# cebarker1000/heatflow

Hardware: AMD Instinct MI355X
Metric: DOF-updates/s (timesteps/s x nDOF) on geballe_with_diamond (higher is better)
Workload: dtype f64

## Files before the change

heatflow_amd/csrc/heatflow_hip.hip:

```cpp

#include "hf_amg_io.hpp"

namespace {

struct MeshTables {
  std::vector<int32_t> rowptr, colidx;
  ColDict spmv;
  RowGather rg;
  std::vector<char> tag_used;
  int max_blk_nnz = 0;
};

constexpr char BLOB_MAGIC[8] = {'H', 'F', 'P', 'A', 'T', '0', '2', 0};
struct BlobHeader {
  char magic[8];
  int64_t total_bytes, nnz;
  int32_t n, ne, rba, ts, max_blk_nnz, tab_len, rg_ok, rg_max_dict, spmv_max_dict, reserved;
  int64_t count[12];
};

void steady_swap(hf_ctx* ctx) {
  hf_ctx::Steady& S = ctx->steady;
  std::swap(ctx->nbc, S.nbc); std::swap(ctx->d_bc_dofs, S.bc_dofs); std::swap(ctx->d_g, S.g);
  std::swap(ctx->nlift_rows, S.nlift_rows); std::swap(ctx->nlift, S.nlift);
// ... 32 lines not shown
  dev_free(&ctx->d_load);
  ctx->have_load = false;
}

void source_free(hf_ctx* ctx) {
  dev_free(&ctx->src.F1); dev_free(&ctx->src.sum); dev_free(&ctx->src.absorb);
  ctx->src = hf_ctx::Source();
}

int source_steps_ok(hf_ctx* ctx, int64_t n_steps, const char* call) {
  hf_ctx::Source& S = ctx->src;
  if (!S.on) return HF_OK;
  if (!S.amp.empty() && S.next + static_cast<size_t>(n_steps) > S.amp.size())
    return fail(ctx, HF_ERR_STATE, "%s: the source has %zu amplitudes left for %lld steps (hf_set_source_amplitudes)", call,
                S.amp.size() - S.next, static_cast<long long>(n_steps));
  if (ctx->have_load && !S.sum) HF_TRY(dev_alloc(ctx, &S.sum, ctx->n));
  return HF_OK;
}

void tangent_free(hf_ctx* ctx) {
  free_batch_state(ctx->tanb);
  dev_free(&ctx->tan.col); dev_free(&ctx->tan.dir); dev_free(&ctx->tan.F);
  ctx->tan = hf_ctx::Tangent();
}

void kt_free(hf_ctx* ctx) {
  hf_ctx::KappaT& K = ctx->kt;
  dev_free(&K.hdr); dev_free(&K.vals); dev_free(&K.pic); dev_free(&K.b0); dev_free(&K.change);
  dev_free(&K.chdr); dev_free(&K.cvals); dev_free(&K.w);
  K = hf_ctx::KappaT();
}

void an_free(hf_ctx* ctx) {
  dev_free(&ctx->an.d_m);
  ctx->an = hf_ctx::Aniso();
}

const char* kt_kind(const hf_ctx* ctx) { return ctx->kt.k_on || !ctx->kt.c_on ? "kappa(T)" : "rho_c(T)"; }

int install_mesh(hf_ctx* ctx, int32_t n, int32_t ne, const double* zr, const int32_t* tri, const int32_t* tag, MeshTables& T) {
  free_batch(ctx);
  free_batch_state(ctx->fluxb);
  free_batch_cols(ctx);
  proj_free(ctx);
  steady_free(ctx);
  load_free(ctx);
  source_free(ctx);
  tangent_free(ctx);
  kt_free(ctx);
  an_free(ctx);
  value_lists_free(ctx);
  ctx->n = n; ctx->ne = ne; ctx->nnz = static_cast<int64_t>(T.colidx.size());
  ctx->nchunks = (n + RB - 1) / RB;
  ctx->nblk_a = (n + RBA - 1) / RBA;
  ctx->P = std::min(ctx->nchunks, MAXP);
  if (ctx->P >= 64) ctx->P &= ~7;
  ctx->nchunks_s = (n + SRPC - 1) / SRPC;
  ctx->Ps = std::min(ctx->nchunks_s, MAXP);
  if (ctx->Ps >= 64) ctx->Ps &= ~7;
  ctx->max_chunk_nnz_s = 0;
  for (int c = 0; c < ctx->nchunks_s; ++c)
    ctx->max_chunk_nnz_s = std::max(ctx->max_chunk_nnz_s, T.rowptr[std::min<int64_t>(n, (c + 1LL) * SRPC)] - T.rowptr[static_cast<size_t>(c) * SRPC]);
  ctx->max_cdict = T.spmv.max_dict;
  ctx->c16 = true;
  if (const char* e = std::getenv("HEATFLOW_SPMV_C16")) ctx->c16 = (e[0] != '0');
  if (static_cast<size_t>(ctx->max_chunk_nnz_s + ctx->max_cdict) * 8 > 64 * 1024) ctx->c16 = false;
  ctx->cdict_own = static_cast<int>(T.spmv.ptr.size()) == ctx->nchunks_s + 1;
  for (int c = 0; c < ctx->nchunks_s && ctx->cdict_own; ++c) {
    const int32_t r0 = c * SRPC, r1 = std::min<int32_t>(n, r0 + SRPC);
    const int32_t* lo = T.spmv.dict.data() + T.spmv.ptr[c];
    const int32_t* hi = T.spmv.dict.data() + T.spmv.ptr[c + 1];
    const int32_t* at = std::lower_bound(lo, hi, r0);
    ctx->cdict_own = hi - at >= r1 - r0 && at[0] == r0 && at[r1 - r0 - 1] == r1 - 1;
  }
  ctx->max_blk_nnz = T.max_blk_nnz;
  if (static_cast<size_t>((ctx->max_blk_nnz + 1) & ~1) * 16 + (RBA + 1) * 4 > 160 * 1024)
    return fail(ctx, HF_ERR_ARG, "row block holds %d nonzeros: LDS slab too large", ctx->max_blk_nnz);
  ctx->tab_len = static_cast<int>(T.tag_used.size());
  ctx->h_tag_used = T.tag_used;
  ctx->assembled = false; ctx->have_mat = false;
  ctx->h_tri.assign(tri, tri + 3 * static_cast<size_t>(ne));
  ctx->h_tag.assign(tag, tag + ne);
  ctx->owner_ready = false;
  ctx->ncolors = 0; ctx->elist_len = 0;
  dev_free(&ctx->d_blk_eptr); dev_free(&ctx->d_blk_cptr); dev_free(&ctx->d_blk_ent);

  std::vector<int4> elem(ne);
  for (int32_t e = 0; e < ne; ++e) elem[e] = make_int4(tri[3 * e], tri[3 * e + 1], tri[3 * e + 2], tag[e]);
  HF_TRY(dev_alloc(ctx, &ctx->d_zr, n));
  HF_TRY(dev_alloc(ctx, &ctx->d_elem, ne));
  HF_TRY(dev_alloc(ctx, &ctx->d_kappa, ctx->tab_len));
  HF_TRY(dev_alloc(ctx, &ctx->d_rhoc, ctx->tab_len));
  HF_TRY(dev_alloc(ctx, &ctx->d_rowptr, n + 1));
  HF_TRY(dev_alloc(ctx, &ctx->d_colidx, ctx->nnz));
  HF_TRY(dev_alloc(ctx, &ctx->d_cdict_ptr, T.spmv.ptr.size()));
  HF_TRY(dev_alloc(ctx, &ctx->d_cdict, T.spmv.dict.size()));
  HF_TRY(dev_alloc(ctx, &ctx->d_cid, T.spmv.id.size()));
  ctx->n_cdict = static_cast<int64_t>(T.spmv.dict.size());
  HF_HIP(copy_sync(ctx, ctx->d_zr, zr, sizeof(double) * 2 * n, hipMemcpyHostToDevice));
  ctx->rg_ok = T.rg.ok && rowgather_smem_bytes(T.max_blk_nnz, T.rg.cols.max_dict) <= 160 * 1024;
  std::fill_n(ctx->rg_grid, static_cast<int>(RG_VARIANTS), 0);
  if (ctx->rg_ok) {
    const RowGather& G = T.rg;
    ctx->rg_max_dict = G.cols.max_dict;
    ctx->h_rg_tags = G.tags;
    ctx->n_rg_ell = static_cast<int64_t>(G.ell.size());
    ctx->n_rg_dict = static_cast<int64_t>(G.cols.dict.size());
    HF_TRY(dev_alloc(ctx, &ctx->d_rg_hdr, G.hdr.size()));
    HF_TRY(dev_alloc(ctx, &ctx->d_rg_ell, G.ell.size()));
    HF_TRY(dev_alloc(ctx, &ctx->d_rg_cid, G.cols.id.size() + 16));
    HF_TRY(dev_alloc(ctx, &ctx->d_rg_dict, G.cols.dict.size()));
    HF_TRY(dev_alloc(ctx, &ctx->d_rg_zrb, G.cols.dict.size()));
    HF_TRY(dev_alloc(ctx, &ctx->d_kappa_rg, 64));
    HF_TRY(dev_alloc(ctx, &ctx->d_rhoc_rg, 64));
    HF_HIP(copy_sync(ctx, ctx->d_rg_hdr, G.hdr.data(), sizeof(int4) * G.hdr.size(), hipMemcpyHostToDevice));
    HF_HIP(copy_sync(ctx, ctx->d_rg_ell, G.ell.data(), sizeof(uint16_t) * G.ell.size(), hipMemcpyHostToDevice));
    HF_HIP(hipMemsetAsync(ctx->d_rg_cid + G.cols.id.size(), 0, sizeof(uint16_t) * 16, ctx->stream));
    HF_HIP(copy_sync(ctx, ctx->d_rg_cid, G.cols.id.data(), sizeof(uint16_t) * G.cols.id.size(), hipMemcpyHostToDevice));
    HF_HIP(copy_sync(ctx, ctx->d_rg_dict, G.cols.dict.data(), sizeof(int32_t) * G.cols.dict.size(), hipMemcpyHostToDevice));
    const int64_t total = ctx->n_rg_dict;
    hipLaunchKernelGGL(k_gather_coords, dim3(static_cast<unsigned>((total + 255) / 256)), dim3(256), 0, ctx->stream, total, ctx->d_rg_dict,
                       ctx->d_zr, ctx->d_rg_zrb);
    HF_HIP(hipGetLastError());
  }
  HF_TRY(dev_alloc(ctx, &ctx->d_M, ctx->nnz));
  HF_TRY(dev_alloc(ctx, &ctx->d_A, ctx->nnz));
  HF_TRY(dev_alloc(ctx, &ctx->d_dinv, n));
  HF_TRY(dev_alloc(ctx, &ctx->d_u, n));
  HF_TRY(dev_alloc(ctx, &ctx->d_uprev, n));
  HF_TRY(dev_alloc(ctx, &ctx->d_ustart, n));
  ctx->have_prev = false;
  ctx->bdf_hist = false;
  free_responses(ctx);
  HF_TRY(dev_alloc(ctx, &ctx->d_b, n));
  HF_TRY(dev_alloc(ctx, &ctx->d_r, 2 * static_cast<size_t>(n) + 4));
  HF_HIP(hipMemsetAsync(ctx->d_r, 0, sizeof(double) * (2 * static_cast<size_t>(n) + 4), ctx->stream));
  HF_TRY(dev_alloc(ctx, &ctx->d_p, n));
  HF_TRY(dev_alloc(ctx, &ctx->d_Ap, n));
  HF_TRY(dev_alloc(ctx, &ctx->d_tmp, n));
  HF_TRY(dev_alloc(ctx, &ctx->d_z, n));
  HF_TRY(dev_alloc(ctx, &ctx->d_z2, n));
  free_amg(ctx);
  HF_HIP(copy_sync(ctx, ctx->d_elem, elem.data(), sizeof(int4) * ne, hipMemcpyHostToDevice));
  HF_HIP(copy_sync(ctx, ctx->d_rowptr, T.rowptr.data(), sizeof(int32_t) * (n + 1), hipMemcpyHostToDevice));
  HF_HIP(copy_sync(ctx, ctx->d_colidx, T.colidx.data(), sizeof(int32_t) * ctx->nnz, hipMemcpyHostToDevice));
  HF_HIP(copy_sync(ctx, ctx->d_cdict_ptr, T.spmv.ptr.data(), sizeof(int32_t) * T.spmv.ptr.size(), hipMemcpyHostToDevice));
  HF_HIP(copy_sync(ctx, ctx->d_cdict, T.spmv.dict.data(), sizeof(int32_t) * T.spmv.dict.size(), hipMemcpyHostToDevice));
  HF_HIP(copy_sync(ctx, ctx->d_cid, T.spmv.id.data(), sizeof(uint16_t) * T.spmv.id.size(), hipMemcpyHostToDevice));
  HF_HIP(hipMemsetAsync(ctx->d_u, 0, sizeof(double) * n, ctx->stream));
  HF_HIP(hipStreamSynchronize(ctx->stream));
  ctx->h_rowptr.swap(T.rowptr);
  ctx->h_colidx.swap(T.colidx);
  ctx->nbc = 0; ctx->nlift = 0; ctx->nlift_rows = 0;
  ctx->have_mesh = true;
  ctx->pred_iters = 0;
  ctx->flux_ready = false;
  if (!ctx->rg_ok) HF_TRY(ensure_owner_lists(ctx));
  return HF_OK;
}

struct Section { const void* src; size_t bytes; bool on_device; };

void list_sections(const hf_ctx* c, Section out[12], int64_t count[12]) {
  const int nblk = c->nblk_a, nch = c->nchunks_s;
  const bool rg = c->rg_ok;
  const Section s[12] = {
      {c->h_rowptr.data(), sizeof(int32_t) * (static_cast<size_t>(c->n) + 1), false},
      {c->h_colidx.data(), sizeof(int32_t) * static_cast<size_t>(c->nnz), false},
      {c->d_cdict_ptr, sizeof(int32_t) * (static_cast<size_t>(nch) + 1), true},
      {c->d_cdict, sizeof(int32_t) * static_cast<size_t>(c->n_cdict), true},
      {c->d_cid, sizeof(uint16_t) * static_cast<size_t>(c->nnz), true},
      {c->h_tag_used.data(), c->h_tag_used.size(), false},
      {c->d_rg_hdr, rg ? sizeof(int4) * 2 * static_cast<size_t>(nblk) : 0, true},
      {c->d_rg_ell, rg ? sizeof(uint16_t) * static_cast<size_t>(c->n_rg_ell) : 0, true},
      {c->h_rg_tags.data(), rg ? sizeof(int32_t) * c->h_rg_tags.size() : 0, false},
      {c->d_rg_dict, rg ? sizeof(int32_t) * static_cast<size_t>(c->n_rg_dict) : 0, true},
      {c->d_rg_cid, rg ? sizeof(uint16_t) * static_cast<size_t>(c->nnz) : 0, true},
      {nullptr, 0, false}};
  const size_t unit[12] = {4, 4, 4, 4, 2, 1, 16, 2, 4, 4, 2, 1};
  for (int k = 0; k < 12; ++k) { out[k] = s[k]; count[k] = static_cast<int64_t>(s[k].bytes / unit[k]); }
}

int64_t mesh_tables_bytes(const hf_ctx* c) {
  Section s[12];
  int64_t cnt[12];
  list_sections(c, s, cnt);
  size_t total = pad16(sizeof(BlobHeader));
  for (int k = 0; k < 12; ++k) total += pad16(s[k].bytes);
  return static_cast<int64_t>(total);
}

int write_mesh_tables(hf_ctx* ctx, unsigned char* dst) {
  Section s[12];
  BlobHeader h{};
  list_sections(ctx, s, h.count);
  std::memcpy(h.magic, BLOB_MAGIC, 8);
  h.total_bytes = mesh_tables_bytes(ctx);
  h.nnz = ctx->nnz; h.n = ctx->n; h.ne = ctx->ne; h.rba = RBA; h.ts = SRPC; h.max_blk_nnz = ctx->max_blk_nnz;
  h.tab_len = ctx->tab_len; h.rg_ok = ctx->rg_ok ? 1 : 0; h.rg_max_dict = ctx->rg_max_dict; h.spmv_max_dict = ctx->max_cdict;
  std::memset(dst, 0, static_cast<size_t>(h.total_bytes));
  std::memcpy(dst, &h, sizeof h);
  size_t at = pad16(sizeof(BlobHeader));
  for (int k = 0; k < 12; ++k) {
    if (s[k].bytes) {
      if (s[k].on_device) HF_HIP(hipMemcpyAsync(dst + at, s[k].src, s[k].bytes, hipMemcpyDeviceToHost, ctx->stream));
      else std::memcpy(dst + at, s[k].src, s[k].bytes);
    }
    at += pad16(s[k].bytes);
  }
  HF_HIP(hipStreamSynchronize(ctx->stream));
  return HF_OK;
}

template <typename T>
bool take_section(const unsigned char* blob, int64_t bytes, size_t& at, int64_t count, std::vector<T>& out) {
  if (count < 0) return false;
  const size_t need = sizeof(T) * static_cast<size_t>(count);
  if (at + need > static_cast<size_t>(bytes)) return false;
  out.resize(static_cast<size_t>(count));
  if (need) std::memcpy(out.data(), blob + at, need);
  at += pad16(need);
  return true;
}

int parse_mesh_tables(hf_ctx* ctx, const unsigned char* blob, int64_t bytes, int32_t n, int32_t ne, MeshTables& T) {
  BlobHeader h;
  if (bytes < static_cast<int64_t>(sizeof h)) return fail(ctx, HF_ERR_ARG, "hf_set_mesh_prebuilt: blob too short");
  std::memcpy(&h, blob, sizeof h);
  if (std::memcmp(h.magic, BLOB_MAGIC, 8) != 0) return fail(ctx, HF_ERR_ARG, "hf_set_mesh_prebuilt: not a pattern blob of this library version");
  if (h.total_bytes != bytes) return fail(ctx, HF_ERR_ARG, "hf_set_mesh_prebuilt: blob says %lld bytes, %lld given", (long long)h.total_bytes, (long long)bytes);
  if (h.n != n || h.ne != ne) return fail(ctx, HF_ERR_ARG, "hf_set_mesh_prebuilt: blob was exported for a mesh of %d nodes / %d triangles, not %d / %d", h.n, h.ne, n, ne);
  if (h.rba != RBA || h.ts != SRPC) return fail(ctx, HF_ERR_ARG, "hf_set_mesh_prebuilt: blob built for other block sizes");
  size_t at = pad16(sizeof(BlobHeader));
  std::vector<int4> hdr;
  bool ok = take_section(blob, bytes, at, h.count[0], T.rowptr) && take_section(blob, bytes, at, h.count[1], T.colidx) &&
            take_section(blob, bytes, at, h.count[2], T.spmv.ptr) && take_section(blob, bytes, at, h.count[3], T.spmv.dict) &&
            take_section(blob, bytes, at, h.count[4], T.spmv.id) && take_section(blob, bytes, at, h.count[5], T.tag_used) &&
            take_section(blob, bytes, at, h.count[6], T.rg.hdr) && take_section(blob, bytes, at, h.count[7], T.rg.ell) &&
            take_section(blob, bytes, at, h.count[8], T.rg.tags) && take_section(blob, bytes, at, h.count[9], T.rg.cols.dict) &&
            take_section(blob, bytes, at, h.count[10], T.rg.cols.id);
  const int nblk = (n + RBA - 1) / RBA, nch = (n + SRPC - 1) / SRPC;
  ok = ok && T.rowptr.size() == static_cast<size_t>(n) + 1 && T.rowptr[0] == 0 && T.rowptr[n] == h.nnz &&
       T.colidx.size() == static_cast<size_t>(h.nnz) && T.spmv.ptr.size() == static_cast<size_t>(nch) + 1 &&
       T.spmv.id.size() == T.colidx.size() && static_cast<int>(T.tag_used.size()) == h.tab_len && h.tab_len > 0 &&
       !T.spmv.ptr.empty() && T.spmv.ptr.back() == static_cast<int32_t>(T.spmv.dict.size());
  if (ok && h.rg_ok)
    ok = T.rg.hdr.size() == 2 * static_cast<size_t>(nblk) && T.rg.cols.id.size() == T.colidx.size() && !T.rg.tags.empty() &&
         T.rg.tags.size() <= 64 && h.rg_max_dict > 0 && h.rg_max_dict <= RBA * RG_NX;
  if (!ok) return fail(ctx, HF_ERR_ARG, "hf_set_mesh_prebuilt: blob sections do not fit the mesh");
  for (int32_t i = 0; i < n && ok; ++i) ok = T.rowptr[i + 1] > T.rowptr[i];
  for (size_t k = 0; k < T.colidx.size() && ok; ++k) ok = T.colidx[k] >= 0 && T.colidx[k] < n;
  for (size_t k = 0; k < T.spmv.dict.size() && ok; ++k) ok = T.spmv.dict[k] >= 0 && T.spmv.dict[k] < n;
  for (int c = 0; c < nch && ok; ++c) {
    const int nd = T.spmv.ptr[c + 1] - T.spmv.ptr[c];
    ok = nd > 0 && nd <= h.spmv_max_dict;
    for (int32_t k = T.rowptr[static_cast<size_t>(c) * SRPC]; k < T.rowptr[std::min<int64_t>(n, (c + 1LL) * SRPC)] && ok; ++k) ok = T.spmv.id[k] < nd;
  }
  if (ok && h.rg_ok) {
    for (size_t k = 0; k < T.rg.cols.dict.size() && ok; ++k) ok = T.rg.cols.dict[k] >= 0 && T.rg.cols.dict[k] < n;
    const int64_t ell16 = static_cast<int64_t>(T.rg.ell.size() / 8);
    for (int b = 0; b < nblk && ok; ++b) {
      const int4 A = T.rg.hdr[2 * b], B = T.rg.hdr[2 * b + 1];
      const int32_t r0 = b * RBA, r1 = std::min<int32_t>(n, r0 + RBA);
      ok = A.x == T.rowptr[r0] && A.y == T.rowptr[r1] - T.rowptr[r0] && A.z >= 0 && A.w > 0 && A.w <= h.rg_max_dict &&
           static_cast<size_t>(A.z) + A.w <= T.rg.cols.dict.size() && B.x >= 0 && B.y >= 1 &&
           static_cast<int64_t>(B.x) + static_cast<int64_t>(B.y) * RBA <= ell16 && B.z >= 0 && B.z + (r1 - r0) <= A.w && B.w == r1 - r0 &&
           A.y <= h.max_blk_nnz;
      for (int32_t k = A.x; k < A.x + A.y && ok; ++k) ok = T.rg.cols.id[k] < A.w;
      for (int32_t i = r0; i < r1 && ok; ++i) {
        const int len = T.rowptr[i + 1] - T.rowptr[i];
        ok = len <= 32;
        for (int g = 0; g < B.y && ok; ++g)
          for (int j = 0; j < 8 && ok; ++j) {
            const unsigned e = T.rg.ell[(static_cast<size_t>(B.x) + static_cast<size_t>(g) * RBA + (i - r0)) * 8 + j];
            ok = e == 0xFFFFu || (static_cast<int>(e & 31u) < len && static_cast<int>((e >> 5) & 31u) < len && (e >> 10) < T.rg.tags.size());
          }
      }
    }
  }
  if (!ok) return fail(ctx, HF_ERR_ARG, "hf_set_mesh_prebuilt: blob holds an index outside its range");
  T.spmv.max_dict = h.spmv_max_dict;
  T.max_blk_nnz = h.max_blk_nnz;
  T.rg.ok = h.rg_ok != 0;
  T.rg.cols.max_dict = h.rg_max_dict;
  return HF_OK;
}

int blob_on_host(hf_ctx* ctx, const void* blob, int64_t bytes, std::vector<unsigned char>& staged, const unsigned char** src) {
  hipPointerAttribute_t at{};
  const hipError_t e = hipPointerGetAttributes(&at, blob);
  if (e != hipSuccess) (void)hipGetLastError();
  const bool on_device = e == hipSuccess && at.type == hipMemoryTypeDevice;
  if (!on_device) { *src = static_cast<const unsigned char*>(blob); return HF_OK; }
  staged.resize(static_cast<size_t>(bytes));
  HF_HIP(hipMemcpy(staged.data(), blob, static_cast<size_t>(bytes), hipMemcpyDeviceToHost));
  *src = staged.data();
  return HF_OK;
}

int upload_rg_tables(hf_ctx* ctx, const std::vector<double>& by_tag_k, const std::vector<double>* by_tag_c) {
  if (!ctx->rg_ok) return HF_OK;
  std::vector<double> k(64, 0.0), c(64, 0.0);
  for (size_t q = 0; q < ctx->h_rg_tags.size(); ++q) {
    k[q] = by_tag_k[ctx->h_rg_tags[q]];
    if (by_tag_c) c[q] = (*by_tag_c)[ctx->h_rg_tags[q]];
  }
// ... 64 lines not shown
    }
  }
  return HF_OK;
}

int ensure_batch_flux(hf_ctx* ctx, int nv, int ncomp) {
  hf_ctx::Batch& F = ctx->fluxnb;
  if (F.nv == nv && (ncomp < 2 || F.uprev != nullptr)) return HF_OK;
  free_batch_state(F);
  const size_t vec = static_cast<size_t>(ctx->n) * nv;
  for (double** v : {&F.u, &F.b, &F.r, &F.p, &F.Ap, &F.z}) {
    HF_TRY(dev_alloc(ctx, v, vec));
    HF_HIP(hipMemsetAsync(*v, 0, sizeof(double) * vec, ctx->stream));
  }
  if (ncomp == 2) {
    HF_TRY(dev_alloc(ctx, &F.uprev, vec));
    HF_HIP(hipMemsetAsync(F.uprev, 0, sizeof(double) * vec, ctx->stream));
  }
  HF_TRY(dev_alloc(ctx, &F.part_pAp, static_cast<size_t>(nv) * MAXP));
  HF_TRY(dev_alloc(ctx, &F.part_rz, 2 * static_cast<size_t>(nv) * MAXP));
  HF_TRY(dev_alloc(ctx, &F.part_zz, static_cast<size_t>(nv) * MAXP));
  HF_TRY(dev_alloc(ctx, &F.part_bn, static_cast<size_t>(nv) * MAXP));
  HF_TRY(dev_alloc(ctx, &F.scal, nv));
  HF_TRY(dev_alloc(ctx, &F.red, 1));
  HF_HIP(hipMemsetAsync(F.scal, 0, sizeof(Scal) * nv, ctx->stream));
  HF_HIP(hipMemsetAsync(F.red, 0, sizeof(BRed), ctx->stream));
  if (hipHostMalloc(reinterpret_cast<void**>(&F.h_scal), sizeof(Scal) * nv) != hipSuccess) return fail(ctx, HF_ERR_ALLOC, "hipHostMalloc failed");
  const int rpb = TPB / nv;
  F.Pb = static_cast<int>(std::min<size_t>((static_cast<size_t>(ctx->n) + rpb - 1) / rpb, MAXP));
  if (F.Pb >= 64) F.Pb &= ~7;
  F.opk = 0; F.pred_iters = 0;
  F.sysA = ctx->d_M1; F.sysDinv = ctx->d_dinv1;
  F.lds = ctx->bcols.nv == nv;
  HF_HIP(hipStreamSynchronize(ctx->stream));
  F.nv = nv;
  return HF_OK;
}

int batch_flux_step(hf_ctx* ctx, int components, double rtol, int max_it, int nfs, double* out, int32_t* it_out) {
  hf_ctx::Batch& B = ctx->batch;
  hf_ctx::Batch& F = ctx->fluxnb;
  const int nv = B.nv;
  const int capd = ctx->rg_max_dict;
  const size_t sm = static_cast<size_t>(capd) * 16 + static_cast<size_t>(capd + (capd & 1)) * 8 + (RBA + 4) * 4 +
                    (static_cast<size_t>((ctx->max_blk_nnz + 1) & ~1) / 8 + 3) * 16;
  const int grid = std::min(ctx->nblk_a, 2048);
  int done = 0;
  for (int comp = 0; comp < 2; ++comp) {
    if (!((components >> comp) & 1)) continue;
    const bool second = done == 1;
    if (second) std::swap(F.u, F.uprev);
    for (int j = 0; j < nv; ++j)
      hipLaunchKernelGGL(k_grad_rows, dim3(grid), dim3(RBA), sm, ctx->stream, ctx->nblk_a, capd, ctx->d_rg_hdr,
                         reinterpret_cast<const uint4*>(ctx->d_rg_ell), reinterpret_cast<const uint4*>(ctx->d_rg_cid), ctx->d_rg_zrb,
                         ctx->d_rg_dict, ctx->d_rowptr, B.u, comp == 0 ? F.b + j : static_cast<double*>(nullptr),
                         comp == 1 ? F.b + j : static_cast<double*>(nullptr), nv, nv, j);
    HF_HIP(hipGetLastError());
    std::swap(ctx->batch, ctx->fluxnb);
    const int rc = batch_dispatch(ctx, [&](auto ops) { return decltype(ops)::pcg(ctx, false, rtol, 0.0, max_it); });
    int itmax = 0;
    for (int j = 0; j < nv; ++j) itmax = std::max(itmax, ctx->batch.h_scal[j].iters);
    std::swap(ctx->batch, ctx->fluxnb);
    if (it_out) it_out[done] = itmax;
    if (rc != HF_OK) { if (second) std::swap(F.u, F.uprev); return rc; }
    double* o = out + static_cast<size_t>(done) * nv * nfs;
    const int thr = nfs * nv;
    switch (nv) {
      case 2: hipLaunchKernelGGL((kb_gather<2>), dim3((thr + 255) / 256), dim3(256), 0, ctx->stream, nfs, ctx->d_fsamp_idx, F.u, o); break;
      case 4: hipLaunchKernelGGL((kb_gather<4>), dim3((thr + 255) / 256), dim3(256), 0, ctx->stream, nfs, ctx->d_fsamp_idx, F.u, o); break;
      case 8: hipLaunchKernelGGL((kb_gather<8>), dim3((thr + 255) / 256), dim3(256), 0, ctx->stream, nfs, ctx->d_fsamp_idx, F.u, o); break;
      default: hipLaunchKernelGGL((kb_gather<16>), dim3((thr + 255) / 256), dim3(256), 0, ctx->stream, nfs, ctx->d_fsamp_idx, F.u, o); break;
    }
    HF_HIP(hipGetLastError());
    if (second) std::swap(F.u, F.uprev);
    ++done;
  }
  return HF_OK;
}
int tangent_reset(hf_ctx* ctx) {
  hf_ctx::Batch& T = ctx->tanb;
  if (T.nv == 0) return HF_OK;
  HF_HIP(hipMemsetAsync(T.u, 0, sizeof(double) * static_cast<size_t>(ctx->n) * T.nv, ctx->stream));
  HF_HIP(hipStreamSynchronize(ctx->stream));
  T.bdf_hist = false;
  for (bool& u_ : T.pused) u_ = false;
  T.pnext = 0; T.ppending = -1;
  T.pred_iters = 0;
  return HF_OK;
}

int tangent_levels(hf_ctx* ctx) {
  hf_ctx::Batch& T = ctx->tanb;
  std::vector<int64_t> sig;
  if (ctx->precond == 1 && ctx->amg_ready)
    for (const DevLevel& L : ctx->amg) { sig.push_back(L.n); sig.push_back(L.P.ncol); }
  if (sig == ctx->tan.lev_sig) return HF_OK;
  for (auto& L : T.lev) { dev_free(&L.x); dev_free(&L.cat); if (L.own_b) dev_free(&L.b); }
  T.lev.clear();
  HF_TRY(batch_levels(ctx, T, T.nv));
  HF_HIP(hipStreamSynchronize(ctx->stream));
  ctx->tan.lev_sig = sig;
  return HF_OK;
}

int tangent_load(hf_ctx* ctx) {
  const int capd = ctx->rg_max_dict;
  const size_t sm = static_cast<size_t>(capd) * 16 + static_cast<size_t>(capd + (capd & 1)) * 8 + (RBA + 4) * 4 +
                    (static_cast<size_t>((ctx->max_blk_nnz + 1) & ~1) / 8 + 3) * 16;
  const int grid = std::min(ctx->nblk_a, 2048);
#define HF_TL(NV) hipLaunchKernelGGL(k_tangent_load<NV>, dim3(grid), dim3(RBA), sm, ctx->stream, ctx->nblk_a, capd, ctx->d_rg_hdr, \
                                     reinterpret_cast<const uint4*>(ctx->d_rg_ell), reinterpret_cast<const uint4*>(ctx->d_rg_cid), \
                                     ctx->d_rg_zrb, ctx->d_rg_dict, ctx->d_rowptr, ctx->tan.col, ctx->d_u, ctx->tan.F)
#define HF_TLD(NV) hipLaunchKernelGGL(k_tangent_load_dir<NV>, dim3(grid), dim3(RBA), sm, ctx->stream, ctx->nblk_a, capd, ctx->d_rg_hdr, \
                                      reinterpret_cast<const uint4*>(ctx->d_rg_ell), reinterpret_cast<const uint4*>(ctx->d_rg_cid), \
                                      ctx->d_rg_zrb, ctx->d_rg_dict, ctx->d_rowptr, ctx->tan.dir, ctx->d_u, ctx->tan.F)
  if (ctx->tan.dir) {
    switch (ctx->tan.nv) {
      case 2: HF_TLD(2); break;
      case 4: HF_TLD(4); break;
      case 8: HF_TLD(8); break;
      default: HF_TLD(16); break;
    }
  } else {
    switch (ctx->tan.nv) {
      case 2: HF_TL(2); break;
      case 4: HF_TL(4); break;
      case 8: HF_TL(8); break;
      default: HF_TL(16); break;
    }
  }
#undef HF_TLD
#undef HF_TL
  HF_HIP(hipGetLastError());
  return HF_OK;
}

}

extern "C" {

const char* hf_version(void) { return "heatflow_hip 0.1 (gfx950)"; }

const char* hf_last_error(const hf_ctx* ctx) { return ctx ? ctx->err.c_str() : "null context"; }

int hf_create(int device_id, hf_ctx** out) {
  if (!out) return HF_ERR_ARG;
  *out = nullptr;
  int count = 0;
  if (hipGetDeviceCount(&count) != hipSuccess || count <= 0) return HF_ERR_HIP;
  if (device_id < 0 || device_id >= count) return HF_ERR_ARG;
  hf_ctx* ctx = new hf_ctx();
  ctx->dev = device_id;
  if (const char* e = std::getenv("HEATFLOW_VALUE_LISTS")) ctx->vl_mode = (e[0] == '0') ? 0 : (e[0] == '2') ? 2 : 1;
  auto bail = [&](int rc) { *out = ctx; return rc; };
  if (hipSetDevice(device_id) != hipSuccess) return bail(fail(ctx, HF_ERR_HIP, "hipSetDevice(%d) failed", device_id));
  if (hipStreamCreateWithFlags(&ctx->stream, hipStreamNonBlocking) != hipSuccess)
    return bail(fail(ctx, HF_ERR_HIP, "hipStreamCreate failed"));
  if (hipEventCreate(&ctx->ev0) != hipSuccess || hipEventCreate(&ctx->ev1) != hipSuccess)
    return bail(fail(ctx, HF_ERR_HIP, "hipEventCreate failed"));
  if (hipHostMalloc(reinterpret_cast<void**>(&ctx->h_scal), sizeof(Scal)) != hipSuccess)
    return bail(fail(ctx, HF_ERR_ALLOC, "hipHostMalloc failed"));
  if (hipHostMalloc(reinterpret_cast<void**>(&ctx->h_mirror), sizeof(ScalMirror), hipHostMallocMapped | hipHostMallocCoherent) != hipSuccess ||
      hipHostGetDevicePointer(reinterpret_cast<void**>(&ctx->d_mirror), ctx->h_mirror, 0) != hipSuccess)
    return bail(fail(ctx, HF_ERR_ALLOC, "hipHostMalloc (mapped) failed"));
  *ctx->h_mirror = ScalMirror{};
  int rc = dev_alloc(ctx, &ctx->d_scal, 1);
  if (rc == HF_OK) rc = dev_alloc(ctx, &ctx->d_part_pAp, MAXP);
  if (rc == HF_OK) rc = dev_alloc(ctx, &ctx->d_part_rz, 2 * MAXP);
  if (rc == HF_OK) rc = dev_alloc(ctx, &ctx->d_part_zz, MAXP);
  if (rc == HF_OK) rc = dev_alloc(ctx, &ctx->d_part_bn, MAXP);
  if (rc == HF_OK && reset_scal(ctx) != HF_OK) rc = HF_ERR_HIP;
  if (rc == HF_OK) {
    hipLaunchKernelGGL(k_zero_entries, dim3(1), dim3(64), 0, ctx->stream, 0, static_cast<const int32_t*>(nullptr), static_cast<double*>(nullptr));
    if (hipStreamSynchronize(ctx->stream) != hipSuccess) rc = fail(ctx, HF_ERR_HIP, "first kernel launch failed: %s", hipGetErrorString(hipGetLastError()));
  }
  *out = ctx;
  return rc;
}

int hf_destroy(hf_ctx* ctx) {
  if (!ctx) return HF_ERR_ARG;
  (void)hipSetDevice(ctx->dev);
  if (ctx->stream) (void)hipStreamSynchronize(ctx->stream);
  dev_free(&ctx->d_zr); dev_free(&ctx->d_elem); dev_free(&ctx->d_kappa); dev_free(&ctx->d_rhoc);
  dev_free(&ctx->d_rowptr); dev_free(&ctx->d_colidx); dev_free(&ctx->d_cdict_ptr); dev_free(&ctx->d_cdict); dev_free(&ctx->d_cid); dev_free(&ctx->d_blk_eptr); dev_free(&ctx->d_blk_cptr); dev_free(&ctx->d_blk_ent); dev_free(&ctx->d_rg_hdr); dev_free(&ctx->d_rg_ell); dev_free(&ctx->d_rg_cid); dev_free(&ctx->d_rg_dict); dev_free(&ctx->d_rg_zrb); dev_free(&ctx->d_kappa_rg); dev_free(&ctx->d_rhoc_rg); dev_free(&ctx->d_M); dev_free(&ctx->d_A); dev_free(&ctx->d_dinv);
  dev_free(&ctx->d_bc_dofs); dev_free(&ctx->d_g); dev_free(&ctx->d_lift_rows); dev_free(&ctx->d_lift_ptr);
  dev_free(&ctx->d_lift_bc); dev_free(&ctx->d_lift_slot); dev_free(&ctx->d_lift_val);
  dev_free(&ctx->d_uprev); dev_free(&ctx->d_ustart);
  dev_free(&ctx->d_u); dev_free(&ctx->d_b); dev_free(&ctx->d_r); dev_free(&ctx->d_p); dev_free(&ctx->d_Ap);
  free_batch(ctx); free_batch_state(ctx->fluxb); free_batch_cols(ctx); free_amg(ctx); free_responses(ctx); proj_free(ctx); dev_free(&ctx->d_z); dev_free(&ctx->d_z2);
  steady_free(ctx); load_free(ctx); source_free(ctx); tangent_free(ctx); kt_free(ctx); an_free(ctx); value_lists_free(ctx);
  dev_free(&ctx->d_M1); dev_free(&ctx->d_dinv1); dev_free(&ctx->d_gz); dev_free(&ctx->d_gr); dev_free(&ctx->d_bz); dev_free(&ctx->d_br);
  dev_free(&ctx->d_tmp); dev_free(&ctx->d_part_pAp); dev_free(&ctx->d_part_rz); dev_free(&ctx->d_part_zz);
  dev_free(&ctx->d_part_bn); dev_free(&ctx->d_scal); dev_free(&ctx->d_samp_idx); dev_free(&ctx->d_samp); dev_free(&ctx->d_fsamp_idx);
  for (auto& e : ctx->prof_ev) (void)hipEventDestroy(e);
  if (ctx->h_scal) (void)hipHostFree(ctx->h_scal);
  if (ctx->h_mirror) (void)hipHostFree(ctx->h_mirror);
  if (ctx->ev0) (void)hipEventDestroy(ctx->ev0);
  if (ctx->ev1) (void)hipEventDestroy(ctx->ev1);
  if (ctx->stream) (void)hipStreamDestroy(ctx->stream);
  delete ctx;
  return HF_OK;
}

int hf_set_mesh(hf_ctx* ctx, int32_t n, int32_t ne, const double* zr, const int32_t* tri, const int32_t* tag) {
  if (!ctx) return HF_ERR_ARG;
  if (!zr || !tri || !tag || n <= 0 || ne <= 0) return fail(ctx, HF_ERR_ARG, "hf_set_mesh: null pointer or empty mesh");
  HF_HIP(hipSetDevice(ctx->dev));
  int32_t maxtag = 0;
  for (int64_t k = 0; k < 3LL * ne; ++k)
    if (tri[k] < 0 || tri[k] >= n) return fail(ctx, HF_ERR_ARG, "hf_set_mesh: triangle %lld references node %d outside [0,%d)", (long long)(k / 3), tri[k], n);
  for (int32_t e = 0; e < ne; ++e) {
    if (tag[e] < 0) return fail(ctx, HF_ERR_ARG, "hf_set_mesh: negative cell tag at cell %d", e);
    maxtag = std::max(maxtag, tag[e]);
    const double* p0 = zr + 2 * tri[3 * e], *p1 = zr + 2 * tri[3 * e + 1], *p2 = zr + 2 * tri[3 * e + 2];
    const double d = (p1[0] - p0[0]) * (p2[1] - p0[1]) - (p2[0] - p0[0]) * (p1[1] - p0[1]);
    if (!(d != 0.0)) return fail(ctx, HF_ERR_ARG, "hf_set_mesh: degenerate triangle %d", e);
  }
  const auto t0 = std::chrono::steady_clock::now();
  auto lap = [&](const char* what) {
    if (std::getenv("HEATFLOW_DEBUG")) std::fprintf(stderr, "[set_mesh] %-28s %.3f s\n", what, std::chrono::duration<double>(std::chrono::steady_clock::now() - t0).count());
  };
  lap("checked");
  MeshTables T;
  Pattern P;
  HF_TRY(build_csr(ctx, n, ne, tri, P));
  lap("+ csr pattern");
  build_rowgather(n, ne, tri, tag, P);
  lap("+ row-gather lists");
  if (!build_coldict(P.rowptr, P.colidx, n, SRPC, T.spmv)) return fail(ctx, HF_ERR_ARG, "an SpMV chunk touches more than 65535 columns (16-bit positions)");
  lap("+ spmv column lists");
  T.rowptr.swap(P.rowptr);
  T.colidx.swap(P.colidx);
  T.max_blk_nnz = P.max_blk_nnz;
  T.rg = std::move(P.rg);
  T.tag_used.assign(static_cast<size_t>(maxtag) + 1, 0);
  for (int32_t e = 0; e < ne; ++e) T.tag_used[tag[e]] = 1;
  const int rc = install_mesh(ctx, n, ne, zr, tri, tag, T);
  lap("+ installed");
  return rc;
}

int hf_set_mesh_prebuilt(hf_ctx* ctx, int32_t n, int32_t ne, const double* zr, const int32_t* tri, const int32_t* tag,
                         const void* blob, int64_t bytes) {
  if (!ctx) return HF_ERR_ARG;
  if (!zr || !tri || !tag || !blob || n <= 0 || ne <= 0 || bytes <= 0) return fail(ctx, HF_ERR_ARG, "hf_set_mesh_prebuilt: null pointer or empty mesh");
  HF_HIP(hipSetDevice(ctx->dev));
  std::vector<unsigned char> staged;
  const unsigned char* src = nullptr;
  HF_TRY(blob_on_host(ctx, blob, bytes, staged, &src));
  MeshTables T;
  HF_TRY(parse_mesh_tables(ctx, src, bytes, n, ne, T));
  return install_mesh(ctx, n, ne, zr, tri, tag, T);
}

int hf_pattern_export_size(hf_ctx* ctx, int64_t* bytes) {
  if (!ctx || !bytes) return HF_ERR_ARG;
  if (!ctx->have_mesh) return fail(ctx, HF_ERR_STATE, "hf_pattern_export_size before hf_set_mesh");
  *bytes = mesh_tables_bytes(ctx);
  return HF_OK;
}

int hf_pattern_export(hf_ctx* ctx, void* blob, int64_t bytes) {
  if (!ctx || !blob) return HF_ERR_ARG;
  if (!ctx->have_mesh) return fail(ctx, HF_ERR_STATE, "hf_pattern_export before hf_set_mesh");
  if (bytes != mesh_tables_bytes(ctx)) return fail(ctx, HF_ERR_ARG, "hf_pattern_export: buffer of %lld bytes, need %lld", (long long)bytes, (long long)mesh_tables_bytes(ctx));
  HF_HIP(hipSetDevice(ctx->dev));
  std::vector<unsigned char> host(static_cast<size_t>(bytes));
  HF_TRY(write_mesh_tables(ctx, host.data()));
  HF_HIP(hipMemcpy(blob, host.data(), static_cast<size_t>(bytes), hipMemcpyDefault));
  return HF_OK;
}

int hf_set_materials(hf_ctx* ctx, int32_t n_mat, const int32_t* tags, const double* kappa, const double* rho_c) {
  if (!ctx) return HF_ERR_ARG;
  if (!ctx->have_mesh) return fail(ctx, HF_ERR_STATE, "hf_set_materials before hf_set_mesh");
  if (n_mat <= 0 || !tags || !kappa || !rho_c) return fail(ctx, HF_ERR_ARG, "hf_set_materials: bad arguments");
  HF_HIP(hipSetDevice(ctx->dev));
  std::vector<double> tk(ctx->tab_len, std::nan("")), tc(ctx->tab_len, std::nan(""));
  for (int32_t i = 0; i < n_mat; ++i) {
    if (tags[i] < 0) return fail(ctx, HF_ERR_ARG, "hf_set_materials: negative tag");
    if (!(kappa[i] > 0.0) || !(rho_c[i] > 0.0)) return fail(ctx, HF_ERR_ARG, "hf_set_materials: kappa and rho_c must be positive");
    if (tags[i] < ctx->tab_len) { tk[tags[i]] = kappa[i]; tc[tags[i]] = rho_c[i]; }
  }
  for (int t = 0; t < ctx->tab_len; ++t)
    if (ctx->h_tag_used[t] && std::isnan(tk[t])) return fail(ctx, HF_ERR_ARG, "hf_set_materials: cell tag %d has no material", t);
  HF_HIP(copy_sync(ctx, ctx->d_kappa, tk.data(), sizeof(double) * ctx->tab_len, hipMemcpyHostToDevice));
  HF_HIP(copy_sync(ctx, ctx->d_rhoc, tc.data(), sizeof(double) * ctx->tab_len, hipMemcpyHostToDevice));
  HF_TRY(upload_rg_tables(ctx, tk, &tc));
  ctx->have_mat = true;
  ctx->assembled = false;
  ctx->steady.ready = false;
  return tangent_reset(ctx);
}

int hf_set_anisotropy(hf_ctx* ctx, int32_t n, const int32_t* tags, const double* m_z, const double* m_r) {
  if (!ctx) return HF_ERR_ARG;
  if (!ctx->have_mesh || !ctx->have_mat) return fail(ctx, HF_ERR_STATE, "hf_set_anisotropy needs hf_set_mesh and hf_set_materials first");
  if (n < 0) return fail(ctx, HF_ERR_ARG, "hf_set_anisotropy: negative tag count");
  if (n > 0 && (!tags || !m_z || !m_r)) return fail(ctx, HF_ERR_ARG, "hf_set_anisotropy: null pointer");
  std::vector<double> by_tag(2 * static_cast<size_t>(ctx->tab_len), 1.0);
  std::vector<char> listed(ctx->tab_len, 0), aniso(ctx->tab_len, 0);
  std::vector<double2> m(64, make_double2(1.0, 1.0));
  bool any = false;
  for (int32_t i = 0; i < n; ++i) {
    const int32_t tg = tags[i];
    if (tg < 0 || tg >= ctx->tab_len || !ctx->h_tag_used[tg]) return fail(ctx, HF_ERR_ARG, "hf_set_anisotropy: tag %d is not a cell tag of the mesh", tg);
    if (listed[tg]) return fail(ctx, HF_ERR_ARG, "hf_set_anisotropy: tag %d listed twice", tg);
    if (!(m_z[i] > 0.0) || !std::isfinite(m_z[i]) || !(m_r[i] > 0.0) || !std::isfinite(m_r[i]))
      return fail(ctx, HF_ERR_ARG, "hf_set_anisotropy: multipliers of tag %d are not positive and finite", tg);
    listed[tg] = 1;
    if (m_z[i] == 1.0 && m_r[i] == 1.0) continue;
    aniso[tg] = 1; any = true;
    by_tag[2 * tg] = m_z[i]; by_tag[2 * tg + 1] = m_r[i];
  }
  if (any && ctx->kt.on)
    return fail(ctx, HF_ERR_STATE, "hf_set_anisotropy: %s tables are set (the table kernels are isotropic)", kt_kind(ctx));
  if (any && (!ctx->rg_ok || (ctx->assembled && ctx->mode != HF_ASM_ROW_GATHER)))
    return fail(ctx, HF_ERR_ARG, "hf_set_anisotropy: anisotropic conductivities are assembled by the row-gather kernel only (HF_ASM_ROW_GATHER on a mesh with row-gather lists)");
  for (int tg = 0; tg < ctx->tab_len; ++tg) {
    if (!aniso[tg]) continue;
    const size_t q = std::find(ctx->h_rg_tags.begin(), ctx->h_rg_tags.end(), tg) - ctx->h_rg_tags.begin();
    if (q >= ctx->h_rg_tags.size() || q >= 64) return fail(ctx, HF_ERR_ARG, "hf_set_anisotropy: tag %d has no row-gather dictionary entry", tg);
    m[q] = make_double2(by_tag[2 * tg], by_tag[2 * tg + 1]);
  }
  HF_HIP(hipSetDevice(ctx->dev));
  if (!any && !ctx->an.on) return HF_OK;
  if (any) {
    if (!ctx->an.d_m) HF_TRY(dev_alloc(ctx, &ctx->an.d_m, 64));
    HF_HIP(copy_sync(ctx, ctx->an.d_m, m.data(), sizeof(double2) * 64, hipMemcpyHostToDevice));
    ctx->an.h_tag = std::move(aniso);
    ctx->an.hash = fnv1a(by_tag.data(), sizeof(double) * by_tag.size());
    ctx->an.h_m = std::move(by_tag);
    ctx->an.on = true;
  } else {
    an_free(ctx);
  }
  free_batch(ctx);
  ctx->assembled = false;
  ctx->pred_iters = 0;
  ctx->steady.ready = false;
  const bool from_steady = ctx->tan.steady_state;
  tangent_free(ctx);
  ctx->tan.steady_state = from_steady;
  return HF_OK;
}

int hf_update_kappa(hf_ctx* ctx, int32_t n_mat, const int32_t* tags, const double* kappa) {
  if (!ctx) return HF_ERR_ARG;
  if (!ctx->have_mat || !ctx->assembled) return fail(ctx, HF_ERR_STATE, "hf_update_kappa needs a completed hf_assemble first");
  if (n_mat <= 0 || !tags || !kappa) return fail(ctx, HF_ERR_ARG, "hf_update_kappa: bad arguments");
  HF_HIP(hipSetDevice(ctx->dev));
  std::vector<double> tk(ctx->tab_len);
  HF_HIP(copy_sync(ctx, tk.data(), ctx->d_kappa, sizeof(double) * ctx->tab_len, hipMemcpyDeviceToHost));
  for (int32_t i = 0; i < n_mat; ++i) {
    if (tags[i] < 0 || tags[i] >= ctx->tab_len || !ctx->h_tag_used[tags[i]])
      return fail(ctx, HF_ERR_ARG, "hf_update_kappa: tag %d is not a cell tag of the mesh", tags[i]);
    if (!(kappa[i] > 0.0)) return fail(ctx, HF_ERR_ARG, "hf_update_kappa: kappa must be positive");
    if (ctx->kt.k_on && ctx->kt.tabled[tags[i]])
      return fail(ctx, HF_ERR_ARG, "hf_update_kappa: tag %d carries a kappa(T) table (hf_set_kappa_tables)", tags[i]);
  }
  for (int32_t i = 0; i < n_mat; ++i) {
    tk[tags[i]] = kappa[i];
  }
  HF_HIP(copy_sync(ctx, ctx->d_kappa, tk.data(), sizeof(double) * ctx->tab_len, hipMemcpyHostToDevice));
  HF_TRY(upload_rg_tables(ctx, tk, nullptr));
  ctx->steady.ready = false;
  return hf_assemble(ctx, ctx->dt_step, ctx->mode);
}

int hf_set_dirichlet(hf_ctx* ctx, int32_t n_bc, const int32_t* dofs) {
  if (!ctx) return HF_ERR_ARG;
  if (!ctx->have_mesh) return fail(ctx, HF_ERR_STATE, "hf_set_dirichlet before hf_set_mesh");
  if (n_bc < 0 || (n_bc > 0 && !dofs)) return fail(ctx, HF_ERR_ARG, "hf_set_dirichlet: bad arguments");
  HF_HIP(hipSetDevice(ctx->dev));
  std::vector<char> seen(ctx->n, 0);
  for (int32_t q = 0; q < n_bc; ++q) {
    if (dofs[q] < 0 || dofs[q] >= ctx->n) return fail(ctx, HF_ERR_ARG, "hf_set_dirichlet: dof %d outside [0,%d)", dofs[q], ctx->n);
    if (seen[dofs[q]]) return fail(ctx, HF_ERR_ARG, "hf_set_dirichlet: dof %d listed twice (resolve overlaps on the host)", dofs[q]);
    seen[dofs[q]] = 1;
  }
  free_batch(ctx);
  ctx->nbc = n_bc;
  HF_TRY(dev_alloc(ctx, &ctx->d_bc_dofs, n_bc));
  HF_TRY(dev_alloc(ctx, &ctx->d_g, n_bc));
  if (n_bc > 0) HF_HIP(copy_sync(ctx, ctx->d_bc_dofs, dofs, sizeof(int32_t) * n_bc, hipMemcpyHostToDevice));
  HF_TRY(build_lift(ctx));
  free_amg(ctx);
  free_responses(ctx);
  ctx->assembled = false;
  return HF_OK;
}

int hf_assemble(hf_ctx* ctx, double dt, int32_t mode) {
  if (!ctx) return HF_ERR_ARG;
  if (!ctx->have_mesh || !ctx->have_mat) return fail(ctx, HF_ERR_STATE, "hf_assemble needs hf_set_mesh and hf_set_materials first");
  if (!(dt > 0.0)) return fail(ctx, HF_ERR_ARG, "hf_assemble: dt must be positive");
  if (mode < 0 || mode > 3) return fail(ctx, HF_ERR_ARG, "hf_assemble: unknown mode %d", mode);
  if (ctx->kt.on && mode != HF_ASM_ROW_GATHER)
    return fail(ctx, HF_ERR_ARG, "hf_assemble: %s tables are evaluated by the row-gather kernel only (HF_ASM_ROW_GATHER)", kt_kind(ctx));
  if (ctx->an.on && (mode != HF_ASM_ROW_GATHER || !ctx->rg_ok))
    return fail(ctx, HF_ERR_ARG, "hf_assemble: anisotropic conductivities (hf_set_anisotropy) are assembled by the row-gather kernel only (HF_ASM_ROW_GATHER)");
  HF_HIP(hipSetDevice(ctx->dev));
  ctx->dt_step = dt;
  ctx->dt = ctx->scheme == HF_TIME_BDF2 ? 2.0 * dt / 3.0 : dt;
  ctx->mode = mode;
  HF_HIP(hipEventRecord(ctx->ev0, ctx->stream));
  value_lists_touch(ctx, ctx->d_A);
  value_lists_touch(ctx, ctx->d_M);
  HF_TRY(launch_assemble(ctx));
  if (ctx->kt.on) {
    HF_TRY(kt_revalue(ctx, ctx->d_u, nullptr));
  } else {
    if (ctx->nbc > 0) {
      if (ctx->nlift > 0)
        hipLaunchKernelGGL(k_take_lift, dim3((ctx->nlift + 255) / 256), dim3(256), 0, ctx->stream, ctx->nlift,
                           ctx->d_lift_slot, ctx->d_A, ctx->d_lift_val);
      hipLaunchKernelGGL(k_bc_rows, dim3((ctx->nbc + 255) / 256), dim3(256), 0, ctx->stream, ctx->nbc, ctx->d_bc_dofs,
                         ctx->d_rowptr, ctx->d_colidx, ctx->d_A);
    }
    hipLaunchKernelGGL(k_dinv, dim3((ctx->n + 255) / 256), dim3(256), 0, ctx->stream, ctx->n, ctx->d_rowptr,
                       ctx->d_colidx, ctx->d_A, ctx->d_dinv);
  }
  const bool lists = value_lists_wanted(ctx);
  if (lists) {
    HF_TRY(value_lists_build(ctx, 0, ctx->d_A));
    HF_TRY(value_lists_build(ctx, 1, ctx->d_M));
  }
  HF_HIP(hipEventRecord(ctx->ev1, ctx->stream));
  HF_HIP(hipGetLastError());
  HF_HIP(hipStreamSynchronize(ctx->stream));
  float ms = 0.f;
  HF_HIP(hipEventElapsedTime(&ms, ctx->ev0, ctx->ev1));
  ctx->last_ms = ms;
  if (lists) HF_TRY(value_lists_finish(ctx));
  if (ctx->precond == 1) {
    OperatorPrint now;
    HF_TRY(operator_print(ctx, now));
    if (!(ctx->amg_ready && ctx->amg_reuse)) {
      HF_TRY(build_amg_auto(ctx));
      ctx->amg_print = std::move(now);
    } else {
      ctx->amg_fine_stale = !same_print(now, ctx->amg_print) || ctx->kt.on;
    }
  }
  if (ctx->precond == 1 && ctx->amg_ready) {
    ctx->amg[0].A.val = ctx->d_A;
    ctx->amg[0].dinv = ctx->d_dinv;
  }
  ctx->assembled = true;
  ctx->pred_iters = 0;
  ctx->have_prev = false;
  ctx->bdf_hist = false;
  free_responses(ctx);
  return tangent_reset(ctx);
}

int hf_set_precond(hf_ctx* ctx, int32_t kind, int32_t reuse) {
  if (!ctx) return HF_ERR_ARG;
  if (kind < 0 || kind > 1) return fail(ctx, HF_ERR_ARG, "hf_set_precond: unknown preconditioner %d", kind);
  if (kind != ctx->precond) { ctx->assembled = false; ctx->pred_iters = 0; (void)hipSetDevice(ctx->dev); free_batch(ctx); }
  if (kind == 0) { (void)hipSetDevice(ctx->dev); free_amg(ctx); }
  ctx->precond = kind;
  ctx->amg_reuse = reuse ? 1 : 0;
  return HF_OK;
}

int hf_set_time_scheme(hf_ctx* ctx, int32_t scheme) {
  if (!ctx) return HF_ERR_ARG;
  if (scheme != HF_TIME_BACKWARD_EULER && scheme != HF_TIME_BDF2) return fail(ctx, HF_ERR_ARG, "hf_set_time_scheme: unknown scheme %d", scheme);
  if (scheme != ctx->scheme) {
    (void)hipSetDevice(ctx->dev);
    free_batch(ctx);
    ctx->assembled = false;
    ctx->pred_iters = 0;
    ctx->scheme = scheme;
  }
  return HF_OK;
}

int kt_set_tables(hf_ctx* ctx, bool cap, int32_t n_tab, const int32_t* tags, const double* t0, const double* dT, const int32_t* n_knots,
                  const double* values) {
  const char* fn = cap ? "hf_set_rhoc_tables" : "hf_set_kappa_tables";
  const char* what = cap ? "rho_c(T)" : "kappa(T)";
  if (!ctx) return HF_ERR_ARG;
  if (!ctx->have_mesh) return fail(ctx, HF_ERR_STATE, "%s before hf_set_mesh", fn);
  if (n_tab < 0) return fail(ctx, HF_ERR_ARG, "%s: negative table count", fn);
  HF_HIP(hipSetDevice(ctx->dev));
  hf_ctx::KappaT& K = ctx->kt;
  if (n_tab == 0) {
    if (ctx->steady.picard) ctx->steady.ready = false;
    if (cap ? K.c_on : K.k_on) {
      free_batch(ctx);
      ctx->assembled = false;
      ctx->pred_iters = 0;
    }
    if (!(cap ? K.k_on : K.c_on)) { kt_free(ctx); return HF_OK; }
    if (cap ? K.c_on : K.k_on) {
      const std::vector<KTab> none(64, KTab{0.0, 0.0, 0, 0});
      HF_HIP(copy_sync(ctx, cap ? K.chdr : K.hdr, none.data(), sizeof(KTab) * 64, hipMemcpyHostToDevice));
      dev_free(cap ? &K.cvals : &K.vals);
      (cap ? K.ctabled : K.tabled).clear();
      (cap ? K.c_on : K.k_on) = false;
      K.have_change = false;
    }
    return HF_OK;
  }
  if (!tags || !t0 || !dT || !n_knots || !values) return fail(ctx, HF_ERR_ARG, "%s: null pointer", fn);
  if (ctx->an.on) return fail(ctx, HF_ERR_STATE, "%s: anisotropic conductivities are set (hf_set_anisotropy; the table kernels are isotropic)", fn);
  if (!ctx->rg_ok || (ctx->assembled && ctx->mode != HF_ASM_ROW_GATHER))
    return fail(ctx, HF_ERR_ARG, "%s: %s is evaluated by the row-gather kernel only (HF_ASM_ROW_GATHER on a mesh with row-gather lists)", fn, what);
  if (cap && ct_smem_bytes(ctx->max_blk_nnz, ctx->rg_max_dict) + 2 * 64 * sizeof(KTab) > 160 * 1024)
    return fail(ctx, HF_ERR_ARG, "%s: the (M, A) slab, the staged state and the table headers of this mesh exceed the 160 KiB of LDS", fn);
  std::vector<KTab> hdr(64, KTab{0.0, 0.0, 0, 0});
  std::vector<double> vals;
  std::vector<char> tabled(ctx->tab_len, 0);
  for (int32_t i = 0; i < n_tab; ++i) {
    const int32_t tg = tags[i];
    if (tg < 0 || tg >= ctx->tab_len || !ctx->h_tag_used[tg]) return fail(ctx, HF_ERR_ARG, "%s: tag %d is not a cell tag of the mesh", fn, tg);
    if (tabled[tg]) return fail(ctx, HF_ERR_ARG, "%s: tag %d listed twice", fn, tg);
    if (n_knots[i] < 2 || n_knots[i] > KT_MAX_KNOTS)
      return fail(ctx, HF_ERR_ARG, "%s: table of tag %d has %d knots (2..%d)", fn, tg, n_knots[i], KT_MAX_KNOTS);
    if (!std::isfinite(t0[i]) || !(dT[i] > 0.0) || !std::isfinite(dT[i]) || !std::isfinite(t0[i] + (n_knots[i] - 1) * dT[i]))
      return fail(ctx, HF_ERR_ARG, "%s: table of tag %d: T0 finite and dT > 0 needed", fn, tg);
    tabled[tg] = 1;
    const size_t q = std::find(ctx->h_rg_tags.begin(), ctx->h_rg_tags.end(), tg) - ctx->h_rg_tags.begin();
    if (q >= ctx->h_rg_tags.size()) return fail(ctx, HF_ERR_ARG, "%s: tag %d has no row-gather dictionary entry", fn, tg);
    hdr[q] = KTab{t0[i], 1.0 / dT[i], n_knots[i], static_cast<int>(vals.size())};
    for (int32_t k = 0; k < n_knots[i]; ++k) {
      const double v = values[vals.size()];
      if (!(v > 0.0) || !std::isfinite(v)) return fail(ctx, HF_ERR_ARG, "%s: value %d of the table of tag %d is not positive and finite", fn, k, tg);
      vals.push_back(v);
    }
  }
  free_batch(ctx);
  if (ctx->steady.picard) ctx->steady.ready = false;
  if (!K.hdr) {
    HF_TRY(dev_alloc(ctx, &K.hdr, 64));
    HF_TRY(dev_alloc(ctx, &K.pic, ctx->n));
// ... 1062 lines not shown
  if (!ctx) return HF_ERR_ARG;
  hf_ctx::Batch& B = ctx->batch;
  if (B.nv == 0) return fail(ctx, HF_ERR_STATE, "hf_batch_run: no batch is open");
  if (!ctx->assembled) return fail(ctx, HF_ERR_STATE, "hf_batch_run before hf_assemble");
  if (B.opk == HF_BATCH_PER_COLUMN && B.loaded != (1u << B.nv) - 1u) return fail(ctx, HF_ERR_STATE, "hf_batch_run: not every column's operator has been loaded");
  if (B.opk == HF_BATCH_AFFINE && B.loaded == 0) return fail(ctx, HF_ERR_STATE, "hf_batch_run: hf_batch_set_affine has not been called");
  if (n_steps <= 0 || (ctx->nbc > 0 && !g_all) || max_it <= 0 || rtol < 0 || atol < 0) return fail(ctx, HF_ERR_ARG, "hf_batch_run: bad arguments");
  if (ns < 0 || (ns > 0 && (!nodes || !samples))) return fail(ctx, HF_ERR_ARG, "hf_batch_run: bad sample arguments");
  for (int32_t q = 0; q < ns; ++q)
    if (nodes[q] < 0 || nodes[q] >= ctx->n) return fail(ctx, HF_ERR_ARG, "hf_batch_run: node %d outside [0,%d)", nodes[q], ctx->n);
  const int ncomp = (flux_components & 1) + ((flux_components >> 1) & 1);
  if (flux_components != 0) {
    if (flux_components < 0 || flux_components > 3 || flux_max_it <= 0 || flux_rtol < 0 || nfs <= 0 || !flux_nodes || !flux_samples)
      return fail(ctx, HF_ERR_ARG, "hf_batch_run_flux: bad flux arguments");
    if (!ctx->flux_ready) return fail(ctx, HF_ERR_STATE, "hf_batch_run_flux before hf_flux_setup");
    if (!ctx->rg_ok) return fail(ctx, HF_ERR_ARG, "hf_batch_run_flux: the row-gather lists are not available for this mesh (a row of more than 32 entries or more than 64 cell tags): project run by run");
    for (int32_t q = 0; q < nfs; ++q)
      if (flux_nodes[q] < 0 || flux_nodes[q] >= ctx->n) return fail(ctx, HF_ERR_ARG, "hf_batch_run_flux: node %d outside [0,%d)", flux_nodes[q], ctx->n);
  }
  HF_HIP(hipSetDevice(ctx->dev));
  const int nv = B.nv;
  const size_t gstep = static_cast<size_t>(ctx->nbc) * nv;
  DevTemp<double> t_sall, t_fall;
  if (flux_components != 0) {
    HF_TRY(ensure_batch_flux(ctx, nv, ncomp));
    if (nfs > ctx->fsamp_cap) { HF_TRY(dev_alloc(ctx, &ctx->d_fsamp_idx, nfs)); ctx->fsamp_cap = nfs; }
    HF_HIP(copy_sync(ctx, ctx->d_fsamp_idx, flux_nodes, sizeof(int32_t) * nfs, hipMemcpyHostToDevice));
    HF_TRY(dev_alloc(ctx, &t_fall.p, static_cast<size_t>(n_steps) * ncomp * nv * nfs));
  }
  if (ctx->nbc > 0) {
    HF_TRY(dev_alloc(ctx, &B.g, gstep * n_steps));
    HF_HIP(copy_sync(ctx, B.g, g_all, sizeof(double) * gstep * n_steps, hipMemcpyHostToDevice));
  }
  if (ns > 0) {
    HF_TRY(ensure_samples(ctx, ns));
    HF_TRY(dev_alloc(ctx, &t_sall.p, static_cast<size_t>(n_steps) * nv * ns));
    HF_HIP(copy_sync(ctx, ctx->d_samp_idx, nodes, sizeof(int32_t) * ns, hipMemcpyHostToDevice));
  }
  int rc = HF_OK;
  HF_HIP(hipEventRecord(ctx->ev0, ctx->stream));
  for (int32_t s = 0; s < n_steps && rc == HF_OK; ++s) {
    const double* gs = ctx->nbc > 0 ? B.g + gstep * s : nullptr;
    rc = batch_dispatch(ctx, [&](auto ops) { return decltype(ops)::step(ctx, gs, rtol, atol, max_it); });
    if (iters)
      for (int j = 0; j < nv; ++j) iters[static_cast<size_t>(s) * nv + j] = B.h_scal[j].iters;
    if (ns > 0 && rc == HF_OK) {
      double* out = t_sall.p + static_cast<size_t>(s) * nv * ns;
      const int thr = ns * nv;
      switch (nv) {
        case 2: hipLaunchKernelGGL((kb_gather<2>), dim3((thr + 255) / 256), dim3(256), 0, ctx->stream, ns, ctx->d_samp_idx, B.u, out); break;
        case 4: hipLaunchKernelGGL((kb_gather<4>), dim3((thr + 255) / 256), dim3(256), 0, ctx->stream, ns, ctx->d_samp_idx, B.u, out); break;
        case 8: hipLaunchKernelGGL((kb_gather<8>), dim3((thr + 255) / 256), dim3(256), 0, ctx->stream, ns, ctx->d_samp_idx, B.u, out); break;
        default: hipLaunchKernelGGL((kb_gather<16>), dim3((thr + 255) / 256), dim3(256), 0, ctx->stream, ns, ctx->d_samp_idx, B.u, out); break;
      }
    }
    if (flux_components != 0 && rc == HF_OK)
      rc = batch_flux_step(ctx, flux_components, flux_rtol, flux_max_it, nfs, t_fall.p + static_cast<size_t>(s) * ncomp * nv * nfs,
                           flux_iters ? flux_iters + static_cast<size_t>(s) * ncomp : nullptr);
  }
  (void)hipEventRecord(ctx->ev1, ctx->stream);
  (void)hipStreamSynchronize(ctx->stream);
  float ms = 0.f;
  (void)hipEventElapsedTime(&ms, ctx->ev0, ctx->ev1);
  ctx->last_ms = ms;
  if (ns > 0 && rc == HF_OK) (void)copy_sync(ctx, samples, t_sall.p, sizeof(double) * n_steps * nv * ns, hipMemcpyDeviceToHost);
  if (flux_components != 0 && rc == HF_OK)
    (void)copy_sync(ctx, flux_samples, t_fall.p, sizeof(double) * n_steps * ncomp * nv * nfs, hipMemcpyDeviceToHost);
  return rc;
}

int hf_get_sizes(hf_ctx* ctx, int32_t* n, int32_t* ne, int64_t* nnz, int32_t* nbc) {
  if (!ctx) return HF_ERR_ARG;
  if (n) *n = ctx->n;
  if (ne) *ne = ctx->ne;
  if (nnz) *nnz = ctx->nnz;
  if (nbc) *nbc = ctx->nbc;
  return HF_OK;
}

int hf_get_csr(hf_ctx* ctx, int32_t* rowptr, int32_t* colidx, double* A, double* M) {
  if (!ctx) return HF_ERR_ARG;
  if (!ctx->have_mesh) return fail(ctx, HF_ERR_STATE, "hf_get_csr before hf_set_mesh");
  if ((A || M) && !ctx->assembled) return fail(ctx, HF_ERR_STATE, "hf_get_csr: values requested before hf_assemble");
  HF_HIP(hipSetDevice(ctx->dev));
  if (rowptr) std::memcpy(rowptr, ctx->h_rowptr.data(), sizeof(int32_t) * (ctx->n + 1));
  if (colidx) std::memcpy(colidx, ctx->h_colidx.data(), sizeof(int32_t) * ctx->nnz);
  if (A) HF_HIP(copy_sync(ctx, A, ctx->d_A, sizeof(double) * ctx->nnz, hipMemcpyDeviceToHost));
  if (M) HF_HIP(copy_sync(ctx, M, ctx->d_M, sizeof(double) * ctx->nnz, hipMemcpyDeviceToHost));
  return HF_OK;
}

int hf_set_value_lists(hf_ctx* ctx, int32_t mode) {
  if (!ctx) return HF_ERR_ARG;
  if (mode < 0 || mode > 2) return fail(ctx, HF_ERR_ARG, "hf_set_value_lists: unknown mode %d", mode);
  ctx->vl_mode = mode;
  return HF_OK;
}

int hf_get_value_lists(hf_ctx* ctx, int32_t which, int32_t* valid, int64_t* sum_vlist, int32_t* max_vlist, int32_t* vcap, int32_t* vptr,
                       double* vlist, uint32_t* cv) {
  if (!ctx) return HF_ERR_ARG;
  if (which < 0 || which > 1) return fail(ctx, HF_ERR_ARG, "hf_get_value_lists: which = %d (0 = A, 1 = M)", which);
  if (!ctx->assembled) return fail(ctx, HF_ERR_STATE, "hf_get_value_lists before hf_assemble");
  const hf_ctx::ValueLists& L = ctx->vl[which];
  const bool live = L.valid && L.src == (which ? ctx->d_M : ctx->d_A);
  if (valid) *valid = live ? 1 : 0;
  if (sum_vlist) *sum_vlist = L.sum_vlist;
  if (max_vlist) *max_vlist = L.max_vlist;
  if (vcap) *vcap = ctx->vl_vcap;
  if (vptr || vlist || cv) {
    if (!live) return fail(ctx, HF_ERR_STATE, "hf_get_value_lists: the tables of %s are not valid", which ? "M" : "A");
    HF_HIP(hipSetDevice(ctx->dev));
    if (vptr) HF_HIP(copy_sync(ctx, vptr, L.vptr, sizeof(int32_t) * (static_cast<size_t>(ctx->nchunks_s) + 1), hipMemcpyDeviceToHost));
    if (vlist) HF_HIP(copy_sync(ctx, vlist, L.vlist, sizeof(double) * static_cast<size_t>(L.sum_vlist), hipMemcpyDeviceToHost));
    if (cv) HF_HIP(copy_sync(ctx, cv, L.cv, sizeof(uint32_t) * static_cast<size_t>(ctx->nnz), hipMemcpyDeviceToHost));
  }
  return HF_OK;
}

int hf_get_projection(hf_ctx* ctx, int32_t column, int32_t* mh, int32_t* mt, int32_t* used, int32_t* next, int32_t* pending, double* G,
                      double* alpha, double* V, double* F) {
  if (mh) *mh = PROJ_MH;
  if (mt) *mt = PROJ_MT;
  if (!used && !next && !pending && !G && !alpha && !V && !F) return HF_OK;
  if (!ctx) return HF_ERR_ARG;
  const hf_ctx::Batch& B = ctx->batch;
  const bool single = column < 0;
  if (single && !ctx->proj.ready) return fail(ctx, HF_ERR_STATE, "hf_get_projection: no projection basis is allocated yet (no step with start vector 3)");
  if (!single && B.nv == 0) return fail(ctx, HF_ERR_STATE, "hf_get_projection: no batch is open");
  if (!single && column >= B.nv) return fail(ctx, HF_ERR_ARG, "hf_get_projection: column %d outside [0,%d)", column, B.nv);
  HF_HIP(hipSetDevice(ctx->dev));
  HF_HIP(hipStreamSynchronize(ctx->stream));
  const int slots = single ? PROJ_MT : PROJ_MH;
  const size_t n = static_cast<size_t>(ctx->n);
  for (int k = 0; k < PROJ_MT; ++k)
    if (used) used[k] = k < slots && (single ? ctx->proj.used[k] : B.pused[k]) ? 1 : 0;
  if (next) *next = single ? ctx->proj.next : B.pnext;
  if (pending) *pending = single ? ctx->proj.pending : B.ppending;
  if (G)
    HF_HIP(copy_sync(ctx, G, single ? ctx->proj.G : B.pG + static_cast<size_t>(column) * PROJ_MT * PROJ_MT, sizeof(double) * PROJ_MT * PROJ_MT,
                     hipMemcpyDeviceToHost));
  if (alpha)
    HF_HIP(copy_sync(ctx, alpha, single ? ctx->proj.alpha : B.palpha + static_cast<size_t>(column) * (PROJ_MT + 1), sizeof(double) * (PROJ_MT + 1),
                     hipMemcpyDeviceToHost));
  if (V || F) {
    std::vector<double> wide(single ? 0 : n * B.nv);
    for (int k = 0; k < PROJ_MT; ++k)
      for (int s = 0; s < 2; ++s) {
        double* out = s ? F : V;
        if (!out) continue;
        out += static_cast<size_t>(k) * n;
        const bool on = k < slots && (single ? ctx->proj.used[k] : B.pused[k]);
        if (!on) { std::fill(out, out + n, 0.0); continue; }
        if (single) {
          HF_HIP(copy_sync(ctx, out, s ? ctx->proj.F[k] : ctx->proj.V[k], sizeof(double) * n, hipMemcpyDeviceToHost));
        } else {
          HF_HIP(copy_sync(ctx, wide.data(), s ? B.pF[k] : B.pV[k], sizeof(double) * n * B.nv, hipMemcpyDeviceToHost));
          for (size_t i = 0; i < n; ++i) out[i] = wide[i * B.nv + column];
        }
      }
  }
  return HF_OK;
}

int hf_spmv(hf_ctx* ctx, int32_t which, const double* x, double* y) {
  if (!ctx) return HF_ERR_ARG;
  if (!ctx->assembled || !x || !y || which < 0 || which > 1) return fail(ctx, HF_ERR_STATE, "hf_spmv: not assembled or bad arguments");
  HF_HIP(hipSetDevice(ctx->dev));
  HF_HIP(copy_sync(ctx, ctx->d_tmp, x, sizeof(double) * ctx->n, hipMemcpyHostToDevice));
  launch_spmv<0>(ctx, which ? ctx->d_M : ctx->d_A, ctx->d_tmp, ctx->d_Ap);
  HF_HIP(hipGetLastError());
  HF_HIP(hipStreamSynchronize(ctx->stream));
  HF_HIP(copy_sync(ctx, y, ctx->d_Ap, sizeof(double) * ctx->n, hipMemcpyDeviceToHost));
  return HF_OK;
}

int hf_amg_apply(hf_ctx* ctx, const double* r, double* z, double* rz) {
  if (!ctx || !r || !z) return HF_ERR_ARG;
  if (ctx->precond != 1 || !ctx->amg_ready || !ctx->assembled || ctx->amg.empty())
    return fail(ctx, HF_ERR_STATE, "hf_amg_apply: no assembled operator with a multigrid hierarchy (hf_set_precond(1, ...) and hf_assemble first)");
  HF_HIP(hipSetDevice(ctx->dev));
  const int n = ctx->n, nl = static_cast<int>(ctx->amg.size());
  HF_TRY(reset_scal(ctx));
  std::vector<double> dinv(n), z0(n);
  HF_HIP(copy_sync(ctx, dinv.data(), ctx->d_dinv, sizeof(double) * n, hipMemcpyDeviceToHost));
  const double w0 = ctx->amg[0].omega;
  for (int i = 0; i < n; ++i) z0[i] = w0 * (dinv[i] * r[i]);
  auto poison = [&](double* p, size_t count) { return count ? hipMemsetAsync(p, 0xFF, sizeof(double) * count, ctx->stream) : hipSuccess; };
  HF_HIP(poison(ctx->d_tmp, n));
  HF_HIP(poison(ctx->d_z2, n));
  HF_HIP(poison(ctx->d_part_rz, MAXP));
  for (int l = 1; l < nl; ++l) {
    DevLevel& L = ctx->amg[l];
    if (L.cat) HF_HIP(poison(L.cat, static_cast<size_t>(L.n) + ctx->amg[l + 1].n));
    else HF_HIP(poison(L.b, L.n));
    if (l == 1) HF_HIP(poison(L.res, L.n));
  }
  HF_HIP(copy_sync(ctx, ctx->d_r, r, sizeof(double) * n, hipMemcpyHostToDevice));
  HF_HIP(copy_sync(ctx, ctx->d_z, z0.data(), sizeof(double) * n, hipMemcpyHostToDevice));
  vcycle(ctx, 0);
  HF_HIP(hipGetLastError());
  HF_HIP(hipStreamSynchronize(ctx->stream));
  HF_HIP(copy_sync(ctx, z, ctx->d_z2, sizeof(double) * n, hipMemcpyDeviceToHost));
  if (rz) {
    std::vector<double> part(ctx->P);
    HF_HIP(copy_sync(ctx, part.data(), ctx->d_part_rz, sizeof(double) * ctx->P, hipMemcpyDeviceToHost));
    double s = 0.0;
    for (double v : part) s += v;
    *rz = s;
  }
  return HF_OK;
}

int hf_batch_apply_precond(hf_ctx* ctx, const double* r, double* z, double* rz) {
  if (!ctx || !r || !z) return HF_ERR_ARG;
  hf_ctx::Batch& B = ctx->batch;
  if (B.nv == 0) return fail(ctx, HF_ERR_STATE, "hf_batch_apply_precond: no batch is open (hf_batch_begin)");
  if (ctx->precond != 1 || !ctx->amg_ready || !ctx->assembled || ctx->amg.empty() || B.lev.size() != ctx->amg.size())
    return fail(ctx, HF_ERR_STATE, "hf_batch_apply_precond: the batch has no multigrid hierarchy");
  HF_HIP(hipSetDevice(ctx->dev));
  const int nv = B.nv, nl = static_cast<int>(ctx->amg.size());
  const size_t n = static_cast<size_t>(ctx->n), vec = n * nv;
  const bool dpc = B.opk != HF_BATCH_SHARED;
  std::vector<double> dinv(dpc ? vec : n), ri(vec), z0(vec);
  HF_HIP(copy_sync(ctx, dinv.data(), dpc ? B.dinv : ctx->d_dinv, sizeof(double) * dinv.size(), hipMemcpyDeviceToHost));
  const double w0 = ctx->amg[0].omega;
  for (size_t i = 0; i < n; ++i)
    for (int j = 0; j < nv; ++j) {
      const size_t q = i * nv + j;
      ri[q] = r[static_cast<size_t>(j) * n + i];
      z0[q] = w0 * ((dpc ? dinv[q] : dinv[i]) * ri[q]);
    }
  auto poison = [&](double* p, size_t count) { return count ? hipMemsetAsync(p, 0xFF, sizeof(double) * count, ctx->stream) : hipSuccess; };
  HF_HIP(poison(B.tmp, vec));
  HF_HIP(poison(B.z2, vec));
  HF_HIP(poison(B.part_rz, static_cast<size_t>(nv) * MAXP));
  for (int l = 1; l < nl; ++l) {
    const hf_ctx::BatchLevel& Q = B.lev[l];
    const size_t ln = static_cast<size_t>(ctx->amg[l].n);
    if (Q.cat) HF_HIP(poison(Q.cat, (ln + ctx->amg[l + 1].n) * nv));
    else HF_HIP(poison(Q.b, ln * nv));
    if (l == 1) HF_HIP(poison(Q.res, ln * nv));
  }
  HF_HIP(hipMemsetAsync(B.scal, 0, sizeof(Scal) * nv, ctx->stream));
  HF_HIP(copy_sync(ctx, B.r, ri.data(), sizeof(double) * vec, hipMemcpyHostToDevice));
  HF_HIP(copy_sync(ctx, B.z, z0.data(), sizeof(double) * vec, hipMemcpyHostToDevice));
  HF_TRY(batch_dispatch(ctx, [&](auto ops) { decltype(ops)::vcycle(ctx, 0); return HF_OK; }));
  HF_HIP(hipGetLastError());
  HF_HIP(hipStreamSynchronize(ctx->stream));
  std::vector<double> zi(vec);
  HF_HIP(copy_sync(ctx, zi.data(), B.z2, sizeof(double) * vec, hipMemcpyDeviceToHost));
  for (size_t i = 0; i < n; ++i)
    for (int j = 0; j < nv; ++j) z[static_cast<size_t>(j) * n + i] = zi[i * nv + j];
  if (rz) {
    BRed red;
    HF_HIP(copy_sync(ctx, &red, B.red, sizeof(BRed), hipMemcpyDeviceToHost));
    for (int j = 0; j < nv; ++j) rz[j] = red.rz[0][j];
  }
  return HF_OK;
}

int hf_dense_inverse(hf_ctx* ctx, int32_t n, const int32_t* ptr, const int32_t* idx, const double* val, const double* b,
                     double* inv, double* x64, double* x32) {
  if (!ctx) return HF_ERR_ARG;
  if (n < 1 || n > 4096 || !ptr || (ptr[n] > 0 && (!idx || !val)))
    return fail(ctx, HF_ERR_ARG, "hf_dense_inverse: n = %d outside [1, 4096] or a null array", n);
  if (ptr[0] != 0) return fail(ctx, HF_ERR_ARG, "hf_dense_inverse: row pointer does not start at 0");
  for (int i = 0; i < n; ++i)
    if (ptr[i + 1] < ptr[i]) return fail(ctx, HF_ERR_ARG, "hf_dense_inverse: row pointer decreases at row %d", i);
  if ((x64 || x32) && !b) return fail(ctx, HF_ERR_ARG, "hf_dense_inverse: products asked for without b");
  HF_HIP(hipSetDevice(ctx->dev));
  const int ld = (n + 3) & ~3;
  const size_t cnt = static_cast<size_t>(n) * ld;
  DevTemp<double> t_inv, t_b, t_x;
  DevTemp<float> t_invf;
  DevTemp<Scal> t_scal;
  HF_TRY(dev_alloc(ctx, &t_inv.p, cnt));
  HF_TRY(dense_inverse(ctx, n, ptr, idx, val, t_inv.p));
  if (inv) {
    HF_HIP(hipMemcpy2DAsync(inv, sizeof(double) * n, t_inv.p, sizeof(double) * ld, sizeof(double) * n, n, hipMemcpyDeviceToHost, ctx->stream));
    HF_HIP(hipStreamSynchronize(ctx->stream));
  }
  if (x64 || x32) {
    HF_TRY(dev_alloc(ctx, &t_b.p, static_cast<size_t>(n) + 4));
    HF_TRY(dev_alloc(ctx, &t_x.p, n));
    HF_TRY(dev_alloc(ctx, &t_scal.p, 1));
    HF_HIP(hipMemsetAsync(t_b.p, 0, sizeof(double) * (n + 4), ctx->stream));
    HF_HIP(hipMemsetAsync(t_scal.p, 0, sizeof(Scal), ctx->stream));
    HF_HIP(copy_sync(ctx, t_b.p, b, sizeof(double) * n, hipMemcpyHostToDevice));
    const int g = std::max(1, std::min((n + 1) / 2, 2048));
    if (x64) {
      HF_HIP(hipMemsetAsync(t_x.p, 0xFF, sizeof(double) * n, ctx->stream));
      hipLaunchKernelGGL(k_dense_mv, dim3(g), dim3(TPB), 0, ctx->stream, n, ld, t_inv.p, t_b.p, t_x.p, t_scal.p);
      HF_HIP(hipGetLastError());
      HF_HIP(copy_sync(ctx, x64, t_x.p, sizeof(double) * n, hipMemcpyDeviceToHost));
    }
    if (x32) {
      HF_TRY(dev_alloc(ctx, &t_invf.p, cnt));
      hipLaunchKernelGGL(k_to_float, dim3(1024), dim3(256), 0, ctx->stream, cnt, t_inv.p, t_invf.p);
      HF_HIP(hipMemsetAsync(t_x.p, 0xFF, sizeof(double) * n, ctx->stream));
      hipLaunchKernelGGL(k_dense_mv_f32, dim3(g), dim3(TPB), 0, ctx->stream, n, ld, t_invf.p, t_b.p, t_x.p, t_scal.p);
      HF_HIP(hipGetLastError());
      HF_HIP(copy_sync(ctx, x32, t_x.p, sizeof(double) * n, hipMemcpyDeviceToHost));
    }
  }
  return HF_OK;
}
// ... 91 lines not shown
```

heatflow_amd/csrc/hf_context.hpp:

```cpp

#pragma once
#include <hip/hip_runtime.h>
#include <hip/hip_ext.h>

#include <algorithm>
#include <chrono>
#include <cmath>
#include <cstdarg>
#include <cstdint>
#include <cstdio>
#include <cstdlib>
#include <cstring>
#include <string>
#include <thread>
#include <vector>

#include "amg_host.hpp"
#include "heatflow_hip.h"

namespace {

constexpr int RB = 256;
#ifndef HF_RBA
#define HF_RBA 256
#endif
constexpr int RBA = HF_RBA;
constexpr int TPB = 256;
constexpr int NCOL = 32;
#ifndef HF_STAGE_U
#define HF_STAGE_U 2
#endif
#ifndef HF_UNROLL
#define HF_UNROLL 4
#endif
constexpr int MAXP = 1024;
constexpr int MAXRESP = 4;
#ifndef HF_PROJ_MH
#define HF_PROJ_MH 6
#endif
constexpr int PROJ_MH = HF_PROJ_MH;
constexpr int PROJ_MT = PROJ_MH + MAXRESP;
constexpr int TS = 512;
#ifndef HF_SPMV_RPC
#define HF_SPMV_RPC 512
#endif
#ifndef HF_SPMV_UN
#define HF_SPMV_UN 8
#endif
constexpr int SRPC = HF_SPMV_RPC;

struct ScalMirror {
  double zz, bn2;
  int iters;
  int pad_;
  unsigned long long done_st;
  unsigned long long tested_st;
};
inline int mirror_tested(const ScalMirror* m, unsigned epoch) {
  const unsigned long long v = __atomic_load_n(&m->tested_st, __ATOMIC_ACQUIRE);
  return static_cast<unsigned>(v >> 32) == epoch ? static_cast<int>(v & 0xffffffffu) - 1 : -1;
}
inline int mirror_done(const ScalMirror* m, unsigned epoch) {
  const unsigned long long v = __atomic_load_n(&m->done_st, __ATOMIC_ACQUIRE);
  return static_cast<unsigned>(v >> 32) == epoch ? static_cast<int>(v & 0xffffffffu) : 0;
}

struct Scal {
  double tol2;
  double bn2;
  double zz;
  int iters;
  int done;
  int first;
  unsigned epoch;
  ScalMirror* mirror;
};

constexpr int NV_MAX = 16;
struct BRed { double pAp[NV_MAX], rz[2][NV_MAX], zz[NV_MAX], bn[NV_MAX]; };

constexpr int KT_MAX_KNOTS = 256;
constexpr int KT_MAX_PICARD = 8;
struct KTab { double t0, inv_dt; int n, off; };

struct TanDir { int32_t c_r, c_z; double w_r, w_z; };

enum RgVariant { RG_ROWS, RG_ROWS_K, RG_AN, RG_AN_K, RG_KT, RG_CT, RG_KT_K, RG_SOURCE, RG_VARIANTS };

}

struct hf_ctx {
  int dev = 0;
  hipStream_t stream = nullptr;
  hipEvent_t ev0 = nullptr, ev1 = nullptr;
  std::string err;
  double last_ms = 0.0;

  int32_t n = 0, ne = 0, nbc = 0;
  int64_t nnz = 0;
  int nchunks = 0, P = 0;
  int nchunks_s = 0, Ps = 0;
  int max_chunk_nnz_s = 0;
  int32_t *d_cdict_ptr = nullptr, *d_cdict = nullptr;
  uint16_t* d_cid = nullptr;
  int max_cdict = 0;
  bool cdict_own = false;
  bool c16 = true;
  struct ValueLists {
    const double* src = nullptr;
    int32_t *vptr = nullptr, *count = nullptr, *info = nullptr;
    double* vlist = nullptr;
    uint32_t* cv = nullptr;
    int64_t cap = 0;
    int64_t sum_vlist = 0;
    int max_vlist = 0;
    bool valid = false;
  } vl[2];
  int vl_mode = 1;
  int vl_vcap = 0;
  int vl_occ = 0;
  bool have_mesh = false, have_mat = false, assembled = false;
  double dt = 0.0;
  double dt_step = 0.0;
  int mode = 0;
  int scheme = HF_TIME_BACKWARD_EULER;

  std::vector<int32_t> h_rowptr, h_colidx, h_tri, h_tag;
  std::vector<char> h_tag_used;
  bool owner_ready = false;

  double2* d_zr = nullptr;
  int4* d_elem = nullptr;
  int tab_len = 0;
  double *d_kappa = nullptr, *d_rhoc = nullptr;
  int32_t *d_rowptr = nullptr, *d_colidx = nullptr;
  int32_t *d_blk_eptr = nullptr, *d_blk_cptr = nullptr;
  int2* d_blk_ent = nullptr;
  int nblk_a = 0;
  int max_blk_nnz = 0, ncolors = 0;
  int64_t elist_len = 0;
  bool rg_ok = false;
  int4* d_rg_hdr = nullptr;
  uint16_t *d_rg_ell = nullptr, *d_rg_cid = nullptr;
  int32_t* d_rg_dict = nullptr;
  double2* d_rg_zrb = nullptr;
  int rg_max_dict = 0;
  int rg_grid[RG_VARIANTS] = {};
  int64_t n_rg_ell = 0, n_rg_dict = 0, n_cdict = 0;
  std::vector<int32_t> h_rg_tags;
  double *d_kappa_rg = nullptr, *d_rhoc_rg = nullptr;
  struct Aniso {
    bool on = false;
    double2* d_m = nullptr;
    std::vector<char> h_tag;
    std::vector<double> h_m;
    uint64_t hash = 0;
  } an;
  double *d_M = nullptr, *d_A = nullptr, *d_dinv = nullptr;
  int32_t* d_bc_dofs = nullptr;
  double* d_g = nullptr;
  int32_t nlift_rows = 0, nlift = 0;
  int32_t *d_lift_rows = nullptr, *d_lift_ptr = nullptr, *d_lift_bc = nullptr, *d_lift_slot = nullptr;
  double* d_lift_val = nullptr;
  double *d_u = nullptr, *d_b = nullptr, *d_r = nullptr, *d_p = nullptr, *d_Ap = nullptr;
  double *d_uprev = nullptr, *d_ustart = nullptr;
  bool have_prev = false;
  bool bdf_hist = false;
  int extrapolate = 1;
  int start_kind = 3;
  std::vector<double> h_g0, h_g1;
  int g_hist = 0;
  struct BcResponse { std::vector<double> dir; double* w = nullptr; };
  std::vector<BcResponse> resp;
  long long resp_solves = 0;
  struct Proj {
    double *V[PROJ_MT] = {nullptr}, *F[PROJ_MT] = {nullptr};
    bool used[PROJ_MT] = {false};
    int next = 0, pending = -1;
    double *G = nullptr, *alpha = nullptr, *part = nullptr;
    bool ready = false;
  } proj;
  double *d_tmp = nullptr;
  double *d_part_pAp = nullptr, *d_part_rz = nullptr, *d_part_zz = nullptr, *d_part_bn = nullptr;
  Scal* d_scal = nullptr;
  Scal* h_scal = nullptr;
  ScalMirror* h_mirror = nullptr;
  ScalMirror* d_mirror = nullptr;
  unsigned epoch = 0;
  int32_t* d_samp_idx = nullptr;
  double* d_samp = nullptr;
  int samp_cap = 0;
  int pred_iters = 0;
  int precond = 0;
  int amg_reuse = 0;
  bool amg_ready = false;
  struct DevCsr {
    int nrow = 0, ncol = 0, lanes = 8; int64_t nnz = 0; int32_t *ptr = nullptr, *idx = nullptr; double* val = nullptr;
    float* valf = nullptr;
    int max_row = 0;
    int rpc = 0, nchunks = 0, chunk_nnz = 0;
    int32_t *dptr = nullptr, *dict = nullptr;
    uint16_t* cid = nullptr;
    int max_dict = 0;
    int64_t ndict = 0;
  };
  struct DevLevel {
    DevCsr A, P, R, Rt, GP;
    double *dinv = nullptr, *x = nullptr, *cat = nullptr, *b = nullptr, *res = nullptr;
    bool own_b = false;
    double omega = 0; int n = 0;
  };
  std::vector<DevLevel> amg;
  double* d_coarse_inv = nullptr;
  float* d_coarse_inv_f = nullptr;
  int coarse_n = 0, coarse_ld = 0;
  bool amg_fine_stale = false;
  int amg_fuse0 = 0;
  bool amg_f32 = true;
  double amg_opc = 0.0, amg_setup_s = 0.0;
  struct OperatorPrint { double dt = 0.0; std::vector<double> kappa, rhoc; int32_t nbc = 0; uint64_t bc_hash = 0; int32_t scheme = 0; uint64_t an_hash = 0; } amg_print;
  long long amg_fallbacks = 0;
  struct Steady {
    bool ready = false;
    bool picard = false;
    KTab* hdr0 = nullptr;
    double* xprev = nullptr;
    unsigned long long* change = nullptr;
    int precond = 0, pred_iters = 0;
    int32_t nbc = 0, nlift_rows = 0, nlift = 0;
    int32_t *bc_dofs = nullptr, *lift_rows = nullptr, *lift_ptr = nullptr, *lift_bc = nullptr, *lift_slot = nullptr;
    double *g = nullptr, *lift_val = nullptr, *K = nullptr, *dinv = nullptr, *Kfree = nullptr;
    std::vector<DevLevel> amg;
    double* coarse_inv = nullptr;
    float* coarse_inv_f = nullptr;
    int coarse_n = 0, coarse_ld = 0;
    bool amg_ready = false, amg_fine_stale = false;
    double amg_opc = 0.0, amg_setup_s = 0.0;
    OperatorPrint amg_print;
  } steady;
  double* d_load = nullptr;
  bool have_load = false;
  struct Source {
    bool on = false;
    double* F1 = nullptr;
    double* sum = nullptr;
    int32_t* absorb = nullptr;
    std::vector<double> amp;
    size_t next = 0;
  } src;
  double *d_z = nullptr, *d_z2 = nullptr;
  bool flux_ready = false;
  int flux_valid = 0;
  double *d_M1 = nullptr, *d_dinv1 = nullptr, *d_gz = nullptr, *d_gr = nullptr, *d_bz = nullptr, *d_br = nullptr;
  int pred_flux[2] = {0, 0};
  struct BatchLevel { double *x = nullptr, *cat = nullptr, *b = nullptr, *res = nullptr; bool own_b = false; };
  struct Batch {
    int nv = 0;
    int opk = 0;
    const double *sysA = nullptr, *sysDinv = nullptr;
    double *A = nullptr, *dinv = nullptr, *lift_val = nullptr;
    double *A1 = nullptr, *lift1 = nullptr;
    double delta[NV_MAX] = {};
    double *g = nullptr;
    double *u = nullptr, *uprev = nullptr, *ustart = nullptr, *b = nullptr, *r = nullptr, *p = nullptr, *Ap = nullptr;
    double *z = nullptr, *z2 = nullptr, *tmp = nullptr;
    double *part_pAp = nullptr, *part_rz = nullptr, *part_zz = nullptr, *part_bn = nullptr;
    Scal *scal = nullptr, *h_scal = nullptr;
    ScalMirror *h_mirror = nullptr, *d_mirror = nullptr;
    unsigned epoch = 0;
    BRed* red = nullptr;
    std::vector<BatchLevel> lev;
    int Pb = 0, pred_iters = 0;
    bool have_prev = false;
    bool bdf_hist = false;
    double *pV[PROJ_MH] = {nullptr}, *pF[PROJ_MH] = {nullptr}, *pG = nullptr, *palpha = nullptr, *ppart = nullptr;
    bool pused[PROJ_MH] = {false};
    int pnext = 0, ppending = -1;
    unsigned loaded = 0;
    bool lds = false;
    const double* load = nullptr;
  } batch;
  struct BatchCols {
    int nv = 0, rpc = 0, nchunks = 0, cap_nnz = 0, cap_dict = 0;
    int32_t *ptr = nullptr, *dict = nullptr, *own = nullptr;
    uint16_t* id = nullptr;
  } bcols;
  Batch fluxb;
  Batch fluxnb;
  int32_t* d_fsamp_idx = nullptr;
  Batch tanb;
  struct Tangent {
    bool ready = false;
    int npar = 0, nv = 0;
    int32_t* col = nullptr;
    TanDir* dir = nullptr;
    double* F = nullptr;
    bool steady_state = false;
    std::vector<int64_t> lev_sig;
  } tan;
  int fsamp_cap = 0;
  struct KappaT {
    bool on = false;
    bool k_on = false, c_on = false;
    int picard = 1;
    KTab* hdr = nullptr;
    double* vals = nullptr;
    std::vector<char> tabled;
    KTab* chdr = nullptr;
    double* cvals = nullptr;
    std::vector<char> ctabled;
    double* w = nullptr;
    double *pic = nullptr, *b0 = nullptr;
    unsigned long long* change = nullptr;
    bool have_change = false;
  } kt;
  bool prof = false;
  std::vector<hipEvent_t> prof_ev;
  int prof_used = 0, prof_base = 0;
  double prof_spmv_ms = 0.0;
  long long prof_spmv_n = 0;
};

namespace {

int fail(hf_ctx* c, int code, const char* fmt, ...);
inline size_t pad16(size_t b) { return (b + 15) & ~static_cast<size_t>(15); }

inline void cpu_relax() {
#if defined(__x86_64__) || defined(__i386__)
  __builtin_ia32_pause();
#else
  std::this_thread::yield();
#endif
}
// ... 52 lines not shown
```

heatflow_amd/csrc/hf_kernels.hpp:

```cpp
#pragma once
#include <type_traits>

#include "hf_context.hpp"

namespace {


template <int NW = 4>
__device__ __forceinline__ double block_sum(double v, double* sw) {
#pragma unroll
  for (int o = 32; o > 0; o >>= 1) v += __shfl_down(v, o, 64);
  const int w = threadIdx.x >> 6;
  if ((threadIdx.x & 63) == 0) sw[w] = v;
  __syncthreads();
  double t = sw[0];
#pragma unroll
  for (int k = 1; k < NW; ++k) t += sw[k];
  __syncthreads();
  return t;
}

__device__ __forceinline__ double sum_partials(const double* __restrict__ part, int P, double* s4) {
  double v = 0.0;
  for (int k = threadIdx.x; k < P; k += TPB) v += part[k];
// ... 732 lines not shown
    double kappa = kappa_idx[tg];
    if (kh.n > 0) kappa = ktab_eval(kh, kvals, element_temperature(sU, ui, cj, ck));
    return element_row(Pi, Pj, Pk, 0.0, kappa);
  }
};

__global__ __launch_bounds__(RBA) void k_assemble_rows_kT_K(int nblk, int cap , int capd ,
                                                            const int32_t* __restrict__ rowptr, const int4* __restrict__ hdr,
                                                            const uint4* __restrict__ ell, const uint4* __restrict__ cid16,
                                                            const double2* __restrict__ zrb, const int32_t* __restrict__ dict,
                                                            const KTab* __restrict__ ktab, const double* __restrict__ kvals,
                                                            const double* __restrict__ kappa_idx, const double* __restrict__ u,
                                                            double* __restrict__ Kv) {
  extern __shared__ double smem[];
  __shared__ KTab sK[64];
  if (threadIdx.x < 64) sK[threadIdx.x] = ktab[threadIdx.x];
  rowgather_assemble(nblk, cap, capd, rowptr, hdr, ell, cid16, zrb, dict, RowsKappaTK{sK, kvals, kappa_idx, u}, nullptr, Kv, smem);
}

__global__ __launch_bounds__(TPB) void k_picard_w(int n, const double* __restrict__ u, const double* __restrict__ um1,
                                                  double* __restrict__ out) {
#pragma clang fp contract(off)
  for (int i = blockIdx.x * TPB + threadIdx.x; i < n; i += gridDim.x * TPB) out[i] = um1 ? (4.0 * u[i] - um1[i]) * (1.0 / 3.0) : u[i];
}

__global__ __launch_bounds__(TPB) void k_max_abs_diff(int n, const double* __restrict__ a, const double* __restrict__ b,
                                                      unsigned long long* __restrict__ out) {
  __shared__ double s[TPB];
  double m = 0.0;
  for (int i = blockIdx.x * TPB + threadIdx.x; i < n; i += gridDim.x * TPB) m = fmax(m, fabs(a[i] - b[i]));
  s[threadIdx.x] = m;
  __syncthreads();
  for (int h = TPB / 2; h > 0; h >>= 1) {
    if (threadIdx.x < h) s[threadIdx.x] = fmax(s[threadIdx.x], s[threadIdx.x + h]);
    __syncthreads();
  }
  if (threadIdx.x == 0) atomicMax(out, static_cast<unsigned long long>(__double_as_longlong(s[0])));
}

__global__ __launch_bounds__(TPB) void k_eval_state(int n, const double* __restrict__ u, const double* __restrict__ uprev,
                                                    double* __restrict__ out) {
#pragma clang fp contract(off)
  for (int i = blockIdx.x * TPB + threadIdx.x; i < n; i += gridDim.x * TPB) out[i] = uprev ? 2.0 * u[i] - uprev[i] : u[i];
}

__global__ void k_gather_coords(int64_t total, const int32_t* __restrict__ dict, const double2* __restrict__ zr,
                                double2* __restrict__ zrb) {
  const int64_t i = static_cast<int64_t>(blockIdx.x) * blockDim.x + threadIdx.x;
  if (i < total) zrb[i] = zr[dict[i]];
}

__global__ __launch_bounds__(TPB) void k_assemble_global(int ne, const int32_t* __restrict__ rowptr,
                                                         const int32_t* __restrict__ colidx,
                                                         const int4* __restrict__ elem,
                                                         const double2* __restrict__ zr,
                                                         const double* __restrict__ kappa_tab,
                                                         const double* __restrict__ rhoc_tab, double dt,
                                                         double* __restrict__ Mv, double* __restrict__ Av) {
  const int e = blockIdx.x * TPB + threadIdx.x;
  if (e >= ne) return;
  const int4 el = elem[e];
  const int nd[3] = {el.x, el.y, el.z};
  double m[6], kk[6], av6[6];
  element_local(zr[el.x], zr[el.y], zr[el.z], rhoc_tab[el.w], kappa_tab[el.w], m, kk);
#pragma unroll
  for (int q = 0; q < 6; ++q) av6[q] = fma(dt, kk[q], m[q]);
#pragma unroll
  for (int a = 0; a < 3; ++a) {
    const int s0 = rowptr[nd[a]], s1 = rowptr[nd[a] + 1];
#pragma unroll
    for (int b = 0; b < 3; ++b) {
      int s = s0;
      while (s < s1 && colidx[s] != nd[b]) ++s;
      const int q = sym_index(a, b);
      atomicAdd(&Mv[s], m[q]);
      atomicAdd(&Av[s], av6[q]);
    }
  }
}

__global__ __launch_bounds__(RBA) void k_grad_rhs(int n, const int32_t* __restrict__ blk_eptr,
                                                  const int2* __restrict__ blk_ent, const double2* __restrict__ zr,
                                                  const double* __restrict__ u, double* __restrict__ bz,
                                                  double* __restrict__ br) {
  __shared__ double sB[2 * RBA];
  const int blk = blockIdx.x;
  const int r0 = blk * RBA;
  const int r1 = min(n, r0 + RBA);
  for (int k = threadIdx.x; k < 2 * RBA; k += RBA) sB[k] = 0.0;
  __syncthreads();
  for (int q = blk_eptr[blk] + threadIdx.x; q < blk_eptr[blk + 1]; q += RBA) {
#pragma clang fp contract(off)
    const AsmEntry e = load_entry(blk_ent, q);
    const double2 p0 = zr[e.n0], p1 = zr[e.n1], p2 = zr[e.n2];
    const double u0 = u[e.n0], u1 = u[e.n1], u2 = u[e.n2];
    const double d = (p1.x - p0.x) * (p2.y - p0.y) - (p2.x - p0.x) * (p1.y - p0.y);
    const double area = 0.5 * fabs(d);
    const double gz = (u0 * (p1.y - p2.y) + u1 * (p2.y - p0.y) + u2 * (p0.y - p1.y)) / d;
    const double gr = (u0 * (p2.x - p1.x) + u1 * (p0.x - p2.x) + u2 * (p1.x - p0.x)) / d;
    const double rsum = (p0.y + p1.y) + p2.y;
    const double wgt[3] = {area * (p0.y + rsum) / 12.0, area * (p1.y + rsum) / 12.0, area * (p2.y + rsum) / 12.0};
    const int nd[3] = {e.n0, e.n1, e.n2};
    const unsigned owned = (e.w3 >> 8) & 7u;
#pragma unroll
    for (int a = 0; a < 3; ++a) {
      if (!((owned >> a) & 1u)) continue;
      atomicAdd(&sB[2 * (nd[a] - r0)], gz * wgt[a]);
      atomicAdd(&sB[2 * (nd[a] - r0) + 1], gr * wgt[a]);
    }
  }
  __syncthreads();
  for (int k = threadIdx.x; k < r1 - r0; k += RBA) {
    bz[r0 + k] = sB[2 * k];
    br[r0 + k] = sB[2 * k + 1];
  }
}

__global__ void k_take_lift(int nlift, const int32_t* __restrict__ slot, double* __restrict__ A,
                            double* __restrict__ val) {
  const int q = blockIdx.x * blockDim.x + threadIdx.x;
  if (q >= nlift) return;
  val[q] = A[slot[q]];
  A[slot[q]] = 0.0;
}

__global__ void k_bc_rows(int nbc, const int32_t* __restrict__ dofs, const int32_t* __restrict__ rowptr,
                          const int32_t* __restrict__ colidx, double* __restrict__ A) {
  const int q = blockIdx.x * blockDim.x + threadIdx.x;
  if (q >= nbc) return;
  const int row = dofs[q];
  for (int k = rowptr[row]; k < rowptr[row + 1]; ++k) A[k] = (colidx[k] == row) ? 1.0 : 0.0;
}

__global__ void k_dinv(int n, const int32_t* __restrict__ rowptr, const int32_t* __restrict__ colidx,
                       const double* __restrict__ A, double* __restrict__ dinv) {
  const int row = blockIdx.x * blockDim.x + threadIdx.x;
  if (row >= n) return;
  double d = 0.0;
  for (int k = rowptr[row]; k < rowptr[row + 1]; ++k)
    if (colidx[k] == row) d = A[k];
  dinv[row] = 1.0 / d;
}

__global__ void k_lift(int nrows, const int32_t* __restrict__ rows, const int32_t* __restrict__ ptr,
                       const int32_t* __restrict__ bc, const double* __restrict__ val,
                       const double* __restrict__ g, double* __restrict__ b) {
  const int q = blockIdx.x * blockDim.x + threadIdx.x;
  if (q >= nrows) return;
  double s = 0.0;
  for (int k = ptr[q]; k < ptr[q + 1]; ++k) s += val[k] * g[bc[k]];
  b[rows[q]] -= s;
}

__global__ void k_set_bc(int nbc, const int32_t* __restrict__ dofs, const double* __restrict__ g,
                         double* __restrict__ b, double* __restrict__ u) {
  const int q = blockIdx.x * blockDim.x + threadIdx.x;
  if (q >= nbc) return;
  b[dofs[q]] = g[q];
  u[dofs[q]] = g[q];
}

__global__ void k_gather(int ns, const int32_t* __restrict__ idx, const double* __restrict__ u,
                         double* __restrict__ out) {
  const int q = blockIdx.x * blockDim.x + threadIdx.x;
  if (q < ns) out[q] = u[idx[q]];
}

__global__ __launch_bounds__(TPB) void k_hold_load(int n, const int32_t* __restrict__ rowptr, const int32_t* __restrict__ colidx,
                                                   const double* __restrict__ K, const double* __restrict__ u,
                                                   const unsigned char* __restrict__ mask, double* __restrict__ F) {
  const int row = blockIdx.x * blockDim.x + threadIdx.x;
  if (row >= n) return;
  double s = 0.0;
  if (!mask[row])
    for (int k = rowptr[row]; k < rowptr[row + 1]; ++k) s += K[k] * u[colidx[k]];
  F[row] = s;
}

__global__ void k_mark_rows(int nq, const int32_t* __restrict__ idx, unsigned char* __restrict__ mask) {
  const int q = blockIdx.x * blockDim.x + threadIdx.x;
  if (q < nq) mask[idx[q]] = 1;
}

__device__ __forceinline__ unsigned long long mirror_stamp(unsigned epoch, int v) {
  return (static_cast<unsigned long long>(epoch) << 32) | static_cast<unsigned>(v);
}
__device__ __forceinline__ void mirror_publish(ScalMirror* m, double zz, int iters, int done, unsigned epoch) {
  if (m == nullptr) return;
  m->zz = zz;
  m->iters = iters;
  __hip_atomic_store(&m->done_st, mirror_stamp(epoch, done), __ATOMIC_RELAXED, __HIP_MEMORY_SCOPE_SYSTEM);
  __threadfence_system();
  __hip_atomic_store(&m->tested_st, mirror_stamp(epoch, iters + 1), __ATOMIC_RELEASE, __HIP_MEMORY_SCOPE_SYSTEM);
}
__device__ __forceinline__ void mirror_breakdown(ScalMirror* m, unsigned epoch) {
  if (m != nullptr) __hip_atomic_store(&m->done_st, mirror_stamp(epoch, 2), __ATOMIC_RELEASE, __HIP_MEMORY_SCOPE_SYSTEM);
}

struct ColComp { const int32_t* dptr; const int32_t* dict; const uint16_t* id; int xd_off; int own; };
struct ValComp : ColComp { const int32_t* vptr; const double* vlist; const uint32_t* cv; int vl_off; int vcap; };

#ifndef HF_NT_STREAM
#define HF_NT_STREAM 0
#endif
#ifndef HF_PIPE
#define HF_PIPE 1
#endif
#ifndef HF_PHASE_CLOCK
#define HF_PHASE_CLOCK -1
#endif
#if HF_PHASE_CLOCK >= 0
#ifndef HF_PHASE_CONV
#define HF_PHASE_CONV 0
#endif
__device__ unsigned long long g_phase[MAXP * 16];
#define HF_STAMP(slot)                                                                                   \
  do {                                                                                                   \
    if (MODE == HF_PHASE_CLOCK && C16 && (MODE != 0 || (part2 != nullptr) == (HF_PHASE_CONV != 0)) && threadIdx.x == 0 && (slot) < 16) \
      g_phase[blockIdx.x * 16 + (slot)] = wall_clock64();                                                \
  } while (0)
#else
#define HF_STAMP(slot) do { } while (0)
#endif
template <typename T>
__device__ __forceinline__ T stream_load(const T* p) {
#if HF_NT_STREAM
  return __builtin_nontemporal_load(p);
#else
  return *p;
#endif
}

__device__ __forceinline__ double bdf2_operand(double un, double unm1) { return (4.0 * un - unm1) * (1.0 / 3.0); }

template <int MODE, bool C16 = false, typename VT = double, int UN = 8, bool VC = false>
__global__ __launch_bounds__(TS) __attribute__((amdgpu_waves_per_eu(8, 8))) void k_spmv(int n, int nchunks, int rpc ,
                                              const int32_t* __restrict__ rowptr, const int32_t* __restrict__ colidx,
                                              const VT* __restrict__ vals, const double* __restrict__ x,
                                              double* __restrict__ y, Scal* __restrict__ scal,
                                              double* __restrict__ part0, const double* __restrict__ bvec,
                                              const double* __restrict__ dinv, double* __restrict__ pvec,
                                              double* __restrict__ part1, double* __restrict__ part2, double w,
                                              int npart ,
                                              int parity, typename std::conditional<VC, ValComp, ColComp>::type comp) {
  extern __shared__ double sprod[];
  __shared__ double s4[TS / 64];
  __shared__ int s_own;
  constexpr bool BDF = MODE >= 12 && MODE <= 15;
  auto opnd = [&](int c) { return BDF ? bdf2_operand(x[c], bvec[c]) : x[c]; };
  if ((MODE == 3 || MODE == 4 || MODE == 6 || MODE == 9) && scal->done) return;
  if ((MODE == 0 || MODE == 7) && scal != nullptr && scal->done) return;
  double acc0 = 0.0, acc1 = 0.0, acc2 = 0.0;
  double beta = 0.0;
  bool first9 = false;
  if (MODE == 9) {
    first9 = scal->first != 0;
    if (!first9) {
      double v0 = 0.0, v1 = 0.0, v2 = 0.0;
      for (int k = threadIdx.x; k < npart; k += TS) {
        v0 += part1[parity * MAXP + k];
        v1 += part1[(parity ^ 1) * MAXP + k];
        v2 += part2[k];
      }
      const double rz_new = block_sum<TS / 64>(v0, s4);
      const double rz_old = block_sum<TS / 64>(v1, s4);
      const double zz = block_sum<TS / 64>(v2, s4);
      const bool conv = zz <= scal->tol2;
      if (blockIdx.x == 0 && threadIdx.x == 0) {
        scal->zz = zz;
        if (conv) scal->done = 1;
      }
      if (conv) return;
      beta = rz_new / rz_old;
    }
  }
  auto cycle_gate = [&]() {
    if (!((MODE == 3 || MODE == 0) && part2 != nullptr)) return false;
    double v2 = 0.0;
    for (int k = threadIdx.x; k < npart; k += TS) v2 += part2[k];
    const double zz = block_sum<TS / 64>(v2, s4);
    const bool conv = zz <= scal->tol2;
    if (blockIdx.x == 0 && threadIdx.x == 0) {
      if (conv) { scal->zz = zz; scal->done = 1; }
      mirror_publish(scal->mirror, zz, scal->iters, conv ? 1 : 0, scal->epoch);
    }
    return conv;
  };
  constexpr bool PIPELINED = C16 && !VC && (HF_PIPE == 2 || (HF_PIPE == 1 && sizeof(VT) == 4));
  static_assert(!VC || (C16 && sizeof(VT) == 8), "value lists: the fine operator's f64 arrays on compressed columns");
  if (!PIPELINED && cycle_gate()) return;
  const ChunkIter sched(nchunks);
  HF_STAMP(0);
  int stamp_at = 1;
  (void)stamp_at;
  const int tpr = (MODE == 0 || MODE == 6 || MODE == 7) ? TS / rpc : 1;
  const int prel = static_cast<int>(threadIdx.x) / tpr;
  const int psub = static_cast<int>(threadIdx.x) % tpr;
  struct RowOps { double b, d, y, p, x; };
  auto row_operands = [&](int prc, bool from_slice) {
    RowOps e{0.0, 0.0, 0.0, 0.0, 0.0};
    if (MODE == 2 || MODE == 3 || MODE == 4 || MODE == 5 || MODE == 7 || MODE == 8 || MODE == 11 || MODE == 13 || MODE == 15) e.b = bvec[prc];
    if (MODE == 2 || MODE == 4 || MODE == 5 || MODE == 10 || MODE == 11 || MODE == 14 || MODE == 15) e.d = dinv[prc];
    if (MODE == 6 || (MODE == 9 && !first9)) e.y = y[prc];
    if (MODE == 9 && !first9) e.p = pvec[prc];
    if ((MODE == 4 || MODE == 8 || MODE == 9 || MODE == 11) && !from_slice) e.x = x[prc];
    if (BDF) e.x = x[prc];
    return e;
  };
  auto rows_phase = [&](bool pin, int prow, int pa, int pb, const RowOps& e) {
    if ((MODE == 0 || MODE == 6 || MODE == 7) && tpr > 1) {
      double s = 0.0;
      if (pin)
        for (int j = pa + psub; j < pb; j += tpr) s += sprod[j];
      for (int o = tpr >> 1; o > 0; o >>= 1) s += __shfl_down(s, o, 64);
      if (pin && psub == 0) {
        y[prow] = (MODE == 6) ? e.y + s : s;
        if (MODE == 7) acc0 += e.b * s;
      }
    } else if (pin) {
      const int row = prow;
      double s = 0.0;
      for (int j = pa; j < pb; ++j) s += sprod[j];
      if (MODE == 0) {
        y[row] = s;
      } else if (MODE == 2) {
        const double ri = e.b - s;
        const double zi = e.d * ri;
        y[row] = ri;
        pvec[row] = zi;
        acc0 += ri * zi;
        acc1 += zi * zi;
        acc2 += (e.d * e.b) * (e.d * e.b);
      } else if (MODE == 3) {
        y[row] = e.b - s;
      } else if (MODE == 4) {
        const double yi = e.x + w * e.d * (e.b - s);
        y[row] = yi;
        acc0 += e.b * yi;
      } else if (MODE == 5) {
        const double ri = e.b - s;
        y[row] = ri;
        pvec[row] = w * e.d * ri;
        acc1 += (e.d * ri) * (e.d * ri);
        acc2 += (e.d * e.b) * (e.d * e.b);
      } else if (MODE == 7) {
        y[row] = s;
        acc0 += e.b * s;
      } else if (MODE == 6) {
        y[row] = e.y + s;
      } else if (MODE == 8) {
        y[row] = s;
        pvec[row] = 2.0 * e.x - e.b;
      } else if (MODE == 10) {
        y[row] = s + w * e.d;
      } else if (MODE == 11) {
        y[row] = s + w * e.d;
        pvec[row] = 2.0 * e.x - e.b;
      } else if (BDF) {
        y[row] = (MODE == 14 || MODE == 15) ? s + w * e.d : s;
        pvec[row] = (MODE == 13 || MODE == 15) ? 2.0 * e.x - e.b : e.x;
      } else {
        const double api = first9 ? s : s + beta * e.y;
        const double pi = first9 ? e.x : e.x + beta * e.p;
        y[row] = api;
        pvec[row] = pi;
        acc0 += pi * api;
      }
    }
  };
  if (PIPELINED) {
    struct Bounds { int k0, k1, d0, d1; };
    auto bounds = [&](int ch) {
      Bounds q;
      const int a0 = ch * rpc, a1 = min(n, a0 + rpc);
      q.k0 = rowptr[a0]; q.k1 = rowptr[a1];
      q.d0 = comp.dptr[ch]; q.d1 = comp.dptr[ch + 1];
      return q;
    };
    int lhead[HF_STAGE_U];
    double v[UN];
    int id[UN];
    auto heads = [&](const Bounds& q, bool live) {
      const int dl = max(q.d1 - 1, 0), kl = max(q.k1 - 1, 0);
      const int t = static_cast<int>(threadIdx.x);
#pragma unroll
      for (int u = 0; u < HF_STAGE_U; ++u) lhead[u] = comp.dict[min(q.d0 + (live ? t + u * TS : (t & 31)), dl)];
      __builtin_amdgcn_sched_barrier(0);
#pragma unroll
      for (int u = 0; u < UN; ++u) {
        const int kk = min(q.k0 + (live ? t + u * TS : (t & 31)), kl);
        v[u] = static_cast<double>(stream_load(&vals[kk]));
        id[u] = static_cast<int>(stream_load(&comp.id[kk]));
      }
    };
    double* xd = sprod + comp.xd_off;
    Bounds cur = bounds(min(sched.chunk, nchunks - 1));
    heads(cur, sched.chunk < sched.end);
    if (cycle_gate()) return;
    for (int chunk = sched.chunk; chunk < sched.end; chunk += sched.step) {
      const bool more = chunk + sched.step < sched.end;
      const int r0 = chunk * rpc, r1 = min(n, r0 + rpc);
      const int k0 = cur.k0, k1 = cur.k1, d0 = cur.d0, nd = cur.d1 - cur.d0;
      const int prow = r0 + prel;
      const bool pin = prow < r1;
      const int prc = min(prow, r1 - 1);
      int c0[HF_STAGE_U];
      double x0[HF_STAGE_U];
#pragma unroll
      for (int u = 0; u < HF_STAGE_U; ++u) { c0[u] = lhead[u]; x0[u] = opnd(c0[u]); }
      const Bounds nxt = bounds(more ? chunk + sched.step : chunk);
      const int pa = rowptr[prc] - k0, pb = rowptr[prc + 1] - k0;
      RowOps e = row_operands(prc, comp.own != 0);
#pragma unroll
      for (int u = 0; u < HF_STAGE_U; ++u) {
        const int i = static_cast<int>(threadIdx.x) + u * TS;
        if (i < nd) {
          xd[i] = x0[u];
          if ((MODE == 4 || MODE == 8 || MODE == 9 || MODE == 11) && c0[u] == r0) s_own = i;
        }
      }
      for (int i = threadIdx.x + HF_STAGE_U * TS; i < nd; i += HF_STAGE_U * TS) {
        int c[HF_STAGE_U];
        double xv[HF_STAGE_U];
#pragma unroll
        for (int u = 0; u < HF_STAGE_U; ++u) c[u] = comp.dict[d0 + min(i + u * TS, nd - 1)];
#pragma unroll
        for (int u = 0; u < HF_STAGE_U; ++u) xv[u] = opnd(c[u]);
#pragma unroll
        for (int u = 0; u < HF_STAGE_U; ++u)
          if (i + u * TS < nd) {
            xd[i + u * TS] = xv[u];
            if ((MODE == 4 || MODE == 8 || MODE == 9 || MODE == 11) && c[u] == r0) s_own = i + u * TS;
          }
      }
      __syncthreads();
      HF_STAMP(stamp_at); ++stamp_at;
      if ((MODE == 4 || MODE == 8 || MODE == 9 || MODE == 11) && comp.own && pin) e.x = xd[s_own + (prow - r0)];
#pragma unroll
      for (int u = 0; u < UN; ++u) {
        const int kk = k0 + static_cast<int>(threadIdx.x) + u * TS;
        if (kk < k1) sprod[kk - k0] = v[u] * xd[id[u]];
      }
      for (int kb = k0 + UN * TS; kb < k1; kb += UN * TS) {
#pragma unroll
        for (int u = 0; u < UN; ++u) {
          const int kk = min(kb + static_cast<int>(threadIdx.x) + u * TS, k1 - 1);
          v[u] = static_cast<double>(stream_load(&vals[kk]));
          id[u] = static_cast<int>(stream_load(&comp.id[kk]));
        }
#pragma unroll
        for (int u = 0; u < UN; ++u) {
          const int kk = kb + static_cast<int>(threadIdx.x) + u * TS;
          if (kk < k1) sprod[kk - k0] = v[u] * xd[id[u]];
        }
      }
      heads(nxt, more);
      __syncthreads();
      HF_STAMP(stamp_at); ++stamp_at;
      rows_phase(pin, prow, pa, pb, e);
      __syncthreads();
      HF_STAMP(stamp_at); ++stamp_at;
      cur = nxt;
    }
  } else {
  const ChunkIter& sched_ = sched;
  for (int chunk = sched_.chunk; chunk < sched_.end; chunk += sched_.step) {
    const int r0 = chunk * rpc;
    const int r1 = min(n, r0 + rpc);
    const int k0 = rowptr[r0];
    const int k1 = rowptr[r1];
    const int prow = r0 + prel;
    const bool pin = prow < r1;
    int pa = 0, pb = 0;
    if (pin) {
      pa = rowptr[prow] - k0;
      pb = rowptr[prow + 1] - k0;
    }
    RowOps e = row_operands(min(prow, r1 - 1), C16 && comp.own != 0);
    if constexpr (VC) {
      double* xd = sprod + comp.xd_off;
      double* vl = sprod + comp.vl_off;
      const int d0 = comp.dptr[chunk], nd = comp.dptr[chunk + 1] - d0;
      const int v0 = comp.vptr[chunk], nv = comp.vptr[chunk + 1] - v0;
      const bool vin = nv <= comp.vcap;
      int k = k0 + threadIdx.x;
      std::uint32_t cw[HF_UNROLL];
#pragma unroll
      for (int u = 0; u < HF_UNROLL; ++u) cw[u] = (k + u * TS < k1) ? stream_load(&comp.cv[k + u * TS]) : 0u;
      double lv[2];
#pragma unroll
      for (int u = 0; u < 2; ++u) {
        const int i = static_cast<int>(threadIdx.x) + u * TS;
        lv[u] = (vin && i < nv) ? comp.vlist[v0 + i] : 0.0;
      }
      for (int i = threadIdx.x; i < nd; i += HF_STAGE_U * TS) {
        int c[HF_STAGE_U];
        double xv[HF_STAGE_U];
#pragma unroll
        for (int u = 0; u < HF_STAGE_U; ++u) c[u] = (i + u * TS < nd) ? comp.dict[d0 + i + u * TS] : 0;
#pragma unroll
        for (int u = 0; u < HF_STAGE_U; ++u) xv[u] = (i + u * TS < nd) ? opnd(c[u]) : 0.0;
#pragma unroll
        for (int u = 0; u < HF_STAGE_U; ++u)
          if (i + u * TS < nd) {
            xd[i + u * TS] = xv[u];
            if ((MODE == 4 || MODE == 8 || MODE == 9 || MODE == 11) && c[u] == r0) s_own = i + u * TS;
          }
      }
#pragma unroll
      for (int u = 0; u < 2; ++u) {
        const int i = static_cast<int>(threadIdx.x) + u * TS;
        if (vin && i < nv) vl[i] = lv[u];
      }
      if (vin)
        for (int i = threadIdx.x + 2 * TS; i < nv; i += TS) vl[i] = comp.vlist[v0 + i];
      __syncthreads();
      HF_STAMP(stamp_at); ++stamp_at;
      if ((MODE == 4 || MODE == 8 || MODE == 9 || MODE == 11) && comp.own && pin) e.x = xd[s_own + (prow - r0)];
// ... 338 lines not shown
    }
    const double t = block_sum<TPB / 64>(s, s4);
    if (threadIdx.x == 0) y[row] = (VMODE == 1) ? y0 + t : t;
  }
}

struct RespArgs { const double* w[MAXRESP]; double c[MAXRESP]; int k; };
__global__ __launch_bounds__(TPB) void k_start_vector(int n, const double* __restrict__ base, RespArgs a,
                                                      double* __restrict__ u) {
  for (int i = blockIdx.x * TPB + threadIdx.x; i < n; i += gridDim.x * TPB) {
    double s = base[i];
    for (int k = 0; k < a.k; ++k) s += a.c[k] * a.w[k][i];
    u[i] = s;
  }
}

struct ProjVecs { const double* V[PROJ_MT]; int slot[PROJ_MT]; int m; };

__global__ __launch_bounds__(TPB) void k_proj_dots(int n, ProjVecs a, const double* __restrict__ f, const double* __restrict__ Fnew,
                                                   double* __restrict__ part ) {
  __shared__ double sw[TPB / 64][2 * PROJ_MT];
  double ah[PROJ_MT], ag[PROJ_MT];
#pragma unroll
  for (int k = 0; k < PROJ_MT; ++k) { ah[k] = 0.0; ag[k] = 0.0; }
  const int stride = gridDim.x * TPB;
  for (int i = blockIdx.x * TPB + threadIdx.x; i < n; i += 2 * stride) {
    const int i2 = i + stride;
    const bool two = i2 < n;
    const double fi = f ? f[i] : 0.0, gi = Fnew ? Fnew[i] : 0.0;
    const double fj = (f && two) ? f[i2] : 0.0, gj = (Fnew && two) ? Fnew[i2] : 0.0;
    double v0[PROJ_MT], v1[PROJ_MT];
#pragma unroll
    for (int k = 0; k < PROJ_MT; ++k) {
      v0[k] = k < a.m ? a.V[k][i] : 0.0;
      v1[k] = (k < a.m && two) ? a.V[k][i2] : 0.0;
    }
#pragma unroll
    for (int k = 0; k < PROJ_MT; ++k) {
      ah[k] += v0[k] * fi;
      ag[k] += v0[k] * gi;
      ah[k] += v1[k] * fj;
      ag[k] += v1[k] * gj;
    }
  }
  const int lane = threadIdx.x & 63, wave = threadIdx.x >> 6;
#pragma unroll
  for (int k = 0; k < PROJ_MT; ++k)
    if (k < a.m) {
      double th = ah[k], tg = ag[k];
#pragma unroll
      for (int o = 32; o > 0; o >>= 1) { th += __shfl_down(th, o, 64); tg += __shfl_down(tg, o, 64); }
      if (lane == 0) { sw[wave][2 * k] = th; sw[wave][2 * k + 1] = tg; }
    }
  __syncthreads();
  if (static_cast<int>(threadIdx.x) < 2 * a.m) {
    double t = sw[0][threadIdx.x];
#pragma unroll
    for (int w = 1; w < TPB / 64; ++w) t += sw[w][threadIdx.x];
    part[threadIdx.x * MAXP + blockIdx.x] = t;
  }
}

static_assert(PROJ_MT * PROJ_MT <= 1024, "k_proj_solve holds one matrix entry per thread");
constexpr int PROJ_SOLVE_T = 1024;
__global__ __launch_bounds__(PROJ_SOLVE_T) void k_proj_solve(int P, ProjVecs a, int jnew, int do_solve, double* __restrict__ part,
                                                    double* __restrict__ G , double* __restrict__ alpha) {
  __shared__ double sh[PROJ_MT], sg[PROJ_MT];
  __shared__ double A[PROJ_MT][PROJ_MT + 1], bb[PROJ_MT], dd[PROJ_MT], xx[PROJ_MT];
  __shared__ int perm[PROJ_MT], piv, stop, rank_s;
  __shared__ double pmax;
  part += static_cast<size_t>(blockIdx.x) * 2 * PROJ_MT * MAXP;
  G += blockIdx.x * PROJ_MT * PROJ_MT;
  alpha += blockIdx.x * (PROJ_MT + 1);
  const int m = a.m, t = threadIdx.x, lane = t & 63, wave = t >> 6;
  for (int q = wave; q < 2 * m; q += PROJ_SOLVE_T / 64) {
    double v = 0.0;
    for (int k0 = 0; k0 < P; k0 += 256) {
      double e[4];
#pragma unroll
      for (int u = 0; u < 4; ++u) { const int k = k0 + lane + 64 * u; e[u] = k < P ? part[q * MAXP + k] : 0.0; }
      v += (e[0] + e[1]) + (e[2] + e[3]);
    }
#pragma unroll
    for (int o = 32; o > 0; o >>= 1) v += __shfl_down(v, o, 64);
    if (lane == 0) { if (q & 1) sg[q >> 1] = v; else sh[q >> 1] = v; }
  }
  __syncthreads();
  if (jnew >= 0 && t < m) { G[a.slot[t] * PROJ_MT + jnew] = sg[t]; G[jnew * PROJ_MT + a.slot[t]] = sg[t]; }
  if (!do_solve) return;
  __syncthreads();
  if (t < PROJ_MT + 1) alpha[t] = 0.0;
  if (t < m) {
    double gii = (jnew >= 0 && a.slot[t] == jnew) ? sg[t] : G[a.slot[t] * PROJ_MT + a.slot[t]];
    const bool ok = gii > 0.0 && gii < 1e300;
    dd[t] = ok ? 1.0 / sqrt(gii) : 0.0;
    perm[t] = t;
    xx[t] = 0.0;
  }
  __syncthreads();
  const int i = t / PROJ_MT, j = t % PROJ_MT;
  if (i < m && j < m) {
    double gij;
    if (jnew >= 0 && a.slot[j] == jnew) gij = sg[i];
    else if (jnew >= 0 && a.slot[i] == jnew) gij = sg[j];
    else gij = G[a.slot[i] * PROJ_MT + a.slot[j]];
    const bool ok = dd[i] > 0.0 && dd[j] > 0.0;
    A[i][j] = ok ? gij * dd[i] * dd[j] : (i == j ? 0.0 : 0.0);
  }
  if (t < m) bb[t] = sh[t] * dd[t];
  if (t == 0) { rank_s = 0; stop = 0; }
  __syncthreads();
  for (int c = 0; c < m; ++c) {
    if (t == 0) {
      int pi = c;
      double best = A[c][c];
      for (int q = c + 1; q < m; ++q)
        if (A[q][q] > best) { best = A[q][q]; pi = q; }
      if (c == 0) pmax = best;
      piv = pi;
      stop = !(best > 1e-12 * pmax) || !(best > 0.0);
    }
    __syncthreads();
    if (stop) break;
    const int pv = piv;
    if (pv != c) {
      if (t < m) { const double x0 = A[c][t]; A[c][t] = A[pv][t]; A[pv][t] = x0; }
      __syncthreads();
      if (t < m) { const double x0 = A[t][c]; A[t][c] = A[t][pv]; A[t][pv] = x0; }
      if (t == 0) {
        const double x0 = bb[c]; bb[c] = bb[pv]; bb[pv] = x0;
        const int p0 = perm[c]; perm[c] = perm[pv]; perm[pv] = p0;
      }
      __syncthreads();
    }
    if (i > c && i < m && j > c && j < m) A[i][j] -= A[i][c] / A[c][c] * A[c][j];
    if (i > c && i < m && j == c) bb[i] -= A[i][c] / A[c][c] * bb[c];
    if (t == 0) rank_s = c + 1;
    __syncthreads();
  }
  if (t != 0) return;
  const int rank = rank_s;
  for (int c = rank - 1; c >= 0; --c) {
    double v = bb[c];
    for (int q = c + 1; q < rank; ++q) v -= A[c][q] * xx[q];
    xx[c] = v / A[c][c];
  }
  bool finite = true;
  for (int c = 0; c < rank; ++c) finite = finite && (fabs(xx[c]) < 1e300);
  if (!finite) return;
  for (int c = 0; c < rank; ++c) alpha[a.slot[perm[c]]] = xx[c] * dd[perm[c]];
  alpha[PROJ_MT] = static_cast<double>(rank);
}

__global__ __launch_bounds__(TPB) void k_proj_combine(int n, ProjVecs a, const double* __restrict__ alpha, double* __restrict__ u) {
  double c[PROJ_MT];
#pragma unroll
  for (int k = 0; k < PROJ_MT; ++k) c[k] = k < a.m ? alpha[a.slot[k]] : 0.0;
  const int stride = gridDim.x * TPB;
  for (int i = blockIdx.x * TPB + threadIdx.x; i < n; i += 2 * stride) {
    const int i2 = i + stride;
    const bool two = i2 < n;
    double v0[PROJ_MT], v1[PROJ_MT];
#pragma unroll
    for (int k = 0; k < PROJ_MT; ++k) {
      v0[k] = k < a.m ? a.V[k][i] : 0.0;
      v1[k] = (k < a.m && two) ? a.V[k][i2] : 0.0;
    }
    double s0 = 0.0, s1 = 0.0;
#pragma unroll
    for (int k = 0; k < PROJ_MT; ++k) { s0 += c[k] * v0[k]; s1 += c[k] * v1[k]; }
    u[i] = s0;
    if (two) u[i2] = s1;
  }
}

__global__ __launch_bounds__(TPB) void k_copy2(int n, const double* __restrict__ a, double* __restrict__ a_out,
                                               const double* __restrict__ b, double* __restrict__ b_out) {
  for (int i = blockIdx.x * TPB + threadIdx.x; i < n; i += gridDim.x * TPB) {
    a_out[i] = a[i];
    b_out[i] = b[i];
  }
}

__global__ void k_zero_entries(int nq, const int32_t* __restrict__ idx, double* __restrict__ v) {
  const int q = blockIdx.x * blockDim.x + threadIdx.x;
  if (q < nq) v[idx[q]] = 0.0;
}

__global__ __launch_bounds__(TS) void k_stream_read(size_t n16a, const double2* __restrict__ a, size_t n16b,
                                                    const double2* __restrict__ b, double* __restrict__ sink) {
  double s = 0.0;
  const size_t stride = static_cast<size_t>(gridDim.x) * TS;
  for (int pass = 0; pass < 2; ++pass) {
    const double2* __restrict__ p = pass ? b : a;
    const size_t n16 = pass ? n16b : n16a;
    size_t i = static_cast<size_t>(blockIdx.x) * TS + threadIdx.x;
    for (; i + 3 * stride < n16; i += 4 * stride) {
      const double2 v0 = p[i], v1 = p[i + stride], v2 = p[i + 2 * stride], v3 = p[i + 3 * stride];
      s += (v0.x + v0.y) + (v1.x + v1.y) + (v2.x + v2.y) + (v3.x + v3.y);
    }
    for (; i < n16; i += stride) { const double2 v = p[i]; s += v.x + v.y; }
  }
  if (s == 1.2345678e301) sink[0] = s;
}

__global__ __launch_bounds__(TPB) void k_scale(int n, double w, const double* __restrict__ dinv,
                                               const double* __restrict__ b, double* __restrict__ x,
                                               const Scal* __restrict__ scal) {
  if (scal->done) return;
  for (int i = blockIdx.x * TPB + threadIdx.x; i < n; i += gridDim.x * TPB) x[i] = w * dinv[i] * b[i];
}

__global__ __launch_bounds__(TPB) void k_dense_mv(int n, int ld, const double* __restrict__ Ainv,
                                                  const double* __restrict__ b, double* __restrict__ x,
                                                  const Scal* __restrict__ scal) {
  __shared__ double half_sum[4];
  if (scal->done) return;
  const int lane = threadIdx.x & 63;
  const int wave = threadIdx.x >> 6;
  const int npair = (n + 1) >> 1;
  for (int pr = blockIdx.x; pr < npair; pr += gridDim.x) {
    const int row = 2 * pr + (wave >> 1);
    double s = 0.0;
    if (row < n) {
      const double2* arow = reinterpret_cast<const double2*>(Ainv + static_cast<size_t>(row) * ld);
      const double2* bv = reinterpret_cast<const double2*>(b);
      const int nv = ld >> 1;
      for (int j = (wave & 1) * 64 + lane; j < nv; j += 128) {
        const double2 a = arow[j];
        const double2 v = bv[j];
        s += a.x * v.x + a.y * v.y;
      }
    }
#pragma unroll
    for (int o = 32; o > 0; o >>= 1) s += __shfl_down(s, o, 64);
    if (lane == 0) half_sum[wave] = s;
    __syncthreads();
    if (lane == 0 && (wave & 1) == 0 && row < n) x[row] = half_sum[wave] + half_sum[wave + 1];
    __syncthreads();
  }
}

__global__ __launch_bounds__(TPB) void k_dense_mv_f32(int n, int ld , const float* __restrict__ Ainv,
                                                      const double* __restrict__ b, double* __restrict__ x,
                                                      const Scal* __restrict__ scal) {
  __shared__ double half_sum[4];
  if (scal->done) return;
  const int lane = threadIdx.x & 63;
  const int wave = threadIdx.x >> 6;
  const int npair = (n + 1) >> 1;
  for (int pr = blockIdx.x; pr < npair; pr += gridDim.x) {
    const int row = 2 * pr + (wave >> 1);
    double s = 0.0;
    if (row < n) {
      const float4* arow = reinterpret_cast<const float4*>(Ainv + static_cast<size_t>(row) * ld);
      const double2* bv = reinterpret_cast<const double2*>(b);
      const int nv = ld >> 2;
      for (int j = (wave & 1) * 64 + lane; j < nv; j += 128) {
        const float4 a = arow[j];
        const double2 v0 = bv[2 * j], v1 = bv[2 * j + 1];
        s += static_cast<double>(a.x) * v0.x + static_cast<double>(a.y) * v0.y + static_cast<double>(a.z) * v1.x + static_cast<double>(a.w) * v1.y;
      }
    }
#pragma unroll
    for (int o = 32; o > 0; o >>= 1) s += __shfl_down(s, o, 64);
    if (lane == 0) half_sum[wave] = s;
    __syncthreads();
    if (lane == 0 && (wave & 1) == 0 && row < n) x[row] = half_sum[wave] + half_sum[wave + 1];
    __syncthreads();
  }
}

__global__ void k_to_float(size_t n, const double* __restrict__ src, float* __restrict__ dst) {
  for (size_t i = static_cast<size_t>(blockIdx.x) * blockDim.x + threadIdx.x; i < n; i += static_cast<size_t>(gridDim.x) * blockDim.x)
    dst[i] = static_cast<float>(src[i]);
}

constexpr int GJ_B = 32;
__global__ __launch_bounds__(TPB) void k_gjb_rows(int n, int c0, int b, const double* __restrict__ W, double* __restrict__ R ) {
  __shared__ double D[GJ_B][GJ_B + 1], Di[GJ_B][GJ_B + 1];
  const int t = threadIdx.x, ld = 2 * n;
  for (int q = t; q < GJ_B * GJ_B; q += TPB) {
    const int r = q / GJ_B, c = q % GJ_B;
    D[r][c] = (r < b && c < b) ? W[static_cast<size_t>(c0 + r) * ld + c0 + c] : (r == c ? 1.0 : 0.0);
    Di[r][c] = r == c ? 1.0 : 0.0;
  }
  __syncthreads();
  for (int p = 0; p < b; ++p) {
    const double piv = D[p][p];
    __syncthreads();
    for (int q = t; q < 2 * GJ_B; q += TPB) {
      if (q < GJ_B) D[p][q] /= piv; else Di[p][q - GJ_B] /= piv;
    }
    __syncthreads();
    for (int q = t; q < GJ_B * 2 * GJ_B; q += TPB) {
      const int r = q / (2 * GJ_B), c = q % (2 * GJ_B);
      if (r == p) continue;
      const double f = D[r][p];
      if (c < GJ_B) { if (c != p) D[r][c] -= f * D[p][c]; } else Di[r][c - GJ_B] -= f * Di[p][c - GJ_B];
    }
    __syncthreads();
    for (int r = t; r < GJ_B; r += TPB)
      if (r != p) D[r][p] = 0.0;
    __syncthreads();
  }
  for (int j = blockIdx.x * TPB + t; j < n; j += gridDim.x * TPB) {
    const size_t col = static_cast<size_t>(c0 + b + j);
    double w[GJ_B];
#pragma unroll
    for (int r = 0; r < GJ_B; ++r) w[r] = r < b ? W[static_cast<size_t>(c0 + r) * ld + col] : 0.0;
    for (int r = 0; r < b; ++r) {
      double s = 0.0;
#pragma unroll
      for (int c = 0; c < GJ_B; ++c) s += Di[r][c] * w[c];
      R[static_cast<size_t>(r) * n + j] = s;
    }
  }
}

__global__ void k_gjb_fill(int n, const int32_t* __restrict__ ptr, const int32_t* __restrict__ idx, const double* __restrict__ val,
                           double* __restrict__ W) {
  const int i = blockIdx.x * blockDim.x + threadIdx.x;
  if (i >= n) return;
  double* w = W + static_cast<size_t>(i) * 2 * n;
  for (int k = ptr[i]; k < ptr[i + 1]; ++k) w[idx[k]] = val[k];
  w[n + i] = 1.0;
}

__global__ __launch_bounds__(TPB) void k_gjb_update(int n, int c0, int b, double* __restrict__ W, const double* __restrict__ R) {
  __shared__ double sC[64][GJ_B + 1], sR[GJ_B][64 + 1];
  const int ld = 2 * n, t = threadIdx.x;
  const int i0 = blockIdx.y * 64, j0 = blockIdx.x * 64;
  for (int q = t; q < 64 * GJ_B; q += TPB) {
    const int r = q / GJ_B, c = q % GJ_B;
    sC[r][c] = (i0 + r < n && c < b) ? W[static_cast<size_t>(i0 + r) * ld + c0 + c] : 0.0;
  }
  for (int q = t; q < GJ_B * 64; q += TPB) {
    const int r = q / 64, c = q % 64;
    sR[r][c] = (r < b && j0 + c < n) ? R[static_cast<size_t>(r) * n + j0 + c] : 0.0;
  }
  __syncthreads();
  const int ti = (t / 16) * 4, tj = (t % 16) * 4;
  double acc[4][4];
#pragma unroll
  for (int u = 0; u < 4; ++u)
#pragma unroll
    for (int v = 0; v < 4; ++v) acc[u][v] = 0.0;
  for (int k = 0; k < GJ_B; ++k) {
    double cu[4], rv[4];
#pragma unroll
    for (int u = 0; u < 4; ++u) cu[u] = sC[ti + u][k];
#pragma unroll
    for (int v = 0; v < 4; ++v) rv[v] = sR[k][tj + v];
#pragma unroll
    for (int u = 0; u < 4; ++u)
#pragma unroll
      for (int v = 0; v < 4; ++v) acc[u][v] += cu[u] * rv[v];
  }
#pragma unroll
  for (int u = 0; u < 4; ++u) {
    const int i = i0 + ti + u;
    if (i >= n) continue;
    const bool pivot_row = i >= c0 && i < c0 + b;
#pragma unroll
    for (int v = 0; v < 4; ++v) {
      const int j = j0 + tj + v;
      if (j >= n) continue;
      double* w = W + static_cast<size_t>(i) * ld + c0 + b + j;
      *w = pivot_row ? sR[i - c0][tj + v] : *w - acc[u][v];
    }
  }
}

__global__ __launch_bounds__(TPB) void k_pcg_update_amg(int n, int nchunks, int P, int parity, Scal* __restrict__ scal,
                                                        const double* __restrict__ part_pAp,
                                                        const double* __restrict__ part_rz, double* __restrict__ part_zz,
                                                        double* __restrict__ x, double* __restrict__ r,
                                                        const double* __restrict__ p, const double* __restrict__ Ap,
                                                        const double* __restrict__ dinv, double w, double* __restrict__ z0) {
  __shared__ double s4[4];
  if (scal->done) return;
  const double pAp = sum_partials(part_pAp, P, s4);
  const double rz = sum_partials(part_rz + parity * MAXP, P, s4);
  if (!(pAp > 0.0)) {
    if (blockIdx.x == 0 && threadIdx.x == 0) {
      scal->done = 2;
      mirror_breakdown(scal->mirror, scal->epoch);
    }
    return;
  }
  if (blockIdx.x == 0 && threadIdx.x == 0) { scal->iters += 1; scal->first = 0; }
  const double alpha = rz / pAp;
  double a_zz = 0.0;
  const ChunkIter sched(nchunks);
  for (int chunk = sched.chunk; chunk < sched.end; chunk += sched.step) {
    const int i = chunk * RB + threadIdx.x;
    if (i < n) {
      const double ri = r[i] - alpha * Ap[i];
      const double zi = dinv[i] * ri;
      x[i] += alpha * p[i];
      r[i] = ri;
      if (z0 != nullptr) z0[i] = w * zi;
      a_zz += zi * zi;
    }
  }
  const double t1 = block_sum(a_zz, s4);
  if (threadIdx.x == 0) part_zz[blockIdx.x] = t1;
}

}
```

heatflow_amd/csrc/hf_solver.hpp:

```cpp
#pragma once
#include "hf_pattern.hpp"

namespace {

using DevCsr = hf_ctx::DevCsr;
using DevLevel = hf_ctx::DevLevel;

void free_dev_csr(DevCsr& m) { dev_free(&m.ptr); dev_free(&m.idx); dev_free(&m.val); dev_free(&m.valf); dev_free(&m.dptr); dev_free(&m.dict); dev_free(&m.cid); m = DevCsr(); }

void free_amg(hf_ctx* ctx) {
  for (size_t l = 0; l < ctx->amg.size(); ++l) {
    DevLevel& L = ctx->amg[l];
    if (l > 0) { free_dev_csr(L.A); dev_free(&L.dinv); dev_free(&L.x); dev_free(&L.cat); }
    if (L.own_b) dev_free(&L.b);
    free_dev_csr(L.P); free_dev_csr(L.R); free_dev_csr(L.Rt); free_dev_csr(L.GP);
  }
  ctx->amg.clear();
  dev_free(&ctx->d_coarse_inv);
  dev_free(&ctx->d_coarse_inv_f);
  ctx->coarse_n = 0;
  ctx->amg_ready = false;
}

int lanes_for_avg(double avg) {
// ... 193 lines not shown
    HF_HIP(hipStreamSynchronize(ctx->stream));
    ctx->coarse_ld = ld;
    ctx->coarse_n = nc;
  }
  lap("+ dense inverse");
  ctx->amg_opc = op_complexity;
  ctx->amg_fine_stale = false;
  ctx->amg_ready = true;
  ctx->amg_setup_s = std::chrono::duration<double>(std::chrono::steady_clock::now() - t0).count();
  return HF_OK;
}

int build_amg(hf_ctx* ctx) {
  const auto t0 = std::chrono::steady_clock::now();
  free_amg(ctx);
  amg::Csr A0;
  A0.nrow = A0.ncol = ctx->n;
  A0.ptr.assign(ctx->h_rowptr.begin(), ctx->h_rowptr.end());
  A0.idx.assign(ctx->h_colidx.begin(), ctx->h_colidx.end());
  A0.val.resize(ctx->nnz);
  HF_HIP(copy_sync(ctx, A0.val.data(), ctx->d_A, sizeof(double) * ctx->nnz, hipMemcpyDeviceToHost));
  amg::Hierarchy H;
  amg::Params prm;
  amg_params(ctx, prm);
  auto lap = [&](const char* what) {
    if (prm.verbose) std::fprintf(stderr, "[amg setup] %-28s %.3f s\n", what, std::chrono::duration<double>(std::chrono::steady_clock::now() - t0).count());
  };
  lap("operator downloaded");
  if (!amg::build(std::move(A0), prm, H)) return fail(ctx, HF_ERR_STATE, "AMG set-up failed (non-positive diagonal or singular coarse operator)");
  lap("+ host hierarchy");
  ctx->amg.resize(H.levels.size());
  HF_TRY(upload_host_levels(ctx, H, 0));
  return finish_amg(ctx, H.levels.back().A, H.coarse_n, H.op_complexity, t0);
}

inline bool short_chunks(const DevCsr& m) { return m.nchunks > 0 && m.nnz <= static_cast<int64_t>(m.nchunks) * (7 * TS / 2); }

template <int SM, typename VT>
void launch_stream_t(hf_ctx* c, const DevCsr& m, const VT* val, const double* x, double* y, double* part0, const double* bvec,
                     double* conv_part) {
  const int npart = c->P;
  static const int grid_cap = std::getenv("HEATFLOW_STREAM_GRID") ? std::atoi(std::getenv("HEATFLOW_STREAM_GRID")) : MAXP;
  int grid = std::min(m.nchunks, (SM == 0 && part0 == nullptr) ? std::max(grid_cap, 1) : npart);
  if (grid >= 64) grid &= ~7;
#define HF_STREAM_ARGS2 m.nrow, m.nchunks, m.rpc, m.ptr, m.idx, val, x, y, c->d_scal, part0, bvec, static_cast<const double*>(nullptr), \
                        static_cast<double*>(nullptr), static_cast<double*>(nullptr), conv_part, 0.0, npart, 0
  if (m.cid != nullptr && sizeof(VT) == 4 && short_chunks(m))
    hipLaunchKernelGGL((k_spmv<SM, true, VT, 4>), dim3(grid), dim3(TS), static_cast<size_t>(m.chunk_nnz + m.max_dict) * 8, c->stream,
                       HF_STREAM_ARGS2, ColComp{m.dptr, m.dict, m.cid, m.chunk_nnz, 0});
  else if (m.cid != nullptr)
    hipLaunchKernelGGL((k_spmv<SM, true, VT>), dim3(grid), dim3(TS), static_cast<size_t>(m.chunk_nnz + m.max_dict) * 8, c->stream,
                       HF_STREAM_ARGS2, ColComp{m.dptr, m.dict, m.cid, m.chunk_nnz, 0});
  else
    hipLaunchKernelGGL((k_spmv<SM, false, VT>), dim3(grid), dim3(TS), static_cast<size_t>(m.chunk_nnz) * 8, c->stream,
                       HF_STREAM_ARGS2, ColComp{nullptr, nullptr, nullptr, 0, 0});
#undef HF_STREAM_ARGS2
}

template <int SM>
void launch_stream(hf_ctx* c, const DevCsr& m, const double* x, double* y, double* part0, const double* bvec, double* conv_part) {
  if (m.valf != nullptr) launch_stream_t<SM, float>(c, m, m.valf, x, y, part0, bvec, conv_part);
  else launch_stream_t<SM, double>(c, m, m.val, x, y, part0, bvec, conv_part);
}

template <int VMODE, typename VT>
void launch_vec_t(hf_ctx* c, const DevCsr& m, const VT* val, const double* x, double* y) {
  if (m.rpc > 0) {
    constexpr int SM = VMODE == 0 ? 0 : 6;
    static const int grid_cap = std::getenv("HEATFLOW_STREAM_GRID") ? std::atoi(std::getenv("HEATFLOW_STREAM_GRID")) : MAXP;
    int grid = std::min(m.nchunks, std::max(grid_cap, 1));
    if (grid >= 64) grid &= ~7;
#define HF_STREAM_ARGS m.nrow, m.nchunks, m.rpc, m.ptr, m.idx, val, x, y, c->d_scal, static_cast<double*>(nullptr),                       \
                       static_cast<const double*>(nullptr), static_cast<const double*>(nullptr), static_cast<double*>(nullptr),   \
                       static_cast<double*>(nullptr), static_cast<double*>(nullptr), 0.0, 0, 0
    if (m.cid != nullptr && sizeof(VT) == 4 && short_chunks(m))
      hipLaunchKernelGGL((k_spmv<SM, true, VT, 4>), dim3(grid), dim3(TS), static_cast<size_t>(m.chunk_nnz + m.max_dict) * 8, c->stream,
                         HF_STREAM_ARGS, ColComp{m.dptr, m.dict, m.cid, m.chunk_nnz, 0});
    else if (m.cid != nullptr)
      hipLaunchKernelGGL((k_spmv<SM, true, VT>), dim3(grid), dim3(TS), static_cast<size_t>(m.chunk_nnz + m.max_dict) * 8, c->stream,
                         HF_STREAM_ARGS, ColComp{m.dptr, m.dict, m.cid, m.chunk_nnz, 0});
    else
      hipLaunchKernelGGL((k_spmv<SM, false, VT>), dim3(grid), dim3(TS), static_cast<size_t>(m.chunk_nnz) * 8, c->stream,
                         HF_STREAM_ARGS, ColComp{nullptr, nullptr, nullptr, 0, 0});
#undef HF_STREAM_ARGS
    return;
  }
  if (m.lanes > 64) {
    hipLaunchKernelGGL((k_spmv_row<VMODE, VT>), dim3(std::max(1, std::min(m.nrow, 4096))), dim3(TPB), 0, c->stream, m.nrow, m.ptr,
                       m.idx, val, x, y, c->d_scal);
    return;
  }
  const int lanes = m.lanes;
  const long long threads = static_cast<long long>(m.nrow) * lanes;
  const int grid = static_cast<int>(std::max(1LL, std::min<long long>((threads + TPB - 1) / TPB, 2048)));
#define HF_VEC(L) hipLaunchKernelGGL((k_spmv_vec<L, VMODE, VT>), dim3(grid), dim3(TPB), 0, c->stream, m.nrow, m.ptr, m.idx, val, x, y, c->d_scal)
  switch (lanes) {
    case 4: HF_VEC(4); break;
    case 8: HF_VEC(8); break;
    case 16: HF_VEC(16); break;
    case 32: HF_VEC(32); break;
    default: HF_VEC(64); break;
  }
#undef HF_VEC
}

template <int VMODE>
void launch_vec(hf_ctx* c, const DevCsr& m, const double* x, double* y) {
  if (m.valf != nullptr) launch_vec_t<VMODE, float>(c, m, m.valf, x, y);
  else launch_vec_t<VMODE, double>(c, m, m.val, x, y);
}

enum CyclePart { CYCLE_ALL = 0, CYCLE_FIRST = 1, CYCLE_REST = 2 };
void vcycle(hf_ctx* c, int out_slot, bool test_convergence = false, CyclePart part = CYCLE_ALL) {
  const int nl = static_cast<int>(c->amg.size());
  DevLevel& L0 = c->amg[0];
  if (nl == 1) {
    if (part != CYCLE_REST)
      launch_spmv<4>(c, c->d_A, c->d_z, c->d_z2, c->d_part_rz + out_slot * MAXP, c->d_r, nullptr, nullptr, nullptr, L0.omega);
    return;
  }
  const bool fused0 = L0.GP.nrow > 0;
  if (L0.Rt.nrow > 0 && (fused0 || !c->amg_fine_stale)) {
    if (part != CYCLE_REST) launch_stream<0>(c, L0.Rt, c->d_r, c->amg[1].b, nullptr, nullptr, test_convergence ? c->d_part_zz : nullptr);
  } else {
    if (part != CYCLE_REST)
      launch_spmv<3>(c, c->d_A, c->d_z, c->d_tmp, nullptr, c->d_r, nullptr, nullptr,
                     test_convergence ? c->d_part_zz : nullptr);
    if (part != CYCLE_FIRST) launch_vec<0>(c, L0.R, c->d_tmp, c->amg[1].b);
  }
  if (part == CYCLE_FIRST) return;
  for (int l = 1; l + 1 < nl; ++l) launch_vec<0>(c, c->amg[l].Rt, c->amg[l].b, c->amg[l + 1].b);
  {
    DevLevel& Lc = c->amg[nl - 1];
    if (c->coarse_n > 0) {
      const int g = std::max(1, std::min((Lc.n + 1) / 2, 2048));
      if (c->d_coarse_inv_f != nullptr)
        hipLaunchKernelGGL(k_dense_mv_f32, dim3(g), dim3(TPB), 0, c->stream, Lc.n, c->coarse_ld, c->d_coarse_inv_f, Lc.b, Lc.res, c->d_scal);
      else
        hipLaunchKernelGGL(k_dense_mv, dim3(g), dim3(TPB), 0, c->stream, Lc.n, c->coarse_ld, c->d_coarse_inv, Lc.b, Lc.res, c->d_scal);
    } else {
      const int g = std::max(1, std::min((Lc.n + TPB - 1) / TPB, 1024));
      hipLaunchKernelGGL(k_scale, dim3(g), dim3(TPB), 0, c->stream, Lc.n, Lc.omega, Lc.dinv, Lc.b, Lc.res, c->d_scal);
    }
  }
  for (int l = nl - 2; l >= 1; --l) launch_vec<0>(c, c->amg[l].GP, c->amg[l].cat, c->amg[l].res);
  if (fused0) {
    launch_stream<7>(c, L0.GP, c->d_r, c->d_z2, c->d_part_rz + out_slot * MAXP, c->d_r, nullptr);
    return;
  }
  launch_vec<1>(c, L0.P, c->amg[1].res, c->d_z);
  launch_spmv<4>(c, c->d_A, c->d_z, c->d_z2, c->d_part_rz + out_slot * MAXP, c->d_r, nullptr, nullptr, nullptr, L0.omega);
}

void launch_amg_iteration(hf_ctx* c, double* x, int parity, CyclePart part = CYCLE_ALL) {
  if (part == CYCLE_REST) { vcycle(c, parity ^ 1, true, CYCLE_REST); return; }
  const bool timed = c->prof && c->prof_used < PROF_PAIRS;
  hipEvent_t e0 = timed ? c->prof_ev[2 * c->prof_used] : nullptr, e1 = timed ? c->prof_ev[2 * c->prof_used + 1] : nullptr;
  launch_spmv<9>(c, c->d_A, c->d_z2, c->d_Ap, c->d_part_pAp, nullptr, c->d_p, c->d_part_rz, c->d_part_zz, 0.0, nullptr, e0,
                 e1, parity);
  if (timed) c->prof_used++;
  hipLaunchKernelGGL(k_pcg_update_amg, dim3(c->P), dim3(TPB), 0, c->stream, c->n, c->nchunks, c->P, parity, c->d_scal,
                     c->d_part_pAp, c->d_part_rz, c->d_part_zz, x, c->d_r, c->d_p, c->d_Ap, c->d_dinv,
                     c->amg[0].omega, c->amg[0].GP.nrow > 0 ? static_cast<double*>(nullptr) : c->d_z);
  vcycle(c, parity ^ 1, true, part);
}

inline bool poll_enabled() {
  static const bool on = !(std::getenv("HEATFLOW_POLL") && std::getenv("HEATFLOW_POLL")[0] == '0');
  return on;
}

int reset_scal(hf_ctx* ctx) {
  *ctx->h_scal = Scal{};
  ctx->h_scal->mirror = ctx->d_mirror;
  HF_HIP(hipMemcpyAsync(ctx->d_scal, ctx->h_scal, sizeof(Scal), hipMemcpyHostToDevice, ctx->stream));
  HF_HIP(hipStreamSynchronize(ctx->stream));
  return HF_OK;
}

void harvest_profile(hf_ctx* ctx);

int read_scal(hf_ctx* ctx) {
  HF_HIP(hipMemcpyAsync(ctx->h_scal, ctx->d_scal, sizeof(Scal), hipMemcpyDeviceToHost, ctx->stream));
  HF_HIP(hipStreamSynchronize(ctx->stream));
  harvest_profile(ctx);
  return HF_OK;
}

int wait_tested(hf_ctx* ctx, int k) {
  static const double limit_s = std::getenv("HEATFLOW_POLL_TIMEOUT_S") ? std::atof(std::getenv("HEATFLOW_POLL_TIMEOUT_S")) : 60.0;
  ScalMirror* m = ctx->h_mirror;
  const unsigned ep = ctx->epoch;
  const auto t0 = std::chrono::steady_clock::now();
  auto last_query = t0;
  for (unsigned spin = 1;; ++spin) {
    const int tested = mirror_tested(m, ep);
    const int done = mirror_done(m, ep);
    if (tested >= k || done != 0) break;
    cpu_relax();
    if ((spin & 0x3ff) == 0) {
      const auto now = std::chrono::steady_clock::now();
      if (now - last_query < std::chrono::milliseconds(2)) continue;
      last_query = now;
      if (hipStreamQuery(ctx->stream) == hipSuccess) {
        if (mirror_tested(m, ep) >= k || mirror_done(m, ep) != 0) break;
        return fail(ctx, HF_ERR_HIP, "PCG progress: stream drained before the test of iteration %d ran (%s)", k, hipGetErrorString(hipGetLastError()));
      }
      if (std::chrono::duration<double>(std::chrono::steady_clock::now() - t0).count() > limit_s)
        return fail(ctx, HF_ERR_HIP, "PCG progress: no convergence test within %.0f s (waiting for iteration %d, at %d)", limit_s, k, tested);
    }
  }
  __atomic_thread_fence(__ATOMIC_ACQUIRE);
  ctx->h_scal->iters = m->iters;
  ctx->h_scal->zz = m->zz;
  ctx->h_scal->bn2 = m->bn2;
  ctx->h_scal->done = mirror_done(m, ep);
  return HF_OK;
}

void harvest_profile(hf_ctx* ctx) {
  if (ctx->prof) {
    for (int k = 0; k < ctx->prof_used; ++k) {
      float ms = 0.f;
      const bool ran = !ctx->h_scal->done || (ctx->prof_base + k) < ctx->h_scal->iters;
      if (ran && hipEventElapsedTime(&ms, ctx->prof_ev[2 * k], ctx->prof_ev[2 * k + 1]) == hipSuccess) {
        ctx->prof_spmv_ms += ms;
        ctx->prof_spmv_n += 1;
      }
    }
    ctx->prof_used = 0;
  }
}

int pcg_solve(hf_ctx* ctx, const LinSys& sys, bool use_amg, double rtol, double atol, int max_it, int* pred) {
  static const bool trace_res = std::getenv("HEATFLOW_TRACE_RES") != nullptr;
  ctx->epoch += 1;
  if (!use_amg) {
    launch_spmv<2>(ctx, sys.A, sys.x, ctx->d_r, ctx->d_part_rz, sys.b, ctx->d_z, ctx->d_part_zz, ctx->d_part_bn, 0.0,
                   sys.dinv);
    hipLaunchKernelGGL(k_pcg_begin, dim3(1), dim3(TPB), 0, ctx->stream, ctx->P, rtol, atol, ctx->d_part_zz,
                       ctx->d_part_bn, ctx->d_scal, ctx->epoch);
  } else {
    launch_spmv<5>(ctx, sys.A, sys.x, ctx->d_r, nullptr, sys.b, ctx->d_z, ctx->d_part_zz, ctx->d_part_bn,
                   ctx->amg[0].omega);
    hipLaunchKernelGGL(k_pcg_begin, dim3(1), dim3(TPB), 0, ctx->stream, ctx->P, rtol, atol, ctx->d_part_zz,
                       ctx->d_part_bn, ctx->d_scal, ctx->epoch);
    vcycle(ctx, 0);
  }
  HF_HIP(hipGetLastError());

  int launched = 0;
  if (use_amg && !trace_res && ctx->amg.size() > 1 && poll_enabled()) {
    ctx->prof_base = 0;
    auto finish = [&](int rc) {
      if (ctx->prof) { (void)hipStreamSynchronize(ctx->stream); harvest_profile(ctx); }
      return rc;
    };
    if (*pred <= 0) {
      HF_TRY(wait_tested(ctx, 0));
      if (ctx->h_scal->done == 1) return finish(HF_OK);
    }
    static const bool hold_back = !(std::getenv("HEATFLOW_HOLD_BACK") && std::getenv("HEATFLOW_HOLD_BACK")[0] == '0');
    int burst = std::max(1, std::min(max_it, *pred - 2));
    bool rest_pending = false;
    while (true) {
      if (rest_pending) launch_amg_iteration(ctx, sys.x, (launched - 1) & 1, CYCLE_REST);
      const bool split = hold_back && burst == 1 && launched > 0;
      for (int k = 0; k < burst; ++k) launch_amg_iteration(ctx, sys.x, (launched + k) & 1, split ? CYCLE_FIRST : CYCLE_ALL);
      rest_pending = split;
      launched += burst;
      HF_HIP(hipGetLastError());
      const int rc = wait_tested(ctx, launched);
      if (rc != HF_OK) return finish(rc);
      if (ctx->h_scal->done || launched >= max_it) break;
      burst = 1;
    }
    *pred = ctx->h_scal->iters;
    if (ctx->h_scal->done == 2) return finish(fail(ctx, HF_ERR_NOCONV, "PCG breakdown (p.Ap <= 0) after %d iterations", ctx->h_scal->iters));
    if (!ctx->h_scal->done)
      return finish(fail(ctx, HF_ERR_NOCONV, "PCG not converged in %d iterations (rel. residual %.3e)", ctx->h_scal->iters,
                         std::sqrt(ctx->h_scal->zz / std::max(ctx->h_scal->bn2, 1e-300))));
    return finish(HF_OK);
  }
  if (*pred <= 0) {
    HF_TRY(read_scal(ctx));
    if (ctx->h_scal->done == 1) return HF_OK;
  }
  int burst = std::max(1, std::min(max_it, *pred > 0 ? *pred : (use_amg ? 8 : 32)));
  if (trace_res) burst = 2;
  while (true) {
    ctx->prof_base = launched;
    for (int k = 0; k < burst; ++k) {
      if (use_amg) launch_amg_iteration(ctx, sys.x, (launched + k) & 1);
      else launch_pcg_iteration(ctx, sys, (launched + k) & 1);
    }
    launched += burst;
    HF_HIP(hipGetLastError());
    HF_TRY(read_scal(ctx));
    if (trace_res) std::fprintf(stderr, "[res] it %d rel %.3e\n", ctx->h_scal->iters, std::sqrt(ctx->h_scal->zz / std::max(ctx->h_scal->bn2, 1e-300)));
    if (ctx->h_scal->done) break;
    if (launched >= max_it) break;
    burst = std::max(1, std::min(std::max(use_amg ? 1 : 8, launched / 8), max_it - launched));
    if (trace_res) burst = 2;
  }
  *pred = ctx->h_scal->iters;
  if (ctx->h_scal->done == 2) return fail(ctx, HF_ERR_NOCONV, "PCG breakdown (p.Ap <= 0) after %d iterations", ctx->h_scal->iters);
  if (!ctx->h_scal->done)
    return fail(ctx, HF_ERR_NOCONV, "PCG not converged in %d iterations (rel. residual %.3e)", ctx->h_scal->iters,
                std::sqrt(ctx->h_scal->zz / std::max(ctx->h_scal->bn2, 1e-300)));
  return HF_OK;
}

void proj_clear(hf_ctx* ctx, bool ring_only = false) {
  for (int k = 0; k < (ring_only ? PROJ_MH : PROJ_MT); ++k) ctx->proj.used[k] = false;
  ctx->proj.next = 0;
  ctx->proj.pending = -1;
}

void proj_free(hf_ctx* ctx) {
  proj_clear(ctx);
  for (auto& v : ctx->proj.V) dev_free(&v);
  for (auto& v : ctx->proj.F) dev_free(&v);
  dev_free(&ctx->proj.G); dev_free(&ctx->proj.alpha); dev_free(&ctx->proj.part);
  ctx->proj.ready = false;
}

void free_responses(hf_ctx* ctx) {
  for (auto& r : ctx->resp) dev_free(&r.w);
  ctx->resp.clear();
  ctx->g_hist = 0;
  proj_clear(ctx);
}

int proj_ensure(hf_ctx* ctx) {
  hf_ctx::Proj& Q = ctx->proj;
  if (Q.ready) return HF_OK;
  for (int k = 0; k < PROJ_MT; ++k) {
    HF_TRY(dev_alloc(ctx, &Q.V[k], ctx->n));
    HF_TRY(dev_alloc(ctx, &Q.F[k], ctx->n));
  }
  HF_TRY(dev_alloc(ctx, &Q.G, PROJ_MT * PROJ_MT));
  HF_TRY(dev_alloc(ctx, &Q.alpha, PROJ_MT + 1));
  HF_TRY(dev_alloc(ctx, &Q.part, static_cast<size_t>(2) * PROJ_MT * MAXP));
  HF_HIP(hipMemsetAsync(Q.G, 0, sizeof(double) * PROJ_MT * PROJ_MT, ctx->stream));
  HF_HIP(hipMemsetAsync(Q.alpha, 0, sizeof(double) * (PROJ_MT + 1), ctx->stream));
  Q.ready = true;
  proj_clear(ctx);
  return HF_OK;
}

ProjVecs proj_active(const hf_ctx* ctx) {
  ProjVecs a{};
  a.m = 0;
  for (int k = 0; k < PROJ_MT; ++k)
    if (ctx->proj.used[k]) { a.V[a.m] = ctx->proj.V[k]; a.slot[a.m] = k; ++a.m; }
  return a;
}

int proj_store(hf_ctx* ctx, int slot, const double* u, const double* rhs) {
  hf_ctx::Proj& Q = ctx->proj;
  hipLaunchKernelGGL(k_copy2, dim3(ctx->P), dim3(TPB), 0, ctx->stream, ctx->n, u, Q.V[slot], rhs, Q.F[slot]);
  if (ctx->nbc > 0)
    hipLaunchKernelGGL(k_zero_entries, dim3((ctx->nbc + 255) / 256), dim3(256), 0, ctx->stream, ctx->nbc, ctx->d_bc_dofs, Q.V[slot]);
  Q.used[slot] = true;
  return HF_OK;
}

void proj_column(hf_ctx* ctx, int slot, const double* f, bool solve) {
  hf_ctx::Proj& Q = ctx->proj;
  const ProjVecs a = proj_active(ctx);
  hipLaunchKernelGGL(k_proj_dots, dim3(ctx->P), dim3(TPB), 0, ctx->stream, ctx->n, a, f, slot >= 0 ? Q.F[slot] : static_cast<const double*>(nullptr),
                     Q.part);
  hipLaunchKernelGGL(k_proj_solve, dim3(1), dim3(PROJ_SOLVE_T), 0, ctx->stream, ctx->P, a, slot, solve ? 1 : 0, Q.part, Q.G, Q.alpha);
}

int solve_response(hf_ctx* ctx, const std::vector<double>& dir, int max_it, double** w_out) {
  double* w = nullptr;
  HF_TRY(dev_alloc(ctx, &w, ctx->n));
  const int nb = ctx->nbc;
  HF_HIP(hipMemsetAsync(w, 0, sizeof(double) * ctx->n, ctx->stream));
  HF_HIP(hipMemsetAsync(ctx->d_b, 0, sizeof(double) * ctx->n, ctx->stream));
  HF_HIP(hipMemcpyAsync(ctx->d_g, dir.data(), sizeof(double) * nb, hipMemcpyHostToDevice, ctx->stream));
  if (ctx->nlift_rows > 0)
    hipLaunchKernelGGL(k_lift, dim3((ctx->nlift_rows + 255) / 256), dim3(256), 0, ctx->stream, ctx->nlift_rows,
                       ctx->d_lift_rows, ctx->d_lift_ptr, ctx->d_lift_bc, ctx->d_lift_val, ctx->d_g, ctx->d_b);
  hipLaunchKernelGGL(k_set_bc, dim3((nb + 255) / 256), dim3(256), 0, ctx->stream, nb, ctx->d_bc_dofs, ctx->d_g, ctx->d_b, w);
  const LinSys sys{ctx->d_A, ctx->d_dinv, w, ctx->d_b};
  const bool use_amg = ctx->precond == 1 && ctx->amg_ready;
  int pred = ctx->pred_iters;
  int rc = pcg_solve(ctx, sys, use_amg, 1e-8, 0.0, max_it, &pred);
  if (rc == HF_ERR_NOCONV && use_amg && ctx->h_scal->done == 2) rc = pcg_solve(ctx, sys, false, 1e-8, 0.0, max_it, &pred);
  if (rc != HF_OK) { dev_free(&w); return rc; }
  ctx->resp_solves += 1;
  *w_out = w;
  if (ctx->start_kind == 3 && ctx->proj.ready) {
    const int slot = PROJ_MH + static_cast<int>(ctx->resp.size());
    HF_TRY(proj_store(ctx, slot, w, ctx->d_b));
    proj_column(ctx, slot, nullptr, false);
  }
  return HF_OK;
}

int prepare_response(hf_ctx* ctx, const double* g_new, int max_it, RespArgs* ra) {
  const int nb = ctx->nbc;
  ra->k = 0;
  std::vector<double> rem(nb);
  double nrm2 = 0.0, gn2 = 0.0;
  for (int q = 0; q < nb; ++q) {
    rem[q] = (g_new[q] - ctx->h_g0[q]) - (ctx->h_g0[q] - ctx->h_g1[q]);
    nrm2 += rem[q] * rem[q];
    gn2 += g_new[q] * g_new[q];
  }
  if (!(nrm2 > 0.0)) return HF_OK;
  for (size_t k = 0; k < ctx->resp.size(); ++k) {
    const std::vector<double>& d = ctx->resp[k].dir;
    double c = 0.0;
    for (int q = 0; q < nb; ++q) c += d[q] * rem[q];
    for (int q = 0; q < nb; ++q) rem[q] -= c * d[q];
    ra->c[k] = c;
    ra->w[k] = ctx->resp[k].w;
  }
  double rn2 = 0.0;
  for (int q = 0; q < nb; ++q) rn2 += rem[q] * rem[q];
  if (rn2 > 1e-12 * nrm2 && nrm2 > 1e-18 * gn2 && ctx->resp.size() < static_cast<size_t>(MAXRESP)) {
    const double rn = std::sqrt(rn2);
    hf_ctx::BcResponse nr;
    nr.dir.resize(nb);
    for (int q = 0; q < nb; ++q) nr.dir[q] = rem[q] / rn;
    const int rc = solve_response(ctx, nr.dir, max_it, &nr.w);
    if (rc == HF_ERR_HIP) return rc;
    if (rc == HF_OK) {
      ra->c[ctx->resp.size()] = rn;
      ra->w[ctx->resp.size()] = nr.w;
      ctx->resp.push_back(std::move(nr));
    } else {
      ctx->start_kind = 1;
    }
  }
  ra->k = static_cast<int>(ctx->resp.size());
  return HF_OK;
}

struct StepLoad { const double* F = nullptr; double w = 0.0; };
StepLoad step_load(hf_ctx* ctx) {
  StepLoad L;
  if (ctx->have_load) { L.F = ctx->d_load; L.w = ctx->dt; }
  hf_ctx::Source& S = ctx->src;
  if (!S.on) return L;
  const double p = S.next < S.amp.size() ? S.amp[S.next] : 0.0;
  if (!S.amp.empty()) S.next += 1;
  if (ctx->have_load) {
    hipLaunchKernelGGL(k_source_sum, dim3(ctx->P), dim3(TPB), 0, ctx->stream, ctx->n, ctx->d_load, p, S.F1, S.sum);
    L.F = S.sum;
  } else {
    L.F = S.F1;
    L.w = ctx->dt * p;
  }
  return L;
}

void launch_rhs(hf_ctx* ctx, const StepLoad& L) {
  if (L.F)
    launch_spmv<10>(ctx, ctx->d_M, ctx->d_u, ctx->d_b, nullptr, nullptr, nullptr, nullptr, nullptr, L.w, L.F);
  else
    launch_spmv<0>(ctx, ctx->d_M, ctx->d_u, ctx->d_b);
}

void launch_rhs_bdf2(hf_ctx* ctx, bool extrap, const StepLoad& L) {
  const double* um1 = ctx->bdf_hist ? ctx->d_uprev : ctx->d_u;
  if (L.F) {
    if (extrap) launch_spmv<15>(ctx, ctx->d_M, ctx->d_u, ctx->d_b, nullptr, um1, ctx->d_ustart, nullptr, nullptr, L.w, L.F);
    else launch_spmv<14>(ctx, ctx->d_M, ctx->d_u, ctx->d_b, nullptr, um1, ctx->d_ustart, nullptr, nullptr, L.w, L.F);
  } else {
    if (extrap) launch_spmv<13>(ctx, ctx->d_M, ctx->d_u, ctx->d_b, nullptr, um1, ctx->d_ustart);
    else launch_spmv<12>(ctx, ctx->d_M, ctx->d_u, ctx->d_b, nullptr, um1, ctx->d_ustart);
  }
}

int kt_finish(hf_ctx* ctx) {
  if (ctx->nbc > 0) {
    if (ctx->nlift > 0)
      hipLaunchKernelGGL(k_take_lift, dim3((ctx->nlift + 255) / 256), dim3(256), 0, ctx->stream, ctx->nlift, ctx->d_lift_slot, ctx->d_A,
                         ctx->d_lift_val);
    hipLaunchKernelGGL(k_bc_rows, dim3((ctx->nbc + 255) / 256), dim3(256), 0, ctx->stream, ctx->nbc, ctx->d_bc_dofs, ctx->d_rowptr,
                       ctx->d_colidx, ctx->d_A);
  }
  hipLaunchKernelGGL(k_dinv, dim3((ctx->n + 255) / 256), dim3(256), 0, ctx->stream, ctx->n, ctx->d_rowptr, ctx->d_colidx, ctx->d_A,
                     ctx->d_dinv);
  HF_HIP(hipGetLastError());
  return HF_OK;
}

int kt_revalue(hf_ctx* ctx, const double* u, const double* uprev) {
  value_lists_touch(ctx, ctx->d_A);
  if (ctx->kt.c_on) value_lists_touch(ctx, ctx->d_M);
  if (ctx->kt.c_on)
    HF_TRY(launch_rowgather<RowsBothT>(ctx, &k_assemble_rows_cT, nullptr, ctx->d_rg_dict, ctx->kt.hdr, ctx->kt.vals, ctx->kt.chdr,
                                       ctx->kt.cvals, ctx->d_kappa_rg, ctx->d_rhoc_rg, ctx->dt, u, uprev, ctx->d_M, ctx->d_A));
  else
    HF_TRY(launch_rowgather<RowsKappaT>(ctx, &k_assemble_rows_kT, nullptr, ctx->d_rg_dict, ctx->kt.hdr, ctx->kt.vals,
                                        ctx->d_kappa_rg, ctx->d_rhoc_rg, ctx->dt, u, uprev, ctx->d_A));
  return kt_finish(ctx);
}

int steady_revalue(hf_ctx* ctx, const KTab* hdr, const double* u, double* Kout) {
  const auto info = []() -> const char* { return std::getenv("HEATFLOW_DEBUG") ? "[steady picard] k_assemble_rows_kT_K" : nullptr; };
  return launch_rowgather<RowsKappaTK>(ctx, &k_assemble_rows_kT_K, info, ctx->d_rg_dict, hdr, ctx->kt.vals, ctx->d_kappa_rg, u, Kout);
}

int step_solve(hf_ctx* ctx, double rtol, double atol, int max_it) {
  const LinSys sys{ctx->d_A, ctx->d_dinv, ctx->d_u, ctx->d_b};
  const bool use_amg = ctx->precond == 1 && ctx->amg_ready;
  int rc = pcg_solve(ctx, sys, use_amg, rtol, atol, max_it, &ctx->pred_iters);
  if (rc == HF_ERR_NOCONV && use_amg && ctx->h_scal->done == 2) {
    ctx->amg_fallbacks += 1;
    int pred = 0;
    rc = pcg_solve(ctx, sys, false, rtol, atol, max_it, &pred);
  }
  return rc;
}

int step_device(hf_ctx* ctx, const double* g_host, const double* g_dev, double rtol, double atol, int max_it, bool last = true) {
  const int nb = ctx->nbc;
  RespArgs ra{};
  ra.k = 0;
  const bool kt = ctx->kt.on;
  const int kind = kt && ctx->start_kind >= 2 ? 1 : ctx->start_kind;
  const bool projected = kind == 3;
  const bool bdf2 = ctx->scheme == HF_TIME_BDF2;
  if (projected) HF_TRY(proj_ensure(ctx));
  const bool hist_ok = nb > 0 && ctx->extrapolate && ctx->have_prev && ctx->g_hist >= 2;
  if (kind >= 2 && hist_ok && !(bdf2 && kind == 2)) HF_TRY(prepare_response(ctx, g_host, max_it, &ra));
  const int sweeps = kt ? ctx->kt.picard : 1;
  const bool ct = kt && ctx->kt.c_on;
  const bool track = kt && last;
  if (kt) {
    const double* um1 = bdf2 && ctx->bdf_hist ? ctx->d_uprev : nullptr;
    HF_TRY(kt_revalue(ctx, ctx->d_u, um1));
    if (ctx->precond == 1 && ctx->amg_ready) ctx->amg_fine_stale = true;
    if (track && sweeps == 1)
      hipLaunchKernelGGL(k_eval_state, dim3(ctx->P), dim3(TPB), 0, ctx->stream, ctx->n, ctx->d_u, um1, ctx->kt.pic);
    if (ct && sweeps > 1)
      hipLaunchKernelGGL(k_picard_w, dim3(ctx->P), dim3(TPB), 0, ctx->stream, ctx->n, ctx->d_u,
                         bdf2 ? (ctx->bdf_hist ? ctx->d_uprev : ctx->d_u) : nullptr, ctx->kt.w);
  }
  const double* g = g_dev ? g_dev : ctx->d_g;
  if (nb > 0 && !g_dev) HF_HIP(hipMemcpyAsync(ctx->d_g, g_host, sizeof(double) * nb, hipMemcpyHostToDevice, ctx->stream));
  const StepLoad L = step_load(ctx);
  if (bdf2 && (projected || !ctx->extrapolate)) {
    launch_rhs_bdf2(ctx, false, L);
    std::swap(ctx->d_uprev, ctx->d_ustart);
    ctx->bdf_hist = true;
    ctx->have_prev = true;
  } else if (bdf2) {
    launch_rhs_bdf2(ctx, true, L);
    HF_HIP(hipMemcpyAsync(ctx->d_uprev, ctx->d_u, sizeof(double) * ctx->n, hipMemcpyDeviceToDevice, ctx->stream));
    HF_HIP(hipMemcpyAsync(ctx->d_u, ctx->d_ustart, sizeof(double) * ctx->n, hipMemcpyDeviceToDevice, ctx->stream));
    ctx->bdf_hist = true;
    ctx->have_prev = true;
  } else if (projected) {
    launch_rhs(ctx, L);
    ctx->have_prev = true;
  } else if (ctx->extrapolate && ctx->have_prev) {
    if (L.F)
      launch_spmv<11>(ctx, ctx->d_M, ctx->d_u, ctx->d_b, nullptr, ctx->d_uprev, ctx->d_ustart, nullptr, nullptr, L.w, L.F);
    else
      launch_spmv<8>(ctx, ctx->d_M, ctx->d_u, ctx->d_b, nullptr, ctx->d_uprev, ctx->d_ustart);
    HF_HIP(hipMemcpyAsync(ctx->d_uprev, ctx->d_u, sizeof(double) * ctx->n, hipMemcpyDeviceToDevice, ctx->stream));
    if (ra.k > 0)
      hipLaunchKernelGGL(k_start_vector, dim3(ctx->P), dim3(TPB), 0, ctx->stream, ctx->n, ctx->d_ustart, ra, ctx->d_u);
    else
      HF_HIP(hipMemcpyAsync(ctx->d_u, ctx->d_ustart, sizeof(double) * ctx->n, hipMemcpyDeviceToDevice, ctx->stream));
  } else {
    launch_rhs(ctx, L);
    if (ctx->extrapolate) {
      HF_HIP(hipMemcpyAsync(ctx->d_uprev, ctx->d_u, sizeof(double) * ctx->n, hipMemcpyDeviceToDevice, ctx->stream));
      ctx->have_prev = true;
    }
  }
  const bool combine = projected && proj_active(ctx).m > 0;
  if (sweeps > 1 && !ct)
    HF_HIP(hipMemcpyAsync(ctx->kt.b0, ctx->d_b, sizeof(double) * ctx->n, hipMemcpyDeviceToDevice, ctx->stream));
  if (nb > 0) {
    if (ctx->nlift_rows > 0)
      hipLaunchKernelGGL(k_lift, dim3((ctx->nlift_rows + 255) / 256), dim3(256), 0, ctx->stream, ctx->nlift_rows,
                         ctx->d_lift_rows, ctx->d_lift_ptr, ctx->d_lift_bc, ctx->d_lift_val, g, ctx->d_b);
    if (!combine)
      hipLaunchKernelGGL(k_set_bc, dim3((nb + 255) / 256), dim3(256), 0, ctx->stream, nb, ctx->d_bc_dofs, g,
                         ctx->d_b, ctx->d_u);
  }
  if (combine) {
    hf_ctx::Proj& Q = ctx->proj;
    proj_column(ctx, Q.pending, ctx->d_b, true);
    Q.pending = -1;
    hipLaunchKernelGGL(k_proj_combine, dim3(ctx->P), dim3(TPB), 0, ctx->stream, ctx->n, proj_active(ctx), Q.alpha, ctx->d_u);
    if (nb > 0)
      hipLaunchKernelGGL(k_set_bc, dim3((nb + 255) / 256), dim3(256), 0, ctx->stream, nb, ctx->d_bc_dofs, g, ctx->d_b, ctx->d_u);
  }
  int rc = step_solve(ctx, rtol, atol, max_it);
  if (kt) {
    int total = ctx->h_scal->iters;
    for (int k = 2; k <= sweeps && rc == HF_OK; ++k) {
      if (track && k == sweeps)
        HF_HIP(hipMemcpyAsync(ctx->kt.pic, ctx->d_u, sizeof(double) * ctx->n, hipMemcpyDeviceToDevice, ctx->stream));
      HF_TRY(kt_revalue(ctx, ctx->d_u, nullptr));
      if (!ct)
        HF_HIP(hipMemcpyAsync(ctx->d_b, ctx->kt.b0, sizeof(double) * ctx->n, hipMemcpyDeviceToDevice, ctx->stream));
      else if (L.F)
        launch_spmv<10>(ctx, ctx->d_M, ctx->kt.w, ctx->d_b, nullptr, nullptr, nullptr, nullptr, nullptr, L.w, L.F);
      else
        launch_spmv<0>(ctx, ctx->d_M, ctx->kt.w, ctx->d_b);
      if (nb > 0) {
        if (ctx->nlift_rows > 0)
          hipLaunchKernelGGL(k_lift, dim3((ctx->nlift_rows + 255) / 256), dim3(256), 0, ctx->stream, ctx->nlift_rows,
                             ctx->d_lift_rows, ctx->d_lift_ptr, ctx->d_lift_bc, ctx->d_lift_val, g, ctx->d_b);
        hipLaunchKernelGGL(k_set_bc, dim3((nb + 255) / 256), dim3(256), 0, ctx->stream, nb, ctx->d_bc_dofs, g, ctx->d_b, ctx->d_u);
      }
      rc = step_solve(ctx, rtol, atol, max_it);
      total += ctx->h_scal->iters;
    }
    ctx->h_scal->iters = total;
    if (rc == HF_OK && track) {
      HF_HIP(hipMemsetAsync(ctx->kt.change, 0, sizeof(unsigned long long), ctx->stream));
      hipLaunchKernelGGL(k_max_abs_diff, dim3(ctx->P), dim3(TPB), 0, ctx->stream, ctx->n, ctx->d_u, ctx->kt.pic, ctx->kt.change);
      ctx->kt.have_change = true;
    }
  }
  if (rc == HF_OK && projected) {
    hf_ctx::Proj& Q = ctx->proj;
    HF_TRY(proj_store(ctx, Q.next, ctx->d_u, ctx->d_b));
    Q.pending = Q.next;
    Q.next = (Q.next + 1) % PROJ_MH;
  }
  if (rc == HF_OK && nb > 0) {
    ctx->h_g1.swap(ctx->h_g0);
    ctx->h_g0.assign(g_host, g_host + nb);
    if (ctx->g_hist < 2) ctx->g_hist += 1;
  }
  return rc;
}

int ensure_samples(hf_ctx* ctx, int ns) {
  if (ns <= ctx->samp_cap) return HF_OK;
  HF_TRY(dev_alloc(ctx, &ctx->d_samp_idx, ns));
  HF_TRY(dev_alloc(ctx, &ctx->d_samp, ns));
  ctx->samp_cap = ns;
  return HF_OK;
}

int build_lift(hf_ctx* ctx) {
  const int32_t n = ctx->n, nbc = ctx->nbc;
  std::vector<int32_t> dofs(nbc);
  HF_HIP(copy_sync(ctx, dofs.data(), ctx->d_bc_dofs, sizeof(int32_t) * nbc, hipMemcpyDeviceToHost));
  std::vector<int32_t> bc_index(n, -1);
  for (int32_t q = 0; q < nbc; ++q) bc_index[dofs[q]] = q;
  std::vector<int32_t> rows;
  for (int32_t q = 0; q < nbc; ++q) {
    const int32_t j = dofs[q];
    for (int32_t k = ctx->h_rowptr[j]; k < ctx->h_rowptr[j + 1]; ++k) {
      const int32_t i = ctx->h_colidx[k];
      if (bc_index[i] < 0) rows.push_back(i);
    }
  }
  std::sort(rows.begin(), rows.end());
  rows.erase(std::unique(rows.begin(), rows.end()), rows.end());
  std::vector<int32_t> ptr(rows.size() + 1, 0), lbc, lslot;
  for (size_t r = 0; r < rows.size(); ++r) {
    const int32_t i = rows[r];
    for (int32_t k = ctx->h_rowptr[i]; k < ctx->h_rowptr[i + 1]; ++k) {
      const int32_t q = bc_index[ctx->h_colidx[k]];
      if (q >= 0) { lbc.push_back(q); lslot.push_back(k); }
    }
    ptr[r + 1] = static_cast<int32_t>(lbc.size());
  }
  ctx->nlift_rows = static_cast<int32_t>(rows.size());
  ctx->nlift = static_cast<int32_t>(lbc.size());
  HF_TRY(dev_alloc(ctx, &ctx->d_lift_rows, rows.size()));
  HF_TRY(dev_alloc(ctx, &ctx->d_lift_ptr, ptr.size()));
  HF_TRY(dev_alloc(ctx, &ctx->d_lift_bc, lbc.size()));
  HF_TRY(dev_alloc(ctx, &ctx->d_lift_slot, lslot.size()));
  HF_TRY(dev_alloc(ctx, &ctx->d_lift_val, lbc.size()));
  if (!rows.empty()) HF_HIP(copy_sync(ctx, ctx->d_lift_rows, rows.data(), sizeof(int32_t) * rows.size(), hipMemcpyHostToDevice));
  HF_HIP(copy_sync(ctx, ctx->d_lift_ptr, ptr.data(), sizeof(int32_t) * ptr.size(), hipMemcpyHostToDevice));
  if (!lbc.empty()) {
    HF_HIP(copy_sync(ctx, ctx->d_lift_bc, lbc.data(), sizeof(int32_t) * lbc.size(), hipMemcpyHostToDevice));
    HF_HIP(copy_sync(ctx, ctx->d_lift_slot, lslot.data(), sizeof(int32_t) * lslot.size(), hipMemcpyHostToDevice));
  }
  return HF_OK;
}

}
```

Measured before the change: 806.0 million.

## Defer PCG x-update, fold projection store via buffer swaps, and wave-level projection solve

Several step-level changes are added and enabled by default. The AMG-PCG update kernel no longer writes x each iteration. It records a pending alpha, and the next SpMV (mode 9) or a final flush kernel applies x += alpha*p, which saves one streaming pass over x per iteration. The projection history store swaps buffer pointers instead of copying u and b into the history, with BC zeroing fused into the lift kernel. The combine is fused with the BC set, and the small Gram solve moves to a single-wave kernel using readlane. The cost is added state-tracking complexity (epochs, pending take slots) and a larger risk of correctness bugs around aliasing.

```diff
diff --git a/heatflow_amd/csrc/heatflow_hip.hip b/heatflow_amd/csrc/heatflow_hip.hip
--- a/heatflow_amd/csrc/heatflow_hip.hip
+++ b/heatflow_amd/csrc/heatflow_hip.hip
@@ -208,6 +208,7 @@
   ctx->h_rowptr.swap(T.rowptr);
   ctx->h_colidx.swap(T.colidx);
   ctx->nbc = 0; ctx->nlift = 0; ctx->nlift_rows = 0;
+  ctx->h_bc_dofs.clear();
   ctx->have_mesh = true;
   ctx->pred_iters = 0;
   ctx->flux_ready = false;
@@ -578,6 +579,8 @@
   hf_ctx* ctx = new hf_ctx();
   ctx->dev = device_id;
   if (const char* e = std::getenv("HEATFLOW_VALUE_LISTS")) ctx->vl_mode = (e[0] == '0') ? 0 : (e[0] == '2') ? 2 : 1;
+  if (const char* e = std::getenv("HEATFLOW_STEP_FOLD")) ctx->step_fold = (e[0] != '0');
+  if (const char* e = std::getenv("HEATFLOW_DEFER_X")) ctx->defer_x = (e[0] != '0');
   auto bail = [&](int rc) { *out = ctx; return rc; };
   if (hipSetDevice(device_id) != hipSuccess) return bail(fail(ctx, HF_ERR_HIP, "hipSetDevice(%d) failed", device_id));
   if (hipStreamCreateWithFlags(&ctx->stream, hipStreamNonBlocking) != hipSuccess)
@@ -590,7 +593,8 @@
       hipHostGetDevicePointer(reinterpret_cast<void**>(&ctx->d_mirror), ctx->h_mirror, 0) != hipSuccess)
     return bail(fail(ctx, HF_ERR_ALLOC, "hipHostMalloc (mapped) failed"));
   *ctx->h_mirror = ScalMirror{};
-  int rc = dev_alloc(ctx, &ctx->d_scal, 1);
+  int rc = dev_alloc(ctx, &ctx->d_scal, 2);
+  if (rc == HF_OK && hipMemsetAsync(ctx->d_scal, 0, 2 * sizeof(Scal), ctx->stream) != hipSuccess) rc = HF_ERR_HIP;
   if (rc == HF_OK) rc = dev_alloc(ctx, &ctx->d_part_pAp, MAXP);
   if (rc == HF_OK) rc = dev_alloc(ctx, &ctx->d_part_rz, 2 * MAXP);
   if (rc == HF_OK) rc = dev_alloc(ctx, &ctx->d_part_zz, MAXP);
@@ -811,6 +815,7 @@
   HF_TRY(dev_alloc(ctx, &ctx->d_bc_dofs, n_bc));
   HF_TRY(dev_alloc(ctx, &ctx->d_g, n_bc));
   if (n_bc > 0) HF_HIP(copy_sync(ctx, ctx->d_bc_dofs, dofs, sizeof(int32_t) * n_bc, hipMemcpyHostToDevice));
+  ctx->h_bc_dofs.assign(dofs, dofs + n_bc);
   HF_TRY(build_lift(ctx));
   free_amg(ctx);
   free_responses(ctx);
@@ -2179,7 +2184,10 @@
         out += static_cast<size_t>(k) * n;
         const bool on = k < slots && (single ? ctx->proj.used[k] : B.pused[k]);
         if (!on) { std::fill(out, out + n, 0.0); continue; }
-        if (single) {
+        if (single && s == 0 && k == ctx->proj.take) {
+          HF_HIP(copy_sync(ctx, out, ctx->d_u, sizeof(double) * n, hipMemcpyDeviceToHost));
+          for (const int32_t q : ctx->h_bc_dofs) out[q] = 0.0;
+        } else if (single) {
           HF_HIP(copy_sync(ctx, out, s ? ctx->proj.F[k] : ctx->proj.V[k], sizeof(double) * n, hipMemcpyDeviceToHost));
         } else {
           HF_HIP(copy_sync(ctx, wide.data(), s ? B.pF[k] : B.pV[k], sizeof(double) * n * B.nv, hipMemcpyDeviceToHost));
diff --git a/heatflow_amd/csrc/hf_context.hpp b/heatflow_amd/csrc/hf_context.hpp
--- a/heatflow_amd/csrc/hf_context.hpp
+++ b/heatflow_amd/csrc/hf_context.hpp
@@ -75,6 +75,13 @@
   unsigned epoch;
   ScalMirror* mirror;
 };
+struct ScalX : Scal {
+  double pend_alpha;
+  double* pend_x;
+  unsigned pend_epoch;
+  unsigned pad_;
+};
+static_assert(sizeof(ScalX) <= 2 * sizeof(Scal), "hf_create allocates d_scal as two Scal");
 
 constexpr int NV_MAX = 16;
 struct BRed { double pAp[NV_MAX], rz[2][NV_MAX], zz[NV_MAX], bn[NV_MAX]; };
@@ -177,9 +184,13 @@
     double *V[PROJ_MT] = {nullptr}, *F[PROJ_MT] = {nullptr};
     bool used[PROJ_MT] = {false};
     int next = 0, pending = -1;
+    int take = -1;
     double *G = nullptr, *alpha = nullptr, *part = nullptr;
     bool ready = false;
   } proj;
+  bool step_fold = true;
+  bool defer_x = true;
+  std::vector<int32_t> h_bc_dofs;
   double *d_tmp = nullptr;
   double *d_part_pAp = nullptr, *d_part_rz = nullptr, *d_part_zz = nullptr, *d_part_bn = nullptr;
   Scal* d_scal = nullptr;
diff --git a/heatflow_amd/csrc/hf_kernels.hpp b/heatflow_amd/csrc/hf_kernels.hpp
--- a/heatflow_amd/csrc/hf_kernels.hpp
+++ b/heatflow_amd/csrc/hf_kernels.hpp
@@ -908,6 +908,22 @@
   b[rows[q]] -= s;
 }
 
+__global__ void k_lift_zero(int nrows, const int32_t* __restrict__ rows, const int32_t* __restrict__ ptr,
+                            const int32_t* __restrict__ bc, const double* __restrict__ val,
+                            const double* __restrict__ g, double* __restrict__ b, int lift_blocks, int nq,
+                            const int32_t* __restrict__ idx, double* __restrict__ v) {
+  if (static_cast<int>(blockIdx.x) >= lift_blocks) {
+    const int q = (blockIdx.x - lift_blocks) * blockDim.x + threadIdx.x;
+    if (q < nq) v[idx[q]] = 0.0;
+    return;
+  }
+  const int q = blockIdx.x * blockDim.x + threadIdx.x;
+  if (q >= nrows) return;
+  double s = 0.0;
+  for (int k = ptr[q]; k < ptr[q + 1]; ++k) s += val[k] * g[bc[k]];
+  b[rows[q]] -= s;
+}
+
 __global__ void k_set_bc(int nbc, const int32_t* __restrict__ dofs, const double* __restrict__ g,
                          double* __restrict__ b, double* __restrict__ u) {
   const int q = blockIdx.x * blockDim.x + threadIdx.x;
@@ -1009,6 +1025,10 @@
   double acc0 = 0.0, acc1 = 0.0, acc2 = 0.0;
   double beta = 0.0;
   bool first9 = false;
+  constexpr bool X9 = MODE == 9;
+  bool pend9 = false;
+  double apend = 0.0;
+  double* xpend = nullptr;
   if (MODE == 9) {
     first9 = scal->first != 0;
     if (!first9) {
@@ -1028,6 +1048,11 @@
       }
       if (conv) return;
       beta = rz_new / rz_old;
+      if (X9) {
+        const ScalX* sx = static_cast<const ScalX*>(scal);
+        const unsigned pe = sx->pend_epoch;
+        if (pe != 0u && pe == scal->epoch) { pend9 = true; apend = sx->pend_alpha; xpend = sx->pend_x; }
+      }
     }
   }
   auto cycle_gate = [&]() {
@@ -1059,6 +1084,7 @@
     if (MODE == 2 || MODE == 4 || MODE == 5 || MODE == 10 || MODE == 11 || MODE == 14 || MODE == 15) e.d = dinv[prc];
     if (MODE == 6 || (MODE == 9 && !first9)) e.y = y[prc];
     if (MODE == 9 && !first9) e.p = pvec[prc];
+    if (MODE == 9 && pend9) e.b = xpend[prc];
     if ((MODE == 4 || MODE == 8 || MODE == 9 || MODE == 11) && !from_slice) e.x = x[prc];
     if (BDF) e.x = x[prc];
     return e;
@@ -1120,6 +1146,7 @@
         const double pi = first9 ? e.x : e.x + beta * e.p;
         y[row] = api;
         pvec[row] = pi;
+        if (pend9) xpend[row] = e.b + apend * e.p;
         acc0 += pi * api;
       }
     }
@@ -1764,6 +1791,142 @@
   alpha[PROJ_MT] = static_cast<double>(rank);
 }
 
+__device__ __forceinline__ int lane_value(int v, int l) { return __builtin_amdgcn_readlane(v, l); }
+__device__ __forceinline__ double lane_value(double v, int l) {
+  return __hiloint2double(__builtin_amdgcn_readlane(__double2hiint(v), l), __builtin_amdgcn_readlane(__double2loint(v), l));
+}
+
+__global__ __launch_bounds__(PROJ_SOLVE_T) void k_proj_solve_wave(int P, ProjVecs a, int jnew, int do_solve, const double* __restrict__ part,
+                                                                  double* __restrict__ G , double* __restrict__ alpha) {
+  __shared__ double sh[PROJ_MT], sg[PROJ_MT];
+  const int m = a.m, t = threadIdx.x, lane = t & 63, wave = t >> 6;
+  for (int q = wave; q < 2 * m; q += PROJ_SOLVE_T / 64) {
+    double v = 0.0;
+    for (int k0 = 0; k0 < P; k0 += 256) {
+      double e[4];
+#pragma unroll
+      for (int u = 0; u < 4; ++u) { const int k = k0 + lane + 64 * u; e[u] = k < P ? part[q * MAXP + k] : 0.0; }
+      v += (e[0] + e[1]) + (e[2] + e[3]);
+    }
+#pragma unroll
+    for (int o = 32; o > 0; o >>= 1) v += __shfl_down(v, o, 64);
+    if (lane == 0) { if (q & 1) sg[q >> 1] = v; else sh[q >> 1] = v; }
+  }
+  __syncthreads();
+  if (wave != 0) return;
+  const bool row = lane < m;
+  int slot = 0;
+#pragma unroll
+  for (int k = 0; k < PROJ_MT; ++k)
+    if (k == lane) slot = a.slot[k];
+  const double sgl = row ? sg[lane] : 0.0, shl = row ? sh[lane] : 0.0;
+  if (jnew >= 0 && row) { G[slot * PROJ_MT + jnew] = sgl; G[jnew * PROJ_MT + slot] = sgl; }
+  if (!do_solve) return;
+  double d = 0.0;
+  if (row) {
+    const double gii = (jnew >= 0 && slot == jnew) ? sgl : G[slot * PROJ_MT + slot];
+    const bool ok = gii > 0.0 && gii < 1e300;
+    d = ok ? 1.0 / sqrt(gii) : 0.0;
+  }
+  double Ai[PROJ_MT];
+#pragma unroll
+  for (int j = 0; j < PROJ_MT; ++j) {
+    const int sj = lane_value(slot, j);
+    const double dj = lane_value(d, j), sgj = lane_value(sgl, j);
+    double gij = G[slot * PROJ_MT + sj];
+    if (jnew >= 0 && sj == jnew) gij = sgl;
+    else if (jnew >= 0 && slot == jnew) gij = sgj;
+    const bool ok = row && j < m && d > 0.0 && dj > 0.0;
+    Ai[j] = ok ? gij * d * dj : 0.0;
+  }
+  double bi = shl * d;
+  int perm = lane, rank = 0;
+  double pmax = 0.0;
+  bool go = true;
+#pragma unroll
+  for (int c = 0; c < PROJ_MT; ++c) {
+    if (go && c < m) {
+      double dg = 0.0;
+#pragma unroll
+      for (int j = 0; j < PROJ_MT; ++j)
+        if (j == lane) dg = Ai[j];
+      int pv = c;
+      double best = lane_value(dg, c);
+#pragma unroll
+      for (int q = c + 1; q < PROJ_MT; ++q)
+        if (q < m) {
+          const double v = lane_value(dg, q);
+          if (v > best) { best = v; pv = q; }
+        }
+      if (c == 0) pmax = best;
+      go = (best > 1e-12 * pmax) && (best > 0.0);
+      if (go) {
+        if (pv != c) {
+#pragma unroll
+          for (int j = 0; j < PROJ_MT; ++j) {
+            const double rc = lane_value(Ai[j], c), rp = lane_value(Ai[j], pv);
+            Ai[j] = lane == c ? rp : lane == pv ? rc : Ai[j];
+          }
+          {
+            const double rc = lane_value(bi, c), rp = lane_value(bi, pv);
+            bi = lane == c ? rp : lane == pv ? rc : bi;
+            const int qc = lane_value(perm, c), qp = lane_value(perm, pv);
+            perm = lane == c ? qp : lane == pv ? qc : perm;
+          }
+          const double xc = Ai[c];
+          double xp = 0.0;
+#pragma unroll
+          for (int j = 0; j < PROJ_MT; ++j)
+            if (j == pv) { xp = Ai[j]; Ai[j] = xc; }
+          Ai[c] = xp;
+        }
+        const double Acc = lane_value(Ai[c], c), bc = lane_value(bi, c);
+        const bool below = lane > c && lane < m;
+        const double f = Ai[c] / Acc;
+#pragma unroll
+        for (int j = c + 1; j < PROJ_MT; ++j) {
+          const double Acj = lane_value(Ai[j], c);
+          if (below && j < m) Ai[j] -= f * Acj;
+        }
+        if (below) bi -= f * bc;
+        rank = c + 1;
+      }
+    }
+  }
+  double xx[PROJ_MT];
+#pragma unroll
+  for (int c = 0; c < PROJ_MT; ++c) xx[c] = 0.0;
+#pragma unroll
+  for (int c = PROJ_MT - 1; c >= 0; --c) {
+    if (c < rank) {
+      double v = lane_value(bi, c);
+#pragma unroll
+      for (int q = c + 1; q < PROJ_MT; ++q)
+        if (q < rank) v -= lane_value(Ai[q], c) * xx[q];
+      xx[c] = v / lane_value(Ai[c], c);
+    }
+  }
+  bool finite = true;
+#pragma unroll
+  for (int c = 0; c < PROJ_MT; ++c)
+    if (c < rank) finite = finite && (fabs(xx[c]) < 1e300);
+  double xl = 0.0;
+#pragma unroll
+  for (int c = 0; c < PROJ_MT; ++c)
+    if (c == lane) xl = xx[c];
+  const double outv = xl * __shfl(d, perm, 64);
+  const int outs = __shfl(slot, perm, 64);
+  double al = 0.0;
+#pragma unroll
+  for (int c = 0; c < PROJ_MT; ++c) {
+    const int sc = lane_value(outs, c);
+    const double vc = lane_value(outv, c);
+    if (finite && c < rank && sc == lane) al = vc;
+  }
+  if (finite && lane == PROJ_MT) al = static_cast<double>(rank);
+  if (lane < PROJ_MT + 1) alpha[lane] = al;
+}
+
 __global__ __launch_bounds__(TPB) void k_proj_combine(int n, ProjVecs a, const double* __restrict__ alpha, double* __restrict__ u) {
   double c[PROJ_MT];
 #pragma unroll
@@ -1783,6 +1946,42 @@
     for (int k = 0; k < PROJ_MT; ++k) { s0 += c[k] * v0[k]; s1 += c[k] * v1[k]; }
     u[i] = s0;
     if (two) u[i2] = s1;
+  }
+}
+
+__global__ __launch_bounds__(TPB) void k_proj_combine_bc(int n, ProjVecs a, const double* __restrict__ alpha, double* __restrict__ u,
+                                                         int nbc, const int32_t* __restrict__ dofs, const double* __restrict__ g,
+                                                         double* __restrict__ b) {
+  double c[PROJ_MT];
+#pragma unroll
+  for (int k = 0; k < PROJ_MT; ++k) c[k] = k < a.m ? alpha[a.slot[k]] : 0.0;
+  const int stride = gridDim.x * TPB;
+  for (int i = blockIdx.x * TPB + threadIdx.x; i < n; i += 2 * stride) {
+    const int i2 = i + stride;
+    const bool two = i2 < n;
+    double v0[PROJ_MT], v1[PROJ_MT];
+#pragma unroll
+    for (int k = 0; k < PROJ_MT; ++k) {
+      v0[k] = k < a.m ? a.V[k][i] : 0.0;
+      v1[k] = (k < a.m && two) ? a.V[k][i2] : 0.0;
+    }
+    double s0 = 0.0, s1 = 0.0;
+#pragma unroll
+    for (int k = 0; k < PROJ_MT; ++k) { s0 += c[k] * v0[k]; s1 += c[k] * v1[k]; }
+    u[i] = s0;
+    if (two) u[i2] = s1;
+  }
+  if (nbc <= 0) return;
+  __syncthreads();
+  const int lo = blockIdx.x * TPB;
+  for (int q = threadIdx.x; q < nbc; q += TPB) {
+    const int dof = dofs[q];
+    const int res = dof % stride;
+    if (res >= lo && res < lo + TPB) {
+      const double gq = g[q];
+      b[dof] = gq;
+      u[dof] = gq;
+    }
   }
 }
 
@@ -2020,4 +2219,53 @@
   if (threadIdx.x == 0) part_zz[blockIdx.x] = t1;
 }
 
-}
+__global__ __launch_bounds__(TPB) void k_pcg_update_amg_defer(int n, int nchunks, int P, int parity, Scal* __restrict__ scal,
+                                                              const double* __restrict__ part_pAp,
+                                                              const double* __restrict__ part_rz, double* __restrict__ part_zz,
+                                                              double* x, double* __restrict__ r,
+                                                              const double* __restrict__ Ap,
+                                                              const double* __restrict__ dinv, double w, double* __restrict__ z0) {
+  __shared__ double s4[4];
+  if (scal->done) return;
+  const double pAp = sum_partials(part_pAp, P, s4);
+  const double rz = sum_partials(part_rz + parity * MAXP, P, s4);
+  if (!(pAp > 0.0)) {
+    if (blockIdx.x == 0 && threadIdx.x == 0) {
+      scal->done = 2;
+      static_cast<ScalX*>(scal)->pend_epoch = 0u;
+      mirror_breakdown(scal->mirror, scal->epoch);
+    }
+    return;
+  }
+  const double alpha = rz / pAp;
+  if (blockIdx.x == 0 && threadIdx.x == 0) {
+    scal->iters += 1;
+    scal->first = 0;
+    ScalX* sx = static_cast<ScalX*>(scal);
+    sx->pend_alpha = alpha;
+    sx->pend_x = x;
+    sx->pend_epoch = scal->epoch;
+  }
+  double a_zz = 0.0;
+  const ChunkIter sched(nchunks);
+  for (int chunk = sched.chunk; chunk < sched.end; chunk += sched.step) {
+    const int i = chunk * RB + threadIdx.x;
+    if (i < n) {
+      const double ri = r[i] - alpha * Ap[i];
+      const double zi = dinv[i] * ri;
+      r[i] = ri;
+      if (z0 != nullptr) z0[i] = w * zi;
+      a_zz += zi * zi;
+    }
+  }
+  const double t1 = block_sum(a_zz, s4);
+  if (threadIdx.x == 0) part_zz[blockIdx.x] = t1;
+}
+
+__global__ __launch_bounds__(TPB) void k_pcg_flush_x(int n, const ScalX* __restrict__ scal, double* __restrict__ x, const double* __restrict__ p) {
+  if (scal->pend_epoch == 0u || scal->pend_epoch != scal->epoch) return;
+  const double alpha = scal->pend_alpha;
+  for (int i = blockIdx.x * TPB + threadIdx.x; i < n; i += gridDim.x * TPB) x[i] += alpha * p[i];
+}
+
+}
diff --git a/heatflow_amd/csrc/hf_solver.hpp b/heatflow_amd/csrc/hf_solver.hpp
--- a/heatflow_amd/csrc/hf_solver.hpp
+++ b/heatflow_amd/csrc/hf_solver.hpp
@@ -369,6 +369,10 @@
   launch_spmv<4>(c, c->d_A, c->d_z, c->d_z2, c->d_part_rz + out_slot * MAXP, c->d_r, nullptr, nullptr, nullptr, L0.omega);
 }
 
+void flush_x(hf_ctx* c, double* x) {
+  if (c->defer_x) hipLaunchKernelGGL(k_pcg_flush_x, dim3(c->P), dim3(TPB), 0, c->stream, c->n, static_cast<const ScalX*>(c->d_scal), x, c->d_p);
+}
+
 void launch_amg_iteration(hf_ctx* c, double* x, int parity, CyclePart part = CYCLE_ALL) {
   if (part == CYCLE_REST) { vcycle(c, parity ^ 1, true, CYCLE_REST); return; }
   const bool timed = c->prof && c->prof_used < PROF_PAIRS;
@@ -376,9 +380,14 @@
   launch_spmv<9>(c, c->d_A, c->d_z2, c->d_Ap, c->d_part_pAp, nullptr, c->d_p, c->d_part_rz, c->d_part_zz, 0.0, nullptr, e0,
                  e1, parity);
   if (timed) c->prof_used++;
-  hipLaunchKernelGGL(k_pcg_update_amg, dim3(c->P), dim3(TPB), 0, c->stream, c->n, c->nchunks, c->P, parity, c->d_scal,
-                     c->d_part_pAp, c->d_part_rz, c->d_part_zz, x, c->d_r, c->d_p, c->d_Ap, c->d_dinv,
-                     c->amg[0].omega, c->amg[0].GP.nrow > 0 ? static_cast<double*>(nullptr) : c->d_z);
+  if (c->defer_x)
+    hipLaunchKernelGGL(k_pcg_update_amg_defer, dim3(c->P), dim3(TPB), 0, c->stream, c->n, c->nchunks, c->P, parity, c->d_scal,
+                       c->d_part_pAp, c->d_part_rz, c->d_part_zz, x, c->d_r, c->d_Ap, c->d_dinv,
+                       c->amg[0].omega, c->amg[0].GP.nrow > 0 ? static_cast<double*>(nullptr) : c->d_z);
+  else
+    hipLaunchKernelGGL(k_pcg_update_amg, dim3(c->P), dim3(TPB), 0, c->stream, c->n, c->nchunks, c->P, parity, c->d_scal,
+                       c->d_part_pAp, c->d_part_rz, c->d_part_zz, x, c->d_r, c->d_p, c->d_Ap, c->d_dinv,
+                       c->amg[0].omega, c->amg[0].GP.nrow > 0 ? static_cast<double*>(nullptr) : c->d_z);
   vcycle(c, parity ^ 1, true, part);
 }
 
@@ -492,6 +501,7 @@
       if (ctx->h_scal->done || launched >= max_it) break;
       burst = 1;
     }
+    flush_x(ctx, sys.x);
     *pred = ctx->h_scal->iters;
     if (ctx->h_scal->done == 2) return finish(fail(ctx, HF_ERR_NOCONV, "PCG breakdown (p.Ap <= 0) after %d iterations", ctx->h_scal->iters));
     if (!ctx->h_scal->done)
@@ -520,6 +530,7 @@
     burst = std::max(1, std::min(std::max(use_amg ? 1 : 8, launched / 8), max_it - launched));
     if (trace_res) burst = 2;
   }
+  if (use_amg) flush_x(ctx, sys.x);
   *pred = ctx->h_scal->iters;
   if (ctx->h_scal->done == 2) return fail(ctx, HF_ERR_NOCONV, "PCG breakdown (p.Ap <= 0) after %d iterations", ctx->h_scal->iters);
   if (!ctx->h_scal->done)
@@ -532,6 +543,7 @@
   for (int k = 0; k < (ring_only ? PROJ_MH : PROJ_MT); ++k) ctx->proj.used[k] = false;
   ctx->proj.next = 0;
   ctx->proj.pending = -1;
+  ctx->proj.take = -1;
 }
 
 void proj_free(hf_ctx* ctx) {
@@ -583,12 +595,25 @@
   return HF_OK;
 }
 
+int proj_settle(hf_ctx* ctx) {
+  hf_ctx::Proj& Q = ctx->proj;
+  if (Q.take < 0) return HF_OK;
+  HF_HIP(hipMemcpyAsync(Q.V[Q.take], ctx->d_u, sizeof(double) * ctx->n, hipMemcpyDeviceToDevice, ctx->stream));
+  if (ctx->nbc > 0)
+    hipLaunchKernelGGL(k_zero_entries, dim3((ctx->nbc + 255) / 256), dim3(256), 0, ctx->stream, ctx->nbc, ctx->d_bc_dofs, Q.V[Q.take]);
+  Q.take = -1;
+  return HF_OK;
+}
+
 void proj_column(hf_ctx* ctx, int slot, const double* f, bool solve) {
   hf_ctx::Proj& Q = ctx->proj;
   const ProjVecs a = proj_active(ctx);
   hipLaunchKernelGGL(k_proj_dots, dim3(ctx->P), dim3(TPB), 0, ctx->stream, ctx->n, a, f, slot >= 0 ? Q.F[slot] : static_cast<const double*>(nullptr),
                      Q.part);
-  hipLaunchKernelGGL(k_proj_solve, dim3(1), dim3(PROJ_SOLVE_T), 0, ctx->stream, ctx->P, a, slot, solve ? 1 : 0, Q.part, Q.G, Q.alpha);
+  if (ctx->step_fold)
+    hipLaunchKernelGGL(k_proj_solve_wave, dim3(1), dim3(PROJ_SOLVE_T), 0, ctx->stream, ctx->P, a, slot, solve ? 1 : 0, Q.part, Q.G, Q.alpha);
+  else
+    hipLaunchKernelGGL(k_proj_solve, dim3(1), dim3(PROJ_SOLVE_T), 0, ctx->stream, ctx->P, a, slot, solve ? 1 : 0, Q.part, Q.G, Q.alpha);
 }
 
 int solve_response(hf_ctx* ctx, const std::vector<double>& dir, int max_it, double** w_out) {
@@ -611,6 +636,7 @@
   ctx->resp_solves += 1;
   *w_out = w;
   if (ctx->start_kind == 3 && ctx->proj.ready) {
+    HF_TRY(proj_settle(ctx));
     const int slot = PROJ_MH + static_cast<int>(ctx->resp.size());
     HF_TRY(proj_store(ctx, slot, w, ctx->d_b));
     proj_column(ctx, slot, nullptr, false);
@@ -746,6 +772,8 @@
   const bool projected = kind == 3;
   const bool bdf2 = ctx->scheme == HF_TIME_BDF2;
   if (projected) HF_TRY(proj_ensure(ctx));
+  const bool take_bufs = ctx->step_fold && projected && !bdf2;
+  if (!take_bufs) HF_TRY(proj_settle(ctx));
   const bool hist_ok = nb > 0 && ctx->extrapolate && ctx->have_prev && ctx->g_hist >= 2;
   if (kind >= 2 && hist_ok && !(bdf2 && kind == 2)) HF_TRY(prepare_response(ctx, g_host, max_it, &ra));
   const int sweeps = kt ? ctx->kt.picard : 1;
@@ -762,6 +790,7 @@
                          bdf2 ? (ctx->bdf_hist ? ctx->d_uprev : ctx->d_u) : nullptr, ctx->kt.w);
   }
   const double* g = g_dev ? g_dev : ctx->d_g;
+  int taken = -1;
   if (nb > 0 && !g_dev) HF_HIP(hipMemcpyAsync(ctx->d_g, g_host, sizeof(double) * nb, hipMemcpyHostToDevice, ctx->stream));
   const StepLoad L = step_load(ctx);
   if (bdf2 && (projected || !ctx->extrapolate)) {
@@ -778,6 +807,7 @@
   } else if (projected) {
     launch_rhs(ctx, L);
     ctx->have_prev = true;
+    if (ctx->proj.take >= 0) { std::swap(ctx->d_u, ctx->proj.V[ctx->proj.take]); taken = ctx->proj.take; ctx->proj.take = -1; }
   } else if (ctx->extrapolate && ctx->have_prev) {
     if (L.F)
       launch_spmv<11>(ctx, ctx->d_M, ctx->d_u, ctx->d_b, nullptr, ctx->d_uprev, ctx->d_ustart, nullptr, nullptr, L.w, L.F);
@@ -799,7 +829,11 @@
   if (sweeps > 1 && !ct)
     HF_HIP(hipMemcpyAsync(ctx->kt.b0, ctx->d_b, sizeof(double) * ctx->n, hipMemcpyDeviceToDevice, ctx->stream));
   if (nb > 0) {
-    if (ctx->nlift_rows > 0)
+    if (taken >= 0) {
+      const int lb = (ctx->nlift_rows + 255) / 256;
+      hipLaunchKernelGGL(k_lift_zero, dim3(lb + (nb + 255) / 256), dim3(256), 0, ctx->stream, ctx->nlift_rows, ctx->d_lift_rows,
+                         ctx->d_lift_ptr, ctx->d_lift_bc, ctx->d_lift_val, g, ctx->d_b, lb, nb, ctx->d_bc_dofs, ctx->proj.V[taken]);
+    } else if (ctx->nlift_rows > 0)
       hipLaunchKernelGGL(k_lift, dim3((ctx->nlift_rows + 255) / 256), dim3(256), 0, ctx->stream, ctx->nlift_rows,
                          ctx->d_lift_rows, ctx->d_lift_ptr, ctx->d_lift_bc, ctx->d_lift_val, g, ctx->d_b);
     if (!combine)
@@ -810,9 +844,14 @@
     hf_ctx::Proj& Q = ctx->proj;
     proj_column(ctx, Q.pending, ctx->d_b, true);
     Q.pending = -1;
-    hipLaunchKernelGGL(k_proj_combine, dim3(ctx->P), dim3(TPB), 0, ctx->stream, ctx->n, proj_active(ctx), Q.alpha, ctx->d_u);
-    if (nb > 0)
-      hipLaunchKernelGGL(k_set_bc, dim3((nb + 255) / 256), dim3(256), 0, ctx->stream, nb, ctx->d_bc_dofs, g, ctx->d_b, ctx->d_u);
+    if (ctx->step_fold) {
+      hipLaunchKernelGGL(k_proj_combine_bc, dim3(ctx->P), dim3(TPB), 0, ctx->stream, ctx->n, proj_active(ctx), Q.alpha, ctx->d_u,
+                         nb, ctx->d_bc_dofs, g, ctx->d_b);
+    } else {
+      hipLaunchKernelGGL(k_proj_combine, dim3(ctx->P), dim3(TPB), 0, ctx->stream, ctx->n, proj_active(ctx), Q.alpha, ctx->d_u);
+      if (nb > 0)
+        hipLaunchKernelGGL(k_set_bc, dim3((nb + 255) / 256), dim3(256), 0, ctx->stream, nb, ctx->d_bc_dofs, g, ctx->d_b, ctx->d_u);
+    }
   }
   int rc = step_solve(ctx, rtol, atol, max_it);
   if (kt) {
@@ -845,7 +884,13 @@
   }
   if (rc == HF_OK && projected) {
     hf_ctx::Proj& Q = ctx->proj;
-    HF_TRY(proj_store(ctx, Q.next, ctx->d_u, ctx->d_b));
+    if (take_bufs) {
+      std::swap(ctx->d_b, Q.F[Q.next]);
+      Q.used[Q.next] = true;
+      Q.take = Q.next;
+    } else {
+      HF_TRY(proj_store(ctx, Q.next, ctx->d_u, ctx->d_b));
+    }
     Q.pending = Q.next;
     Q.next = (Q.next + 1) % PROJ_MH;
   }
```

After: 807.4 million, median of 2. No clear change (+0.2%).
